# HansiZeng/scaling-retriever

Hardware: AMD Instinct MI355X
Metric: MSMARCO-Dev queries/sec end-to-end (query encode + dense brute-force top-1000) (higher is better)
Workload: dtype f32

## Files before the change

include/sr_hip.h:

```cpp
#ifndef SR_HIP_H
#define SR_HIP_H
#include <stdint.h>
#ifdef __cplusplus
extern "C" {
#endif

#define SR_OK 0
#define SR_ERR_INVALID 1
#define SR_ERR_HIP 2
#define SR_ERR_NOMEM 3
#define SR_ERR_UNSUPPORTED 4

#define SR_DTYPE_F32 0
#define SR_DTYPE_BF16 1

typedef void* sr_stream;

const char* sr_last_error(void);
int sr_version(void);
int sr_max_topk(void);

typedef struct sr_dense_index sr_dense_index;

int sr_dense_index_create(sr_dense_index** out, int dim);
int sr_dense_index_add(sr_dense_index* idx, const float* d_rows, int64_t n_rows,
                       int64_t id_base, int64_t id_stride);
int64_t sr_dense_index_ntotal(const sr_dense_index* idx);
int sr_dense_search(sr_dense_index* idx, const float* d_queries, int64_t nq, int k,
                    float* d_out_scores, int64_t* d_out_ids, sr_stream stream);
#define SR_PRECISION_FP32 0
#define SR_PRECISION_BF16X3 1
#define SR_PRECISION_BF16X6 2
#define SR_PRECISION_FP32_FILTERED 3
int sr_dense_index_set_precision(sr_dense_index* idx, int mode);
int sr_dense_search_begin(sr_dense_index* idx, const float* d_queries, int64_t nq, int k, int share,
                          float* d_lower, sr_stream stream);
int sr_dense_search_finish(sr_dense_index* idx, const float* d_queries, int64_t nq, int k, const float* d_threshold,
                           float* d_out_scores, int64_t* d_out_ids, sr_stream stream);
int sr_dense_index_filter_stats(sr_dense_index* idx, int64_t* n_filtered, int64_t* n_fallback);
int sr_dense_index_filter_query_stats(sr_dense_index* idx, int64_t* n_certified, int64_t* n_redone);
int sr_dense_index_set_workspace_limit(sr_dense_index* idx, int64_t bytes);
int sr_dense_index_set_batch_invariant(sr_dense_index* idx, int on);
int sr_dense_index_destroy(sr_dense_index* idx);
int sr_dense_index_profile(sr_dense_index* idx, int enable);
int sr_dense_index_profile_read(sr_dense_index* idx, int64_t* n_launches, double* total_ms,
                                double* total_flop, double* total_d_bytes);

typedef struct sr_sparse_index sr_sparse_index;

int sr_sparse_index_create(sr_sparse_index** out, const int64_t* d_indptr,
                           const int32_t* d_doc_ids, const float* d_vals,
                           int64_t n_terms, int64_t n_docs, sr_stream stream);
int sr_sparse_search(sr_sparse_index* idx, const int64_t* d_q_indptr, const int32_t* d_q_cols,
                     const float* d_q_vals, int64_t nq, int k, float threshold,
                     int64_t id_base, int64_t id_stride,
                     float* d_out_scores, int64_t* d_out_ids, int32_t* d_out_counts,
                     sr_stream stream);
int sr_sparse_index_set_workspace_limit(sr_sparse_index* idx, int64_t bytes);
int sr_sparse_index_destroy(sr_sparse_index* idx);
int sr_sparse_index_work_counters(sr_sparse_index* idx, int enable, uint64_t* out6);
int sr_sparse_index_profile(sr_sparse_index* idx, int enable);
int sr_sparse_index_profile_read(sr_sparse_index* idx, int64_t* n_launches, double* total_ms,
                                 double* total_posting_bytes);
int sr_sparse_index_block_stats(sr_sparse_index* idx, int64_t* n_dense_terms, int64_t* n_block_calls,
                                int64_t* n_fallback_calls);

int sr_sparse_index_cert_stats(sr_sparse_index* idx, int64_t* out8);
int sr_sparse_index_cert_debug(sr_sparse_index* idx, int enable, uint16_t* h_keys, int64_t keys_capacity,
                               float* h_consts, int64_t nq_pad, float* vscale, int32_t* T);

int sr_sparse_csr_expand_terms(const int64_t* d_indptr, int64_t n_terms, int64_t nnz, int32_t* d_out_terms,
                               sr_stream stream);
int sr_sparse_csr_build(const int32_t* d_rows, const int32_t* d_cols, const float* d_vals, int64_t nnz,
                        int64_t n_terms, int64_t n_docs, int sort_docs, int64_t* d_indptr,
                        int32_t* d_out_rows, float* d_out_vals, sr_stream stream);

int sr_topk_merge(const float* d_scores, const int64_t* d_ids, int n_lists, int64_t nq, int k,
                  float pad_score, float* d_out_scores, int64_t* d_out_ids, sr_stream stream);

typedef struct sr_model sr_model;

typedef struct {
    int32_t vocab_size, hidden_size, intermediate_size, num_layers;
    int32_t num_heads, num_kv_heads, head_dim;
    float rms_norm_eps;
    float rope_theta;
    int32_t rope_llama3;
    float rope_factor, rope_low_freq_factor, rope_high_freq_factor;
    int32_t rope_original_max_pos;
    int32_t tie_word_embeddings;
    int32_t has_lm_head;
    int32_t max_batch_tokens;
    int32_t max_batch_seqs;
    int32_t fp32_planes;
} sr_model_config;

int sr_model_create(sr_model** out, const sr_model_config* cfg);
int sr_model_set_weight(sr_model* m, const char* name, const void* d_ptr, int dtype,
                        int64_t rows, int64_t cols, sr_stream stream);
int sr_model_finalize(sr_model* m);
int sr_encode_dense(sr_model* m, const int64_t* d_input_ids, const int64_t* d_attention_mask,
                    int32_t B, int32_t L, float* d_out, sr_stream stream);
int sr_encode_sparse(sr_model* m, const int64_t* d_input_ids, const int64_t* d_attention_mask,
                     int32_t B, int32_t L, float* d_out, sr_stream stream);
int sr_encode_dense_fp32(sr_model* m, const int64_t* d_input_ids, const int64_t* d_attention_mask,
                         int32_t B, int32_t L, float* d_out, sr_stream stream);
int sr_encode_sparse_fp32(sr_model* m, const int64_t* d_input_ids, const int64_t* d_attention_mask,
                          int32_t B, int32_t L, float* d_out, sr_stream stream);
int sr_encode_both(sr_model* m, const int64_t* d_input_ids, const int64_t* d_attention_mask,
                   int32_t B, int32_t L, int32_t fp32, float* d_out_sparse, float* d_out_dense,
                   sr_stream stream);
int sr_encode_rows(sr_model* m, const int64_t* d_input_ids, const int64_t* d_attention_mask, int32_t B, int32_t L,
                   const int32_t* d_row_shift, int32_t mode, int32_t fp32, float* d_out_sparse, float* d_out_dense,
                   sr_stream stream);
int sr_model_last_hidden(sr_model* m, float* d_out, int64_t capacity_rows, int64_t* n_tokens, sr_stream stream);
int sr_model_destroy(sr_model* m);

int sr_lora_merge(float* d_W, const float* d_A, const float* d_B, int64_t out_features,
                  int64_t in_features, int32_t r, float scale, sr_stream stream);

int sr_sparse_compact(const float* d_reps, int64_t B, int64_t V, int64_t* d_row_ptr,
                      int32_t* d_cols, float* d_vals, int64_t capacity, int64_t* h_nnz,
                      sr_stream stream);

int sr_write_run_json(const char* path, int64_t nq, int64_t k, const float* h_scores, const int64_t* h_idx, const int32_t* h_counts,
                      const int64_t* h_qid_i64, const char* h_qid_bytes, const int64_t* h_qid_off, int64_t qid_width,
                      const int64_t* h_doc_i64, const char* h_doc_bytes, const int64_t* h_doc_off, int64_t doc_width,
                      int64_t n_docs, int32_t n_threads, int64_t* bytes_written);
int sr_write_run_json_part(const char* path, int32_t part, int64_t nq, int64_t k, const float* h_scores, const int64_t* h_idx,
                           const int32_t* h_counts, const int64_t* h_qid_i64, const char* h_qid_bytes, const int64_t* h_qid_off,
                           int64_t qid_width, const int64_t* h_doc_i64, const char* h_doc_bytes, const int64_t* h_doc_off,
                           int64_t doc_width, int64_t n_docs, int32_t n_threads, int64_t* bytes_written);
int64_t sr_run_writer_mapped_rounds(void);

int sr_gemm_bf16(const void* d_A, const void* d_W, int32_t M, int32_t N, int32_t K, int32_t epilogue,
                 void* d_C, const int32_t* d_seq_of, sr_stream stream);
int sr_gemm_f16_scaled(const void* d_A, const void* d_W, int32_t M, int32_t N, int32_t K, const float* d_a_scale,
                       const float* d_w_scale, float* d_C, sr_stream stream);
int sr_gemm_qkv_rope(const void* d_A, const void* d_W, int32_t M, int32_t N, int32_t K, void* d_C,
                     const int32_t* d_pos, const float* d_rope_cos, const float* d_rope_sin,
                     int32_t n_rope, int32_t head_dim, sr_stream stream);
int sr_attention_varlen(const void* d_qkv, void* d_out, const int32_t* d_cu_seqlens, const int32_t* d_pos,
                        const uint8_t* d_key_valid, const float* d_rope_cos, const float* d_rope_sin,
                        int32_t B, int32_t num_heads, int32_t num_kv_heads, int32_t head_dim, sr_stream stream);

#ifdef __cplusplus
}
#endif
#endif
```

scaling_retriever_amd/_lib.py:

```python
import ctypes
import os
import threading

_HERE = os.path.dirname(os.path.abspath(__file__))
LIB_PATH = os.environ.get("SR_HIP_LIB") or os.path.join(_HERE, "libsr_hip.so")

SR_OK, SR_ERR_INVALID, SR_ERR_HIP, SR_ERR_NOMEM, SR_ERR_UNSUPPORTED = 0, 1, 2, 3, 4
SR_DTYPE_F32, SR_DTYPE_BF16 = 0, 1

c_void_p, c_int, c_int32, c_int64, c_float, c_char_p = (ctypes.c_void_p, ctypes.c_int, ctypes.c_int32,
                                                         ctypes.c_int64, ctypes.c_float, ctypes.c_char_p)


class SrModelConfig(ctypes.Structure):
    _fields_ = [
        ("vocab_size", c_int32), ("hidden_size", c_int32), ("intermediate_size", c_int32), ("num_layers", c_int32),
        ("num_heads", c_int32), ("num_kv_heads", c_int32), ("head_dim", c_int32),
        ("rms_norm_eps", c_float), ("rope_theta", c_float), ("rope_llama3", c_int32),
        ("rope_factor", c_float), ("rope_low_freq_factor", c_float), ("rope_high_freq_factor", c_float),
        ("rope_original_max_pos", c_int32), ("tie_word_embeddings", c_int32), ("has_lm_head", c_int32),
        ("max_batch_tokens", c_int32), ("max_batch_seqs", c_int32), ("fp32_planes", c_int32),
    ]


SIGNATURES = {
    "sr_last_error": (c_char_p, []),
    "sr_version": (c_int, []),
    "sr_max_topk": (c_int, []),
    "sr_dense_index_create": (c_int, [ctypes.POINTER(c_void_p), c_int]),
    "sr_dense_index_add": (c_int, [c_void_p, c_void_p, c_int64, c_int64, c_int64]),
    "sr_dense_index_ntotal": (c_int64, [c_void_p]),
    "sr_dense_search": (c_int, [c_void_p, c_void_p, c_int64, c_int, c_void_p, c_void_p, c_void_p]),
    "sr_dense_index_set_workspace_limit": (c_int, [c_void_p, c_int64]),
    "sr_dense_index_set_batch_invariant": (c_int, [c_void_p, c_int]),
    "sr_dense_index_set_precision": (c_int, [c_void_p, c_int]),
    "sr_dense_search_begin": (c_int, [c_void_p, c_void_p, c_int64, c_int, c_int, c_void_p, c_void_p]),
    "sr_dense_search_finish": (c_int, [c_void_p, c_void_p, c_int64, c_int, c_void_p, c_void_p, c_void_p, c_void_p]),
    "sr_dense_index_filter_stats": (c_int, [c_void_p, ctypes.POINTER(c_int64), ctypes.POINTER(c_int64)]),
    "sr_dense_index_filter_query_stats": (c_int, [c_void_p, ctypes.POINTER(c_int64), ctypes.POINTER(c_int64)]),
    "sr_dense_index_destroy": (c_int, [c_void_p]),
    "sr_dense_index_profile": (c_int, [c_void_p, c_int]),
    "sr_dense_index_profile_read": (c_int, [c_void_p, ctypes.POINTER(c_int64), ctypes.POINTER(ctypes.c_double),
                                            ctypes.POINTER(ctypes.c_double), ctypes.POINTER(ctypes.c_double)]),
    "sr_sparse_index_work_counters": (c_int, [c_void_p, c_int, ctypes.POINTER(ctypes.c_uint64)]),
    "sr_sparse_index_profile": (c_int, [c_void_p, c_int]),
    "sr_sparse_index_profile_read": (c_int, [c_void_p, ctypes.POINTER(c_int64), ctypes.POINTER(ctypes.c_double),
                                             ctypes.POINTER(ctypes.c_double)]),
    "sr_sparse_index_create": (c_int, [ctypes.POINTER(c_void_p), c_void_p, c_void_p, c_void_p, c_int64, c_int64,
                                       c_void_p]),
    "sr_sparse_search": (c_int, [c_void_p, c_void_p, c_void_p, c_void_p, c_int64, c_int, c_float, c_int64, c_int64,
                                 c_void_p, c_void_p, c_void_p, c_void_p]),
    "sr_sparse_index_set_workspace_limit": (c_int, [c_void_p, c_int64]),
    "sr_sparse_index_block_stats": (c_int, [c_void_p, ctypes.POINTER(c_int64), ctypes.POINTER(c_int64),
                                            ctypes.POINTER(c_int64)]),
    "sr_sparse_index_destroy": (c_int, [c_void_p]),
    "sr_sparse_index_cert_stats": (c_int, [c_void_p, ctypes.POINTER(c_int64)]),
    "sr_sparse_index_cert_debug": (c_int, [c_void_p, c_int, c_void_p, c_int64, c_void_p, c_int64,
                                           ctypes.POINTER(c_float), ctypes.POINTER(ctypes.c_int32)]),
    "sr_sparse_csr_expand_terms": (c_int, [c_void_p, c_int64, c_int64, c_void_p, c_void_p]),
    "sr_sparse_csr_build": (c_int, [c_void_p, c_void_p, c_void_p, c_int64, c_int64, c_int64, c_int, c_void_p, c_void_p,
                                    c_void_p, c_void_p]),
    "sr_topk_merge": (c_int, [c_void_p, c_void_p, c_int, c_int64, c_int, c_float, c_void_p, c_void_p, c_void_p]),
    "sr_model_create": (c_int, [ctypes.POINTER(c_void_p), ctypes.POINTER(SrModelConfig)]),
    "sr_model_set_weight": (c_int, [c_void_p, c_char_p, c_void_p, c_int, c_int64, c_int64, c_void_p]),
    "sr_model_finalize": (c_int, [c_void_p]),
    "sr_encode_dense": (c_int, [c_void_p, c_void_p, c_void_p, c_int32, c_int32, c_void_p, c_void_p]),
    "sr_encode_sparse": (c_int, [c_void_p, c_void_p, c_void_p, c_int32, c_int32, c_void_p, c_void_p]),
    "sr_encode_dense_fp32": (c_int, [c_void_p, c_void_p, c_void_p, c_int32, c_int32, c_void_p, c_void_p]),
    "sr_encode_sparse_fp32": (c_int, [c_void_p, c_void_p, c_void_p, c_int32, c_int32, c_void_p, c_void_p]),
    "sr_encode_both": (c_int, [c_void_p, c_void_p, c_void_p, c_int32, c_int32, c_int32, c_void_p, c_void_p, c_void_p]),
    "sr_encode_rows": (c_int, [c_void_p, c_void_p, c_void_p, c_int32, c_int32, c_void_p, c_int32, c_int32, c_void_p, c_void_p, c_void_p]),
    "sr_model_last_hidden": (c_int, [c_void_p, c_void_p, c_int64, ctypes.POINTER(c_int64), c_void_p]),
    "sr_model_destroy": (c_int, [c_void_p]),
    "sr_lora_merge": (c_int, [c_void_p, c_void_p, c_void_p, c_int64, c_int64, c_int32, c_float, c_void_p]),
    "sr_run_writer_mapped_rounds": (c_int64, []),
    "sr_write_run_json": (c_int, [c_char_p, c_int64, c_int64, c_void_p, c_void_p, c_void_p, c_void_p, c_void_p, c_void_p, c_int64,
                                  c_void_p, c_void_p, c_void_p, c_int64, c_int64, c_int32, ctypes.POINTER(c_int64)]),
    "sr_write_run_json_part": (c_int, [c_char_p, c_int32, c_int64, c_int64, c_void_p, c_void_p, c_void_p, c_void_p, c_void_p, c_void_p, c_int64,
                                       c_void_p, c_void_p, c_void_p, c_int64, c_int64, c_int32, ctypes.POINTER(c_int64)]),
    "sr_gemm_bf16": (c_int, [c_void_p, c_void_p, c_int32, c_int32, c_int32, c_int32, c_void_p, c_void_p, c_void_p]),
    "sr_gemm_f16_scaled": (c_int, [c_void_p, c_void_p, c_int32, c_int32, c_int32, c_void_p, c_void_p, c_void_p, c_void_p]),
    "sr_gemm_qkv_rope": (c_int, [c_void_p, c_void_p, c_int32, c_int32, c_int32, c_void_p, c_void_p, c_void_p, c_void_p,
                                 c_int32, c_int32, c_void_p]),
    "sr_attention_varlen": (c_int, [c_void_p, c_void_p, c_void_p, c_void_p, c_void_p, c_void_p, c_void_p, c_int32,
                                    c_int32, c_int32, c_int32, c_void_p]),
    "sr_sparse_compact": (c_int, [c_void_p, c_int64, c_int64, c_void_p, c_void_p, c_void_p, c_int64,
                                  ctypes.POINTER(c_int64), c_void_p]),
}

_lib = None
_lock = threading.Lock()


class SrHipError(RuntimeError):
    pass


def load():
    global _lib
    with _lock:
        if _lib is not None:
            return _lib
        if not os.path.exists(LIB_PATH):
            raise SrHipError(
                f"{LIB_PATH} not found: the HIP extension is not built. There is no CPU fallback; "
                "run `make -C scaling_retriever_amd/csrc` (needs hipcc, targets gfx950).")
        import torch
        lib = ctypes.CDLL(LIB_PATH)
        for name, (res, args) in SIGNATURES.items():
            fn = getattr(lib, name)
            fn.restype = res
            fn.argtypes = args
        _lib = lib
        return lib


def check(rc, what=""):
    if rc == SR_OK:
        return
    msg = load().sr_last_error().decode("utf-8", "replace")
    if rc == SR_ERR_INVALID:
        raise ValueError(f"{what}: {msg}" if what else msg)
    if rc == SR_ERR_NOMEM:
        raise MemoryError(f"{what}: {msg}" if what else msg)
    raise SrHipError(f"{what}: [{rc}] {msg}" if what else f"[{rc}] {msg}")


def stream_ptr():
    import torch
    return ctypes.c_void_p(torch.cuda.current_stream().cuda_stream)


def require_gpu():
    import torch
    if not torch.cuda.is_available():
        raise SrHipError("no ROCm device visible: scaling_retriever_amd runs its hot path on MI355X only "
                         "(there is no CPU fallback)")
```

scaling_retriever_amd/csrc/encoder.hip:

```cpp
#include "kernels.h"
#include <math.h>
#include <mutex>
#include <string>
#include <vector>

__global__ void plan_rows_kernel(const int64_t* __restrict__ mask, int B, int L, int mode, int* __restrict__ span_start,
                                 int* __restrict__ span_len, int* __restrict__ pool_start, int* __restrict__ row_len,
                                 const int* __restrict__ row_shift) {
    const int b = blockIdx.x;
    const int lane = threadIdx.x;
    int len = 0, first = L, last = -1;
    for (int p = lane; p < L; p += 64) {
        if (mask[(int64_t)b * L + p] != 0) {
            ++len;
            first = p < first ? p : first;
            last = p > last ? p : last;
        }
    }
    for (int off = 32; off > 0; off >>= 1) {
        len += __shfl_xor(len, off);
        const int f = __shfl_xor(first, off), l = __shfl_xor(last, off);
        first = f < first ? f : first;
        last = l > last ? l : last;
    }
    if (lane == 0) {
        int st, ln, ps;
        if (len == 0) {
            st = 0; ln = 0; ps = 0;
        } else if (mode != 1) {
            ps = L - len;
            st = first < ps ? first : ps;
            ln = L - st;
        } else {
            ps = first;
            st = first;
            ln = last + 1 - first;
        }
        span_start[b] = st;
        span_len[b] = ln;
        pool_start[b] = ps - (row_shift ? row_shift[b] : 0);
        row_len[b] = len;
    }
}

__global__ void plan_scan_kernel(const int* __restrict__ span_len, int B, int* __restrict__ cu) {
    __shared__ int part[256];
    const int tid = threadIdx.x;
    const int per = (B + 255) / 256;
    const int b0 = tid * per, b1 = (b0 + per) < B ? (b0 + per) : B;
    int s = 0;
    for (int b = b0; b < b1; ++b) s += span_len[b];
    part[tid] = s;
    __syncthreads();
    if (tid == 0) {
        int run = 0;
        for (int i = 0; i < 256; ++i) { const int v = part[i]; part[i] = run; run += v; }
        cu[B] = run;
    }
    __syncthreads();
    int run = part[tid];
    for (int b = b0; b < b1; ++b) { cu[b] = run; run += span_len[b]; }
}

__global__ void plan_tokens_kernel(const int64_t* __restrict__ ids, const int64_t* __restrict__ mask, int L,
                                   const int* __restrict__ span_start, const int* __restrict__ cu, int* __restrict__ tok_id,
                                   int* __restrict__ pos, unsigned char* __restrict__ key_valid, int* __restrict__ seq_of,
                                   int vocab, int mode, const int* __restrict__ row_shift) {
    const int b = blockIdx.x;
    const int t0 = cu[b], n = cu[b + 1] - t0, st = span_start[b];
    const int shift = row_shift ? row_shift[b] : 0;
    for (int j = threadIdx.x; j < n; j += blockDim.x) {
        const int p = st + j;
        int64_t id = ids[(int64_t)b * L + p];
        id = id < 0 ? 0 : (id >= vocab ? vocab - 1 : id);
        tok_id[t0 + j] = (int)id;
        pos[t0 + j] = p - shift < 0 ? 0 : p - shift;
        const bool valid = mask[(int64_t)b * L + p] != 0;
        key_valid[t0 + j] = valid ? 1 : 0;
        seq_of[t0 + j] = (mode != 0 && !valid) ? -2 : b;
    }
}

template <int NCH>
__global__ __launch_bounds__(256) void rmsnorm_kernel(float* __restrict__ x, const float* __restrict__ embed,
                                                      const int* __restrict__ tok_id, const bf16_t* __restrict__ delta,
                                                      const float* __restrict__ w, bf16_t* __restrict__ xn,
                                                      float* __restrict__ xn_f32, int T, int H, float eps) {
    const int t = blockIdx.x * 4 + (threadIdx.x >> 6);
    const int lane = threadIdx.x & 63;
    if (t >= T) return;
    float* xr = x + (int64_t)t * H;
    const float* src = embed ? embed + (int64_t)tok_id[t] * H : xr;
    const bf16_t* dr = delta ? delta + (int64_t)t * H : nullptr;
    float ss = 0.f;
    if constexpr (NCH > 0) {
        f32x4 v[NCH];
#pragma unroll
        for (int c = 0; c < NCH; ++c) v[c] = *reinterpret_cast<const f32x4*>(src + lane * 4 + c * 256);
        if (dr) {
            bf16x4 d[NCH];
#pragma unroll
            for (int c = 0; c < NCH; ++c) d[c] = *reinterpret_cast<const bf16x4*>(dr + lane * 4 + c * 256);
#pragma unroll
            for (int c = 0; c < NCH; ++c)
#pragma unroll
                for (int e = 0; e < 4; ++e) v[c][e] += bf16_to_f32((unsigned short)d[c][e]);
        }
#pragma unroll
        for (int c = 0; c < NCH; ++c) {
            ss += v[c][0] * v[c][0] + v[c][1] * v[c][1] + v[c][2] * v[c][2] + v[c][3] * v[c][3];
            if (embed || dr) *reinterpret_cast<f32x4*>(xr + lane * 4 + c * 256) = v[c];
        }
        for (int off = 32; off > 0; off >>= 1) ss += __shfl_xor(ss, off);
        const float rs = 1.0f / sqrtf(ss / (float)H + eps);
        if (!w) return;
#pragma unroll
        for (int c = 0; c < NCH; ++c) {
            const int i = lane * 4 + c * 256;
            const f32x4 g = *reinterpret_cast<const f32x4*>(w + i);
            f32x4 y;
#pragma unroll
            for (int e = 0; e < 4; ++e) y[e] = (v[c][e] * rs) * g[e];
            if (xn) {
                bf16x4 o;
#pragma unroll
                for (int e = 0; e < 4; ++e) o[e] = (short)f32_to_bf16(y[e]);
                *reinterpret_cast<bf16x4*>(xn + (int64_t)t * H + i) = o;
            }
            if (xn_f32) *reinterpret_cast<f32x4*>(xn_f32 + (int64_t)t * H + i) = y;
        }
    } else {
        for (int i = lane * 4; i < H; i += 256) {
            f32x4 v = *reinterpret_cast<const f32x4*>(src + i);
            if (dr) {
                const bf16x4 d = *reinterpret_cast<const bf16x4*>(dr + i);
#pragma unroll
                for (int c = 0; c < 4; ++c) v[c] += bf16_to_f32((unsigned short)d[c]);
            }
            ss += v[0] * v[0] + v[1] * v[1] + v[2] * v[2] + v[3] * v[3];
            if (embed || dr) *reinterpret_cast<f32x4*>(xr + i) = v;
        }
        for (int off = 32; off > 0; off >>= 1) ss += __shfl_xor(ss, off);
        const float rs = 1.0f / sqrtf(ss / (float)H + eps);
        if (!w) return;
        for (int i = lane * 4; i < H; i += 256) {
            const f32x4 v = *reinterpret_cast<const f32x4*>(xr + i);
            const f32x4 g = *reinterpret_cast<const f32x4*>(w + i);
            f32x4 y;
#pragma unroll
            for (int c = 0; c < 4; ++c) y[c] = (v[c] * rs) * g[c];
            if (xn) {
                bf16x4 o;
#pragma unroll
                for (int c = 0; c < 4; ++c) o[c] = (short)f32_to_bf16(y[c]);
                *reinterpret_cast<bf16x4*>(xn + (int64_t)t * H + i) = o;
            }
            if (xn_f32) *reinterpret_cast<f32x4*>(xn_f32 + (int64_t)t * H + i) = y;
        }
    }
}

static int launch_rmsnorm(float* x, const float* embed, const int* tok_id, const bf16_t* delta, const float* w, bf16_t* xn,
                          float* xn_f32, int T, int H, float eps, hipStream_t s) {
    if (T == 0) return SR_OK;
    const dim3 grid((unsigned)ceil_div64(T, 4)), block(256);
#define SR_RMS(NCH) hipLaunchKernelGGL(rmsnorm_kernel<NCH>, grid, block, 0, s, x, embed, tok_id, delta, w, xn, xn_f32, T, H, eps)
    switch (H) {
        case 256: SR_RMS(1); break;
        case 512: SR_RMS(2); break;
        case 1024: SR_RMS(4); break;
        case 2048: SR_RMS(8); break;
        case 3072: SR_RMS(12); break;
        case 4096: SR_RMS(16); break;
        default: SR_RMS(0); break;
    }
#undef SR_RMS
    SR_CHECK_LAUNCH();
    return SR_OK;
}

__global__ __launch_bounds__(256) void dense_head_stats_kernel(const float* __restrict__ x, const float* __restrict__ w,
                                                               float2* __restrict__ stats, int T, int H, float eps) {
    const int t = blockIdx.x * 4 + (threadIdx.x >> 6);
    const int lane = threadIdx.x & 63;
    if (t >= T) return;
    const float* xr = x + (int64_t)t * H;
    float ss = 0.f;
    for (int i = lane * 4; i < H; i += 256) {
        const f32x4 v = *reinterpret_cast<const f32x4*>(xr + i);
        ss += v[0] * v[0] + v[1] * v[1] + v[2] * v[2] + v[3] * v[3];
    }
    for (int off = 32; off > 0; off >>= 1) ss += __shfl_xor(ss, off);
    const float rs = 1.0f / sqrtf(ss / (float)H + eps);
    float s2 = 0.f;
    for (int i = lane * 4; i < H; i += 256) {
        const f32x4 v = *reinterpret_cast<const f32x4*>(xr + i);
        const f32x4 g = *reinterpret_cast<const f32x4*>(w + i);
#pragma unroll
        for (int c = 0; c < 4; ++c) { const float y = (v[c] * rs) * g[c]; s2 += y * y; }
    }
    for (int off = 32; off > 0; off >>= 1) s2 += __shfl_xor(s2, off);
    if (lane == 0) stats[t] = make_float2(rs, 1.0f / fmaxf(sqrtf(s2), 1e-12f));
}
__global__ __launch_bounds__(256) void dense_head_pool_kernel(const float* __restrict__ x, const float* __restrict__ w,
                                                              const float2* __restrict__ stats, const int* __restrict__ cu,
                                                              const int* __restrict__ pos, const int* __restrict__ pool_start,
                                                              float* __restrict__ out, int H) {
    const int b = blockIdx.x, c = blockIdx.y * 256 + threadIdx.x;
    if (c >= H) return;
    const int t0 = cu[b], n = cu[b + 1] - t0, ps = pool_start[b];
    const float wc = w[c];
    float acc = 0.f;
    int cnt = 0;
    for (int j = 0; j < n; ++j) {
        const int t = t0 + j;
        if (pos[t] < ps) continue;
        const float2 st = stats[t];
        acc += ((x[(int64_t)t * H + c] * st.x) * wc) * st.y;
        ++cnt;
    }
    out[(int64_t)b * H + c] = cnt > 0 ? acc / (float)cnt : 0.f;
}

__global__ void sparse_finish_kernel(float* __restrict__ out, int64_t n, float scale, int round_bf16) {
    const int64_t i = (int64_t)blockIdx.x * blockDim.x + threadIdx.x;
    if (i >= n) return;
    float v = out[i];
    if (round_bf16) v = bf16_to_f32(f32_to_bf16(v));
    v *= scale;
    out[i] = logf(fmaxf(v, 0.f) + 1.0f);
}

__global__ void convert_rows_kernel(const void* __restrict__ src, int src_dtype, int64_t rows, int64_t cols,
                                    bf16_t* __restrict__ dst_bf16, float* __restrict__ dst_f32, int64_t dst_row_base,
                                    int interleave ) {
    const int64_t r = blockIdx.x;
    int64_t dr = r;
    if (interleave) dr = (r / 16) * 32 + (interleave == 2 ? 16 : 0) + (r % 16);
    dr += dst_row_base;
    for (int64_t c = threadIdx.x; c < cols; c += blockDim.x) {
        float v;
        if (src_dtype == SR_DTYPE_F32) v = reinterpret_cast<const float*>(src)[r * cols + c];
        else v = bf16_to_f32(reinterpret_cast<const bf16_t*>(src)[r * cols + c]);
        if (dst_bf16) dst_bf16[dr * cols + c] = f32_to_bf16(v);
        if (dst_f32) dst_f32[dr * cols + c] = v;
    }
}

__global__ void convert_rows_split_kernel(const void* __restrict__ src, int src_dtype, int64_t rows, int64_t cols,
                                          bf16_t* __restrict__ dst, int64_t dst_row_base, int interleave, SplitMap map) {
    const int64_t r = blockIdx.x;
    int64_t dr = r;
    if (interleave) dr = (r / 16) * 32 + (interleave == 2 ? 16 : 0) + (r % 16);
    dr += dst_row_base;
    bf16_t* drow = dst + dr * cols * map.n_seg;
    for (int64_t c = threadIdx.x; c < cols; c += blockDim.x) {
        float v;
        if (src_dtype == SR_DTYPE_F32) v = reinterpret_cast<const float*>(src)[r * cols + c];
        else v = bf16_to_f32(reinterpret_cast<const bf16_t*>(src)[r * cols + c]);
        unsigned short p[3];
        split_bf16x3(v, p[0], p[1], p[2]);
        for (int sg = 0; sg < map.n_seg; ++sg) drow[(int64_t)sg * cols + c] = p[map.plane[sg]];
    }
}

__global__ __launch_bounds__(256) void rmsnorm_split_kernel(float* __restrict__ x, const float* __restrict__ embed,
                                                            const int* __restrict__ tok_id, const float* __restrict__ w,
                                                            bf16_t* __restrict__ xs, int T, int H, float eps, SplitMap map) {
    const int t = blockIdx.x * 4 + (threadIdx.x >> 6);
    const int lane = threadIdx.x & 63;
    if (t >= T) return;
    float* xr = x + (int64_t)t * H;
    const float* src = embed ? embed + (int64_t)tok_id[t] * H : xr;
    float ss = 0.f;
    for (int i = lane * 4; i < H; i += 256) {
        const f32x4 v = *reinterpret_cast<const f32x4*>(src + i);
        ss += v[0] * v[0] + v[1] * v[1] + v[2] * v[2] + v[3] * v[3];
        if (embed) *reinterpret_cast<f32x4*>(xr + i) = v;
    }
    for (int off = 32; off > 0; off >>= 1) ss += __shfl_xor(ss, off);
    const float rs = 1.0f / sqrtf(ss / (float)H + eps);
    bf16_t* orow = xs + (int64_t)t * H * map.n_seg;
    for (int i = lane * 4; i < H; i += 256) {
        const f32x4 v = *reinterpret_cast<const f32x4*>(src + i);
        const f32x4 g = *reinterpret_cast<const f32x4*>(w + i);
        bf16x4 pl[3];
#pragma unroll
        for (int c = 0; c < 4; ++c) {
            unsigned short a0, a1, a2;
            split_bf16x3((v[c] * rs) * g[c], a0, a1, a2);
            pl[0][c] = (short)a0; pl[1][c] = (short)a1; pl[2][c] = (short)a2;
        }
        for (int sg = 0; sg < map.n_seg; ++sg) {
            const int pi = map.plane[sg];
            *reinterpret_cast<bf16x4*>(orow + (int64_t)sg * H + i) = pi == 0 ? pl[0] : (pi == 1 ? pl[1] : pl[2]);
        }
    }
}

__global__ __launch_bounds__(256) void convert_rows_split_h_kernel(const void* __restrict__ src, int src_dtype, int64_t rows, int64_t cols,
                                                                   bf16_t* __restrict__ dst, float* __restrict__ w_inv,
                                                                   int64_t dst_row_base, int interleave) {
    __shared__ float red[4];
    const int64_t r = blockIdx.x;
    int64_t dr = r;
    if (interleave) dr = (r / 16) * 32 + (interleave == 2 ? 16 : 0) + (r % 16);
    dr += dst_row_base;
    auto at = [&](int64_t c) {
        return src_dtype == SR_DTYPE_F32 ? reinterpret_cast<const float*>(src)[r * cols + c]
                                         : bf16_to_f32(reinterpret_cast<const bf16_t*>(src)[r * cols + c]);
    };
    float mx = 0.f;
    for (int64_t c = threadIdx.x; c < cols; c += 256) mx = fmaxf(mx, fabsf(at(c)));
    for (int off = 32; off > 0; off >>= 1) mx = fmaxf(mx, __shfl_xor(mx, off));
    if ((threadIdx.x & 63) == 0) red[threadIdx.x >> 6] = mx;
    __syncthreads();
    mx = fmaxf(fmaxf(red[0], red[1]), fmaxf(red[2], red[3]));
    const float sc = row_scale_pow2(mx);
    if (threadIdx.x == 0) w_inv[dr] = 1.0f / sc;
    bf16_t* drow = dst + dr * cols * 3;
    for (int64_t c = threadIdx.x; c < cols; c += 256) {
        unsigned short f0, f1;
        split_f16x2(at(c) * sc, f0, f1);
        drow[c] = f0; drow[cols + c] = f1; drow[2 * cols + c] = f0;
    }
}

__global__ __launch_bounds__(256) void rows_split_h_kernel(float* __restrict__ x, const float* __restrict__ embed,
                                                           const int* __restrict__ tok_id, const float* __restrict__ w,
                                                           bf16_t* __restrict__ xs, float* __restrict__ a_inv, int T, int K, float eps,
                                                           const float* __restrict__ gu_cmax, float* __restrict__ act_sc,
                                                           float* __restrict__ act_inv) {
    const int t = blockIdx.x * 4 + (threadIdx.x >> 6);
    const int lane = threadIdx.x & 63;
    if (t >= T) return;
    float* xr = x + (int64_t)t * K;
    const float* src = embed ? embed + (int64_t)tok_id[t] * K : xr;
    float rs = 1.f;
    if (w) {
        float ss = 0.f;
        for (int i = lane * 4; i < K; i += 256) {
            const f32x4 v = *reinterpret_cast<const f32x4*>(src + i);
            ss += v[0] * v[0] + v[1] * v[1] + v[2] * v[2] + v[3] * v[3];
            if (embed) *reinterpret_cast<f32x4*>(xr + i) = v;
        }
        for (int off = 32; off > 0; off >>= 1) ss += __shfl_xor(ss, off);
        rs = 1.0f / sqrtf(ss / (float)K + eps);
    }
    float mx = 0.f, s2 = 0.f;
    for (int i = lane * 4; i < K; i += 256) {
        const f32x4 v = *reinterpret_cast<const f32x4*>(src + i);
        f32x4 g = {1.f, 1.f, 1.f, 1.f};
        if (w) g = *reinterpret_cast<const f32x4*>(w + i);
#pragma unroll
        for (int c = 0; c < 4; ++c) {
            const float y = w ? (v[c] * rs) * g[c] : v[c];
            mx = fmaxf(mx, fabsf(y));
            s2 += y * y;
        }
    }
    for (int off = 32; off > 0; off >>= 1) mx = fmaxf(mx, __shfl_xor(mx, off));
    const float sc = row_scale_pow2(mx);
    if (lane == 0) a_inv[t] = 1.0f / sc;
    if (gu_cmax) {
        for (int off = 32; off > 0; off >>= 1) s2 += __shfl_xor(s2, off);
        const float osc = row_scale_pow2(s2 * *gu_cmax * 1.02f);
        if (lane == 0) { act_sc[t] = osc; act_inv[t] = 1.0f / osc; }
    }
    bf16_t* orow = xs + (int64_t)t * K * 3;
    for (int i = lane * 4; i < K; i += 256) {
        const f32x4 v = *reinterpret_cast<const f32x4*>(src + i);
        f32x4 g = {1.f, 1.f, 1.f, 1.f};
        if (w) g = *reinterpret_cast<const f32x4*>(w + i);
        bf16x4 p0, p1;
#pragma unroll
        for (int c = 0; c < 4; ++c) {
            unsigned short f0, f1;
            split_f16x2((w ? (v[c] * rs) * g[c] : v[c]) * sc, f0, f1);
            p0[c] = (short)f0; p1[c] = (short)f1;
        }
        *reinterpret_cast<bf16x4*>(orow + i) = p1;
        *reinterpret_cast<bf16x4*>(orow + K + i) = p0;
        *reinterpret_cast<bf16x4*>(orow + 2 * K + i) = p0;
    }
}

template <int NV>
__global__ __launch_bounds__(256) void rows_split_h_reg_kernel(float* __restrict__ x, const float* __restrict__ embed,
                                                               const int* __restrict__ tok_id, const float* __restrict__ w,
                                                               bf16_t* __restrict__ xs, float* __restrict__ a_inv, int T, float eps,
                                                               const float* __restrict__ gu_cmax, float* __restrict__ act_sc,
                                                               float* __restrict__ act_inv) {
    constexpr int K = 256 * NV;
    const int t = blockIdx.x * 4 + (threadIdx.x >> 6);
    const int lane = threadIdx.x & 63;
    if (t >= T) return;
    float* xr = x + (int64_t)t * K;
    const float* src = embed ? embed + (int64_t)tok_id[t] * K : xr;
    f32x4 v[NV];
#pragma unroll
    for (int j = 0; j < NV; ++j) v[j] = *reinterpret_cast<const f32x4*>(src + lane * 4 + 256 * j);
    if (w) {
        float ss = 0.f;
#pragma unroll
        for (int j = 0; j < NV; ++j) {
            ss += v[j][0] * v[j][0] + v[j][1] * v[j][1] + v[j][2] * v[j][2] + v[j][3] * v[j][3];
            if (embed) *reinterpret_cast<f32x4*>(xr + lane * 4 + 256 * j) = v[j];
        }
        for (int off = 32; off > 0; off >>= 1) ss += __shfl_xor(ss, off);
        const float rs = 1.0f / sqrtf(ss / (float)K + eps);
#pragma unroll
        for (int j = 0; j < NV; ++j) {
            const f32x4 g = *reinterpret_cast<const f32x4*>(w + lane * 4 + 256 * j);
#pragma unroll
            for (int c = 0; c < 4; ++c) v[j][c] = (v[j][c] * rs) * g[c];
        }
    }
    float mx = 0.f;
#pragma unroll
    for (int j = 0; j < NV; ++j)
#pragma unroll
        for (int c = 0; c < 4; ++c) mx = fmaxf(mx, fabsf(v[j][c]));
    for (int off = 32; off > 0; off >>= 1) mx = fmaxf(mx, __shfl_xor(mx, off));
    const float sc = row_scale_pow2(mx);
    if (lane == 0) a_inv[t] = 1.0f / sc;
    if (gu_cmax) {
        float s2 = 0.f;
#pragma unroll
        for (int j = 0; j < NV; ++j) s2 += v[j][0] * v[j][0] + v[j][1] * v[j][1] + v[j][2] * v[j][2] + v[j][3] * v[j][3];
        for (int off = 32; off > 0; off >>= 1) s2 += __shfl_xor(s2, off);
        const float osc = row_scale_pow2(s2 * *gu_cmax * 1.02f);
        if (lane == 0) { act_sc[t] = osc; act_inv[t] = 1.0f / osc; }
    }
    bf16_t* orow = xs + (int64_t)t * K * 3;
#pragma unroll
    for (int j = 0; j < NV; ++j) {
        bf16x4 p0, p1;
#pragma unroll
        for (int c = 0; c < 4; ++c) {
            unsigned short f0, f1;
            split_f16x2(v[j][c] * sc, f0, f1);
            p0[c] = (short)f0; p1[c] = (short)f1;
        }
        const int i = lane * 4 + 256 * j;
        *reinterpret_cast<bf16x4*>(orow + i) = p1;
        *reinterpret_cast<bf16x4*>(orow + K + i) = p0;
        *reinterpret_cast<bf16x4*>(orow + 2 * K + i) = p0;
    }
}

static void launch_rows_split_h(float* x, const float* embed, const int* tok, const float* w, bf16_t* xs, float* inv, int T, int K,
                                float eps, hipStream_t s, const float* gu_cmax = nullptr, float* act_sc = nullptr,
                                float* act_inv = nullptr) {
    const dim3 grid((unsigned)ceil_div64(T, 4)), block(256);
    switch (K) {
        case 2048: hipLaunchKernelGGL(rows_split_h_reg_kernel<8>, grid, block, 0, s, x, embed, tok, w, xs, inv, T, eps, gu_cmax, act_sc, act_inv); break;
        case 4096: hipLaunchKernelGGL(rows_split_h_reg_kernel<16>, grid, block, 0, s, x, embed, tok, w, xs, inv, T, eps, gu_cmax, act_sc, act_inv); break;
        case 8192: hipLaunchKernelGGL(rows_split_h_reg_kernel<32>, grid, block, 0, s, x, embed, tok, w, xs, inv, T, eps, gu_cmax, act_sc, act_inv); break;
        default: hipLaunchKernelGGL(rows_split_h_kernel, grid, block, 0, s, x, embed, tok, w, xs, inv, T, K, eps, gu_cmax, act_sc, act_inv);
    }
}

__global__ __launch_bounds__(256) void gu_cmax_kernel(const bf16_t* __restrict__ wgu_s, const float* __restrict__ wgu_i, int I, int K,
                                                      float* __restrict__ cmax) {
    const int j = blockIdx.x * 4 + (threadIdx.x >> 6);
    const int lane = threadIdx.x & 63;
    if (j >= I) return;
    const int64_t rg = (int64_t)(j / 16) * 32 + (j % 16), ru = rg + 16;
    float n2[2];
#pragma unroll
    for (int h = 0; h < 2; ++h) {
        const bf16_t* row = wgu_s + (h ? ru : rg) * 3 * (int64_t)K;
        float ss = 0.f;
        for (int i = lane; i < K; i += 64) {
            const float v = (float)__builtin_bit_cast(_Float16, row[i]) + (float)__builtin_bit_cast(_Float16, row[K + i]);
            ss += v * v;
        }
        for (int off = 32; off > 0; off >>= 1) ss += __shfl_xor(ss, off);
        const float inv = wgu_i[h ? ru : rg];
        n2[h] = ss * inv * inv;
    }
    if (lane == 0) atomicMax(reinterpret_cast<unsigned int*>(cmax), __float_as_uint(sqrtf(n2[0]) * sqrtf(n2[1]) * 1.001f));
}

__global__ void lora_merge_kernel(float* __restrict__ W, const float* __restrict__ A, const float* __restrict__ Bm,
                                  int64_t out_f, int64_t in_f, int r, float scale) {
    const int64_t o = blockIdx.y;
    const int64_t i = (int64_t)blockIdx.x * blockDim.x + threadIdx.x;
    if (i >= in_f) return;
    float acc = 0.f;
    for (int k = 0; k < r; ++k) acc += Bm[o * r + k] * A[(int64_t)k * in_f + i];
    W[o * in_f + i] += scale * acc;
}

__global__ __launch_bounds__(256) void nnz_count_kernel(const float* __restrict__ reps, int64_t V, int64_t* __restrict__ row_nnz) {
    __shared__ int red[4];
    const int64_t b = blockIdx.x;
    int c = 0;
    for (int64_t i = threadIdx.x; i < V; i += 256) c += reps[b * V + i] != 0.f ? 1 : 0;
    for (int off = 32; off > 0; off >>= 1) c += __shfl_xor(c, off);
    if ((threadIdx.x & 63) == 0) red[threadIdx.x >> 6] = c;
    __syncthreads();
    if (threadIdx.x == 0) row_nnz[b] = red[0] + red[1] + red[2] + red[3];
}
__global__ void nnz_scan_kernel(const int64_t* __restrict__ row_nnz, int64_t B, int64_t* __restrict__ row_ptr) {
    if (threadIdx.x == 0 && blockIdx.x == 0) {
        int64_t run = 0;
        for (int64_t b = 0; b < B; ++b) { row_ptr[b] = run; run += row_nnz[b]; }
        row_ptr[B] = run;
    }
}
__global__ __launch_bounds__(256) void nnz_fill_kernel(const float* __restrict__ reps, int64_t V, const int64_t* __restrict__ row_ptr,
                                                       int32_t* __restrict__ cols, float* __restrict__ vals, int64_t capacity) {
    __shared__ int wtot[4];
    __shared__ int64_t base;
    const int64_t b = blockIdx.x;
    const int tid = threadIdx.x, lane = tid & 63, wave = tid >> 6;
    if (tid == 0) base = row_ptr[b];
    __syncthreads();
    for (int64_t i0 = 0; i0 < V; i0 += 256) {
        const int64_t i = i0 + tid;
        const float v = i < V ? reps[b * V + i] : 0.f;
        const int nz = v != 0.f ? 1 : 0;
        int incl = nz;
        for (int off = 1; off < 64; off <<= 1) { const int o = __shfl_up(incl, off); if (lane >= off) incl += o; }
        if (lane == 63) wtot[wave] = incl;
        __syncthreads();
        int wb = 0, tot = 0;
        for (int w = 0; w < 4; ++w) { if (w < wave) wb += wtot[w]; tot += wtot[w]; }
        const int64_t p = base + wb + incl - nz;
        if (nz && p < capacity) { cols[p] = (int32_t)i; vals[p] = v; }
        __syncthreads();
        if (tid == 0) base += tot;
        __syncthreads();
    }
}

struct LayerW {
    bf16_t* wqkv = nullptr;
    bf16_t* wo = nullptr;
    bf16_t* wgu = nullptr;
    bf16_t* wdown = nullptr;
    float* ln1 = nullptr;
    float* ln2 = nullptr;
    unsigned have = 0;
    bf16_t *wqkv_s = nullptr, *wo_s = nullptr, *wgu_s = nullptr, *wdown_s = nullptr;
    float *wqkv_i = nullptr, *wo_i = nullptr, *wgu_i = nullptr, *wdown_i = nullptr;
    float* gu_cmax = nullptr;
};

struct sr_model {
    sr_model_config cfg;
    int Tm = 0, Bm = 0;
    int max_pos = 0;
    float* embed = nullptr;
    bf16_t* lm_head = nullptr;
    bf16_t* lm_head_s = nullptr;
    float* lm_head_i = nullptr;
    float *attn_f = nullptr, *act_f = nullptr;
    float *xs_i = nullptr, *attn_i = nullptr, *act_i = nullptr;
    float* act_sc = nullptr;
    bf16_t* xs = nullptr;
    float* qkv_f = nullptr;
    bf16_t* attn_s = nullptr;
    bf16_t* act_s = nullptr;
    float* norm_w = nullptr;
    std::vector<LayerW> layers;
    bool have_embed = false, have_norm = false, have_lm_head = false, finalized = false;
    float* rope_cos = nullptr;
    float* rope_sin = nullptr;
    float* x = nullptr;
    bf16_t* xn = nullptr;
    bf16_t* qkv = nullptr;
    bf16_t* attn = nullptr;
    bf16_t* act = nullptr;
    bf16_t* delta = nullptr;
    int *span_start = nullptr, *span_len = nullptr, *pool_start = nullptr, *row_len = nullptr, *cu = nullptr;
    int *tok_id = nullptr, *pos = nullptr, *seq_of = nullptr;
    unsigned char* key_valid = nullptr;
    int* h_cu = nullptr;
    int last_T = 0;
    std::mutex mu;
    StreamOrder order;
};

static void model_free(sr_model* m) {
    auto F = [](void* p) { if (p) (void)hipFree(p); };
    F(m->embed); F(m->lm_head); F(m->norm_w); F(m->rope_cos); F(m->rope_sin);
    F(m->lm_head_s); F(m->xs); F(m->qkv_f); F(m->attn_s); F(m->act_s);
    F(m->lm_head_i); F(m->attn_f); F(m->act_f); F(m->xs_i); F(m->attn_i); F(m->act_i); F(m->act_sc);
    for (auto& l : m->layers) {
        F(l.wqkv); F(l.wo); F(l.wgu); F(l.wdown); F(l.ln1); F(l.ln2); F(l.wqkv_s); F(l.wo_s); F(l.wgu_s); F(l.wdown_s);
        F(l.wqkv_i); F(l.wo_i); F(l.wgu_i); F(l.wdown_i); F(l.gu_cmax);
    }
    F(m->x); F(m->xn); F(m->qkv); F(m->attn); F(m->act); F(m->delta);
    F(m->span_start); F(m->span_len); F(m->pool_start); F(m->row_len); F(m->cu);
    F(m->tok_id); F(m->pos); F(m->seq_of); F(m->key_valid);
    if (m->h_cu) (void)hipHostFree(m->h_cu);
}

#define SR_ALLOC(ptr, bytes)                                                                      \
    do {                                                                                          \
        const hipError_t e_ = hipMalloc((void**)&(ptr), (size_t)(bytes));                          \
        if (e_ != hipSuccess) {                                                                   \
            sr_set_error("sr_model_create: hipMalloc of %zu bytes failed: %s", (size_t)(bytes), hipGetErrorString(e_)); \
            model_free(m);                                                                        \
            delete m;                                                                             \
            return SR_ERR_NOMEM;                                                                  \
        }                                                                                         \
    } while (0)

static void rope_tables(const sr_model_config& c, int max_pos, std::vector<float>& cosv, std::vector<float>& sinv) {
    const int hd = c.head_dim, half = hd / 2;
    std::vector<float> inv(half);
    for (int i = 0; i < half; ++i) {
        double f = 1.0 / pow((double)c.rope_theta, (double)(2 * i) / (double)hd);
        if (c.rope_llama3) {
            const double factor = c.rope_factor, lo = c.rope_low_freq_factor, hi = c.rope_high_freq_factor;
            const double old = (double)c.rope_original_max_pos;
            const double low_wl = old / lo, high_wl = old / hi;
            const double wl = 2.0 * M_PI / f;
            const double f_l = wl > low_wl ? f / factor : f;
            if (!(wl < high_wl) && !(wl > low_wl)) {
                const double smooth = (old / wl - lo) / (hi - lo);
                f = (1.0 - smooth) * f_l / factor + smooth * f_l;
            } else {
                f = f_l;
            }
        }
        inv[i] = (float)f;
    }
    cosv.resize((size_t)max_pos * half);
    sinv.resize((size_t)max_pos * half);
    for (int p = 0; p < max_pos; ++p)
        for (int i = 0; i < half; ++i) {
            const float ang = (float)p * inv[i];
            cosv[(size_t)p * half + i] = (float)cos((double)ang);
            sinv[(size_t)p * half + i] = (float)sin((double)ang);
        }
}

extern "C" int sr_model_create(sr_model** out, const sr_model_config* cfg) {
    SR_REQUIRE(out && cfg, "sr_model_create: null argument");
    const sr_model_config& c = *cfg;
    SR_REQUIRE(c.vocab_size > 0 && c.hidden_size > 0 && c.intermediate_size > 0 && c.num_layers > 0,
               "sr_model_create: bad dimensions");
    SR_REQUIRE(c.num_heads > 0 && c.num_kv_heads > 0 && c.num_heads % c.num_kv_heads == 0,
               "sr_model_create: num_heads %d must be a multiple of num_kv_heads %d", c.num_heads, c.num_kv_heads);
    SR_REQUIRE(c.head_dim == 64 || c.head_dim == 128, "sr_model_create: head_dim %d not supported (64 or 128)", c.head_dim);
    SR_REQUIRE(c.hidden_size % 64 == 0 && c.intermediate_size % 64 == 0,
               "sr_model_create: hidden_size and intermediate_size must be multiples of 64");
    SR_REQUIRE(c.vocab_size % 16 == 0 || !c.has_lm_head, "sr_model_create: vocab_size must be a multiple of 16 for the sparse head");
    SR_REQUIRE(c.max_batch_tokens > 0 && c.max_batch_seqs > 0 && c.max_batch_seqs <= 65536, "sr_model_create: bad workspace sizes");
    SR_REQUIRE(c.fp32_planes == 0 || c.fp32_planes == 2 || c.fp32_planes == 3 || c.fp32_planes == SR_FP32_PLANES_F16,
               "sr_model_create: fp32_planes must be 0, 2, 3 or 16");
    sr_model* m = new sr_model();
    m->cfg = c;
    m->Tm = (int)(ceil_div64(c.max_batch_tokens, 128) * 128);
    m->Bm = c.max_batch_seqs;
    m->max_pos = 8192;
    m->layers.resize(c.num_layers);
    const int64_t H = c.hidden_size, I = c.intermediate_size, V = c.vocab_size;
    const int64_t nq = (int64_t)c.num_heads * c.head_dim, nkv = (int64_t)c.num_kv_heads * c.head_dim;
    SR_ALLOC(m->embed, V * H * 4);
    if (c.has_lm_head) SR_ALLOC(m->lm_head, V * H * 2);
    const int64_t nsg = c.fp32_planes ? split_map_w(c.fp32_planes).n_seg : 0;
    const bool f16p = c.fp32_planes == SR_FP32_PLANES_F16;
    if (c.has_lm_head && nsg) SR_ALLOC(m->lm_head_s, V * H * 2 * nsg);
    if (c.has_lm_head && f16p) SR_ALLOC(m->lm_head_i, V * 4);
    SR_ALLOC(m->norm_w, H * 4);
    for (auto& l : m->layers) {
        SR_ALLOC(l.wqkv, (nq + 2 * nkv) * H * 2);
        SR_ALLOC(l.wo, H * nq * 2);
        SR_ALLOC(l.wgu, 2 * I * H * 2);
        SR_ALLOC(l.wdown, H * I * 2);
        if (nsg) {
            SR_ALLOC(l.wqkv_s, (nq + 2 * nkv) * H * 2 * nsg);
            SR_ALLOC(l.wo_s, H * nq * 2 * nsg);
            SR_ALLOC(l.wgu_s, 2 * I * H * 2 * nsg);
            SR_ALLOC(l.wdown_s, H * I * 2 * nsg);
        }
        if (f16p) {
            SR_ALLOC(l.wqkv_i, (nq + 2 * nkv) * 4);
            SR_ALLOC(l.wo_i, H * 4);
            SR_ALLOC(l.wgu_i, 2 * I * 4);
            SR_ALLOC(l.wdown_i, H * 4);
        }
        SR_ALLOC(l.ln1, H * 4);
        SR_ALLOC(l.ln2, H * 4);
    }
    SR_ALLOC(m->rope_cos, (int64_t)m->max_pos * (c.head_dim / 2) * 4);
    SR_ALLOC(m->rope_sin, (int64_t)m->max_pos * (c.head_dim / 2) * 4);
    const int64_t Tm = m->Tm;
    SR_ALLOC(m->x, Tm * H * 4);
    SR_ALLOC(m->xn, Tm * H * 2);
    SR_ALLOC(m->qkv, Tm * (nq + 2 * nkv) * 2);
    SR_ALLOC(m->attn, Tm * nq * 2);
    SR_ALLOC(m->act, Tm * I * 2);
    SR_ALLOC(m->delta, Tm * H * 2);
    SR_ALLOC(m->span_start, m->Bm * 4);
    SR_ALLOC(m->span_len, m->Bm * 4);
    SR_ALLOC(m->pool_start, m->Bm * 4);
    SR_ALLOC(m->row_len, m->Bm * 4);
    SR_ALLOC(m->cu, (m->Bm + 1) * 4);
    SR_ALLOC(m->tok_id, Tm * 4);
    SR_ALLOC(m->pos, Tm * 4);
    SR_ALLOC(m->seq_of, Tm * 4);
    SR_ALLOC(m->key_valid, Tm);
    if (hipHostMalloc((void**)&m->h_cu, (size_t)(2 * m->Bm + 2) * 4) != hipSuccess) {
        sr_set_error("sr_model_create: hipHostMalloc failed");
        model_free(m);
        delete m;
        return SR_ERR_NOMEM;
    }
    (void)hipMemset(m->xn, 0, (size_t)(Tm * H * 2));
    (void)hipMemset(m->attn, 0, (size_t)(Tm * nq * 2));
    (void)hipMemset(m->act, 0, (size_t)(Tm * I * 2));
    std::vector<float> cs, sn;
    rope_tables(c, m->max_pos, cs, sn);
    if (hipMemcpy(m->rope_cos, cs.data(), cs.size() * 4, hipMemcpyHostToDevice) != hipSuccess ||
        hipMemcpy(m->rope_sin, sn.data(), sn.size() * 4, hipMemcpyHostToDevice) != hipSuccess) {
        sr_set_error("sr_model_create: rope table upload failed");
        model_free(m);
        delete m;
        return SR_ERR_HIP;
    }
    *out = m;
    return SR_OK;
}

extern "C" int sr_model_destroy(sr_model* m) {
    if (!m) return SR_OK;
    model_free(m);
    m->order.release();
    delete m;
    return SR_OK;
}

static int convert_rows(const void* src, int dtype, int64_t rows, int64_t cols, bf16_t* dbf, float* df32, int64_t base,
                        int interleave, hipStream_t s, bf16_t* dsplit = nullptr, int planes = 0, float* w_inv = nullptr) {
    hipLaunchKernelGGL(convert_rows_kernel, dim3((unsigned)rows), dim3(256), 0, s, src, dtype, rows, cols, dbf, df32, base,
                       interleave);
    if (dsplit && planes == SR_FP32_PLANES_F16)
        hipLaunchKernelGGL(convert_rows_split_h_kernel, dim3((unsigned)rows), dim3(256), 0, s, src, dtype, rows, cols, dsplit, w_inv, base,
                           interleave);
    else if (dsplit && planes)
        hipLaunchKernelGGL(convert_rows_split_kernel, dim3((unsigned)rows), dim3(256), 0, s, src, dtype, rows, cols, dsplit, base,
                           interleave, split_map_w(planes));
    SR_CHECK_LAUNCH();
    return SR_OK;
}

extern "C" int sr_model_set_weight(sr_model* m, const char* name, const void* d_ptr, int dtype, int64_t rows, int64_t cols,
                                   sr_stream stream) {
    SR_REQUIRE(m && name && d_ptr, "sr_model_set_weight: null argument");
    SR_REQUIRE(dtype == SR_DTYPE_F32 || dtype == SR_DTYPE_BF16, "sr_model_set_weight: dtype %d not supported", dtype);
    hipStream_t s = (hipStream_t)stream;
    std::lock_guard<std::mutex> lock(m->mu);
    const sr_model_config& c = m->cfg;
    const int64_t H = c.hidden_size, I = c.intermediate_size, V = c.vocab_size;
    const int64_t nq = (int64_t)c.num_heads * c.head_dim, nkv = (int64_t)c.num_kv_heads * c.head_dim;
    std::string n(name);
    auto shape_is = [&](int64_t r, int64_t cc) { return rows == r && cols == cc; };
#define SHAPE_REQ(r, cc) SR_REQUIRE(shape_is((r), (cc)), "sr_model_set_weight: %s has shape [%lld, %lld], expected [%lld, %lld]", name, (long long)rows, (long long)cols, (long long)(r), (long long)(cc))
    if (n == "model.embed_tokens.weight") {
        SHAPE_REQ(V, H);
        SR_TRY(convert_rows(d_ptr, dtype, V, H, (c.has_lm_head && c.tie_word_embeddings) ? m->lm_head : nullptr, m->embed, 0, 0, s,
                            (c.has_lm_head && c.tie_word_embeddings) ? m->lm_head_s : nullptr, c.fp32_planes, m->lm_head_i));
        m->have_embed = true;
        if (c.has_lm_head && c.tie_word_embeddings) m->have_lm_head = true;
        return SR_OK;
    }
    if (n == "lm_head.weight") {
        SR_REQUIRE(c.has_lm_head, "sr_model_set_weight: model was created without an lm_head");
        SHAPE_REQ(V, H);
        SR_TRY(convert_rows(d_ptr, dtype, V, H, m->lm_head, nullptr, 0, 0, s, m->lm_head_s, c.fp32_planes, m->lm_head_i));
        m->have_lm_head = true;
        return SR_OK;
    }
    if (n == "model.norm.weight") {
        SHAPE_REQ(H, 1);
        SR_TRY(convert_rows(d_ptr, dtype, H, 1, nullptr, m->norm_w, 0, 0, s));
        m->have_norm = true;
        return SR_OK;
    }
    int li = -1;
    char rest[128] = {0};
    if (sscanf(name, "model.layers.%d.%127s", &li, rest) == 2 && li >= 0 && li < c.num_layers) {
        LayerW& l = m->layers[li];
        std::string r(rest);
        if (r == "self_attn.q_proj.weight") { SHAPE_REQ(nq, H); SR_TRY(convert_rows(d_ptr, dtype, nq, H, l.wqkv, nullptr, 0, 0, s, l.wqkv_s, c.fp32_planes, l.wqkv_i)); l.have |= 1; return SR_OK; }
        if (r == "self_attn.k_proj.weight") { SHAPE_REQ(nkv, H); SR_TRY(convert_rows(d_ptr, dtype, nkv, H, l.wqkv, nullptr, nq, 0, s, l.wqkv_s, c.fp32_planes, l.wqkv_i)); l.have |= 2; return SR_OK; }
        if (r == "self_attn.v_proj.weight") { SHAPE_REQ(nkv, H); SR_TRY(convert_rows(d_ptr, dtype, nkv, H, l.wqkv, nullptr, nq + nkv, 0, s, l.wqkv_s, c.fp32_planes, l.wqkv_i)); l.have |= 4; return SR_OK; }
        if (r == "self_attn.o_proj.weight") { SHAPE_REQ(H, nq); SR_TRY(convert_rows(d_ptr, dtype, H, nq, l.wo, nullptr, 0, 0, s, l.wo_s, c.fp32_planes, l.wo_i)); l.have |= 8; return SR_OK; }
        if (r == "mlp.gate_proj.weight") { SHAPE_REQ(I, H); SR_TRY(convert_rows(d_ptr, dtype, I, H, l.wgu, nullptr, 0, 1, s, l.wgu_s, c.fp32_planes, l.wgu_i)); l.have |= 16; return SR_OK; }
        if (r == "mlp.up_proj.weight") { SHAPE_REQ(I, H); SR_TRY(convert_rows(d_ptr, dtype, I, H, l.wgu, nullptr, 0, 2, s, l.wgu_s, c.fp32_planes, l.wgu_i)); l.have |= 32; return SR_OK; }
        if (r == "mlp.down_proj.weight") { SHAPE_REQ(H, I); SR_TRY(convert_rows(d_ptr, dtype, H, I, l.wdown, nullptr, 0, 0, s, l.wdown_s, c.fp32_planes, l.wdown_i)); l.have |= 64; return SR_OK; }
        if (r == "input_layernorm.weight") { SHAPE_REQ(H, 1); SR_TRY(convert_rows(d_ptr, dtype, H, 1, nullptr, l.ln1, 0, 0, s)); l.have |= 128; return SR_OK; }
        if (r == "post_attention_layernorm.weight") { SHAPE_REQ(H, 1); SR_TRY(convert_rows(d_ptr, dtype, H, 1, nullptr, l.ln2, 0, 0, s)); l.have |= 256; return SR_OK; }
    }
    sr_set_error("sr_model_set_weight: unknown tensor name '%s'", name);
    return SR_ERR_INVALID;
}

extern "C" int sr_model_finalize(sr_model* m) {
    SR_REQUIRE(m, "sr_model_finalize: null model");
    SR_REQUIRE(m->have_embed, "sr_model_finalize: model.embed_tokens.weight missing");
    SR_REQUIRE(m->have_norm, "sr_model_finalize: model.norm.weight missing");
    SR_REQUIRE(!m->cfg.has_lm_head || m->have_lm_head, "sr_model_finalize: lm_head.weight missing");
    for (int i = 0; i < m->cfg.num_layers; ++i)
        SR_REQUIRE(m->layers[i].have == 511, "sr_model_finalize: layer %d is missing tensors (mask 0x%x)", i, m->layers[i].have);
    SR_CHECK_HIP(hipDeviceSynchronize());
    if (m->cfg.fp32_planes == SR_FP32_PLANES_F16) {
        for (int i = 0; i < m->cfg.num_layers; ++i) {
            LayerW& l = m->layers[i];
            if (!l.gu_cmax) SR_CHECK_HIP(hipMalloc((void**)&l.gu_cmax, 4));
            SR_CHECK_HIP(hipMemsetAsync(l.gu_cmax, 0, 4, nullptr));
            hipLaunchKernelGGL(gu_cmax_kernel, dim3((unsigned)ceil_div64(m->cfg.intermediate_size, 4)), dim3(256), 0, nullptr, l.wgu_s, l.wgu_i,
                               m->cfg.intermediate_size, m->cfg.hidden_size, l.gu_cmax);
        }
        SR_CHECK_LAUNCH();
    }
    SR_CHECK_HIP(hipDeviceSynchronize());
    m->finalized = true;
    return SR_OK;
}

enum { PREC_BF16 = 0, PREC_FP32 = 1 };

static int ensure_fp32_workspace(sr_model* m) {
    if (m->xs) return SR_OK;
    const sr_model_config& c = m->cfg;
    SR_REQUIRE(c.fp32_planes > 0, "encode(fp32): the model was created with fp32_planes = 0 (bf16 regime only)");
    const int64_t Tm = m->Tm, H = c.hidden_size, I = c.intermediate_size;
    const int64_t nq = (int64_t)c.num_heads * c.head_dim, nkv = (int64_t)c.num_kv_heads * c.head_dim;
    const int64_t nsg = split_map_a(c.fp32_planes).n_seg;
    auto A = [&](void** p, int64_t bytes) {
        if (hipMalloc(p, (size_t)bytes) != hipSuccess) { *p = nullptr; return false; }
        return hipMemset(*p, 0, (size_t)bytes) == hipSuccess;
    };
    const bool f16p = c.fp32_planes == SR_FP32_PLANES_F16;
    bool ok = A((void**)&m->xs, Tm * H * 2 * nsg) && A((void**)&m->qkv_f, Tm * (nq + 2 * nkv) * 4) &&
              A((void**)&m->attn_s, Tm * nq * 2 * nsg) && A((void**)&m->act_s, Tm * I * 2 * nsg);
    if (ok && f16p)
        ok = A((void**)&m->attn_f, Tm * nq * 4) && A((void**)&m->act_f, Tm * I * 4) && A((void**)&m->xs_i, Tm * 4) &&
             A((void**)&m->attn_i, Tm * 4) && A((void**)&m->act_i, Tm * 4) && A((void**)&m->act_sc, Tm * 4);
    if (!ok) {
        auto F = [](void* p) { if (p) (void)hipFree(p); };
        F(m->xs); F(m->qkv_f); F(m->attn_s); F(m->act_s); F(m->attn_f); F(m->act_f); F(m->xs_i); F(m->attn_i); F(m->act_i);
        m->xs = nullptr; m->qkv_f = nullptr; m->attn_s = nullptr; m->act_s = nullptr;
        m->attn_f = nullptr; m->act_f = nullptr; m->xs_i = nullptr; m->attn_i = nullptr; m->act_i = nullptr;
        sr_set_error("encode(fp32): hipMalloc of the fp32-regime workspace failed (%lld tokens)", (long long)Tm);
        return SR_ERR_NOMEM;
    }
    return SR_OK;
}

static int launch_rmsnorm_split(float* x, const float* embed, const int* tok_id, const float* w, bf16_t* xs, int T, int H,
                                float eps, const SplitMap& map, hipStream_t s) {
    if (T == 0) return SR_OK;
    hipLaunchKernelGGL(rmsnorm_split_kernel, dim3((unsigned)ceil_div64(T, 4)), dim3(256), 0, s, x, embed, tok_id, w, xs, T, H, eps,
                       map);
    SR_CHECK_LAUNCH();
    return SR_OK;
}

static int model_forward(sr_model* m, const int64_t* d_ids, const int64_t* d_mask, int B, int L, int mode, int prec,
                         hipStream_t s, int* T_out, const int32_t* d_shift = nullptr) {
    const sr_model_config& c = m->cfg;
    SR_REQUIRE(m->finalized, "encode: sr_model_finalize was not called");
    SR_REQUIRE(B >= 1 && L >= 1, "encode: bad batch shape [%d, %d]", B, L);
    SR_REQUIRE(B <= m->Bm, "encode: batch of %d sequences exceeds max_batch_seqs %d", B, m->Bm);
    SR_REQUIRE(L <= m->max_pos, "encode: sequence length %d exceeds %d", L, m->max_pos);
    SR_REQUIRE(d_ids && d_mask, "encode: null input");
    if (prec == PREC_FP32) SR_TRY(ensure_fp32_workspace(m));
    const int H = c.hidden_size, I = c.intermediate_size;
    const int nq = c.num_heads * c.head_dim, nkv = c.num_kv_heads * c.head_dim;

    hipLaunchKernelGGL(plan_rows_kernel, dim3(B), dim3(64), 0, s, d_mask, B, L, mode, m->span_start, m->span_len,
                       m->pool_start, m->row_len, d_shift);
    hipLaunchKernelGGL(plan_scan_kernel, dim3(1), dim3(256), 0, s, m->span_len, B, m->cu);
    SR_CHECK_LAUNCH();
    SR_CHECK_HIP(hipMemcpyAsync(m->h_cu, m->cu, (size_t)(B + 1) * 4, hipMemcpyDeviceToHost, s));
    SR_CHECK_HIP(hipStreamSynchronize(s));
    const int T = m->h_cu[B];
    int max_len = 0;
    for (int b = 0; b < B; ++b) max_len = (m->h_cu[b + 1] - m->h_cu[b]) > max_len ? (m->h_cu[b + 1] - m->h_cu[b]) : max_len;
    SR_REQUIRE(T <= m->Tm, "encode: batch packs to %d tokens, workspace holds %d (raise max_batch_tokens or split the batch)", T, m->Tm);
    *T_out = T;
    m->last_T = T;
    if (T == 0) return SR_OK;
    hipLaunchKernelGGL(plan_tokens_kernel, dim3(B), dim3(128), 0, s, d_ids, d_mask, L, m->span_start, m->cu, m->tok_id,
                       m->pos, m->key_valid, m->seq_of, c.vocab_size, mode, d_shift);
    SR_CHECK_LAUNCH();

    if (prec == PREC_FP32 && c.fp32_planes == SR_FP32_PLANES_F16) {
        auto split_rows = [&](float* src, const float* embed, const int* tok, const float* w, bf16_t* dst, float* inv, int K) {
            launch_rows_split_h(src, embed, tok, w, dst, inv, T, K, c.rms_norm_eps, s);
        };
        const char* env_fa = sr_dev_getenv("SR_FP32_FUSED_ACT");
        const bool fused_act = m->layers[0].gu_cmax && !(env_fa && *env_fa == '0');
        for (int li = 0; li < c.num_layers; ++li) {
            LayerW& l = m->layers[li];
            split_rows(m->x, li == 0 ? m->embed : (const float*)nullptr, li == 0 ? m->tok_id : (const int*)nullptr, l.ln1, m->xs, m->xs_i, H);
            GemmArgs g{};
            g.A = m->xs; g.W = l.wqkv_s; g.M = T; g.N = nq + 2 * nkv; g.K = 3 * H; g.C = m->qkv_f; g.a_scale = m->xs_i; g.w_scale = l.wqkv_i;
            g.pos = m->pos; g.rope_cos = m->rope_cos; g.rope_sin = m->rope_sin; g.n_rope = nq + nkv; g.head_dim = c.head_dim;
            SR_TRY(launch_gemm_bf16(EPI_QKV_ROPE_F32_H, g, s));
            AttnF32Args a{};
            a.qkv = m->qkv_f; a.out_f32 = m->attn_f; a.out = nullptr; a.cu_seqlens = m->cu; a.key_valid = m->key_valid;
            a.B = B; a.nh = c.num_heads; a.nkv = c.num_kv_heads; a.hd = c.head_dim;
            a.scale = 1.0f / sqrtf((float)c.head_dim); a.max_seqlen = max_len;
            SR_TRY(launch_attention_f32(a, s));
            split_rows(m->attn_f, nullptr, nullptr, nullptr, m->attn_s, m->attn_i, nq);
            g = GemmArgs{};
            g.A = m->attn_s; g.W = l.wo_s; g.M = T; g.N = H; g.K = 3 * nq; g.C = m->x; g.a_scale = m->attn_i; g.w_scale = l.wo_i;
            SR_TRY(launch_gemm_bf16(EPI_RESID_F32_H, g, s));
            if (fused_act) {
                launch_rows_split_h(m->x, nullptr, nullptr, l.ln2, m->xs, m->xs_i, T, H, c.rms_norm_eps, s, l.gu_cmax, m->act_sc, m->act_i);
                g = GemmArgs{};
                g.A = m->xs; g.W = l.wgu_s; g.M = T; g.N = 2 * I; g.K = 3 * H; g.C = m->act_s; g.a_scale = m->xs_i; g.w_scale = l.wgu_i;
                g.out_scale = m->act_sc;
                SR_TRY(launch_gemm_bf16(EPI_SWIGLU_SPLIT_H, g, s));
            } else {
                split_rows(m->x, nullptr, nullptr, l.ln2, m->xs, m->xs_i, H);
                g = GemmArgs{};
                g.A = m->xs; g.W = l.wgu_s; g.M = T; g.N = 2 * I; g.K = 3 * H; g.C = m->act_f; g.a_scale = m->xs_i; g.w_scale = l.wgu_i;
                SR_TRY(launch_gemm_bf16(EPI_SWIGLU_F32_H, g, s));
                split_rows(m->act_f, nullptr, nullptr, nullptr, m->act_s, m->act_i, I);
            }
            g = GemmArgs{};
            g.A = m->act_s; g.W = l.wdown_s; g.M = T; g.N = H; g.K = 3 * I; g.C = m->x; g.a_scale = m->act_i; g.w_scale = l.wdown_i;
            SR_TRY(launch_gemm_bf16(EPI_RESID_F32_H, g, s));
        }
        SR_CHECK_LAUNCH();
        return SR_OK;
    }
    if (prec == PREC_FP32) {
        const SplitMap ma = split_map_a(c.fp32_planes);
        const int nsg = ma.n_seg;
        for (int li = 0; li < c.num_layers; ++li) {
            LayerW& l = m->layers[li];
            SR_TRY(launch_rmsnorm_split(m->x, li == 0 ? m->embed : (const float*)nullptr, li == 0 ? m->tok_id : (const int*)nullptr,
                                        l.ln1, m->xs, T, H, c.rms_norm_eps, ma, s));
            GemmArgs g{};
            g.A = m->xs; g.W = l.wqkv_s; g.M = T; g.N = nq + 2 * nkv; g.K = nsg * H; g.C = m->qkv_f;
            g.pos = m->pos; g.rope_cos = m->rope_cos; g.rope_sin = m->rope_sin; g.n_rope = nq + nkv; g.head_dim = c.head_dim;
            SR_TRY(launch_gemm_bf16(EPI_QKV_ROPE_F32, g, s));
            AttnF32Args a{};
            a.qkv = m->qkv_f; a.out = m->attn_s; a.cu_seqlens = m->cu; a.key_valid = m->key_valid;
            a.B = B; a.nh = c.num_heads; a.nkv = c.num_kv_heads; a.hd = c.head_dim;
            a.scale = 1.0f / sqrtf((float)c.head_dim); a.max_seqlen = max_len; a.out_map = ma;
            SR_TRY(launch_attention_f32(a, s));
            g = GemmArgs{};
            g.A = m->attn_s; g.W = l.wo_s; g.M = T; g.N = H; g.K = nsg * nq; g.C = m->x;
            SR_TRY(launch_gemm_bf16(EPI_RESID_F32, g, s));
            SR_TRY(launch_rmsnorm_split(m->x, (const float*)nullptr, (const int*)nullptr, l.ln2, m->xs, T, H, c.rms_norm_eps, ma, s));
            g = GemmArgs{};
            g.A = m->xs; g.W = l.wgu_s; g.M = T; g.N = 2 * I; g.K = nsg * H; g.C = m->act_s; g.out_map = ma;
            SR_TRY(launch_gemm_bf16(EPI_SWIGLU_SPLIT, g, s));
            g = GemmArgs{};
            g.A = m->act_s; g.W = l.wdown_s; g.M = T; g.N = H; g.K = nsg * I; g.C = m->x;
            SR_TRY(launch_gemm_bf16(EPI_RESID_F32, g, s));
        }
        return SR_OK;
    }

    SR_TRY(launch_rmsnorm(m->x, m->embed, m->tok_id, (const bf16_t*)nullptr, m->layers[0].ln1, m->xn,
                       (float*)nullptr, T, H, c.rms_norm_eps, s));
    for (int li = 0; li < c.num_layers; ++li) {
        LayerW& l = m->layers[li];
        if (li > 0) {
            SR_TRY(launch_rmsnorm(m->x, (const float*)nullptr, (const int*)nullptr,
                               (const bf16_t*)m->delta, l.ln1, m->xn, (float*)nullptr, T, H, c.rms_norm_eps, s));
        }
        GemmArgs g{};
        g.A = m->xn; g.W = l.wqkv; g.M = T; g.N = nq + 2 * nkv; g.K = H; g.C = m->qkv;
        g.pos = m->pos; g.rope_cos = m->rope_cos; g.rope_sin = m->rope_sin; g.n_rope = nq + nkv; g.head_dim = c.head_dim;
        SR_TRY(launch_gemm_bf16(EPI_QKV_ROPE, g, s));
        AttnArgs a{};
        a.qkv = m->qkv; a.out = m->attn; a.cu_seqlens = m->cu; a.pos = m->pos; a.key_valid = m->key_valid;
        a.rope_cos = m->rope_cos; a.rope_sin = m->rope_sin; a.B = B; a.nh = c.num_heads; a.nkv = c.num_kv_heads;
        a.hd = c.head_dim; a.scale = 1.0f / sqrtf((float)c.head_dim);
        a.apply_rope = 0; a.max_seqlen = max_len;
        SR_TRY(launch_attention(a, s));
        g = GemmArgs{};
        g.A = m->attn; g.W = l.wo; g.M = T; g.N = H; g.K = nq; g.C = m->delta;
        SR_TRY(launch_gemm_bf16(EPI_STORE_BF16, g, s));
        SR_TRY(launch_rmsnorm(m->x, (const float*)nullptr, (const int*)nullptr,
                           (const bf16_t*)m->delta, l.ln2, m->xn, (float*)nullptr, T, H, c.rms_norm_eps, s));
        g = GemmArgs{};
        g.A = m->xn; g.W = l.wgu; g.M = T; g.N = 2 * I; g.K = H; g.C = m->act;
        SR_TRY(launch_gemm_bf16(EPI_SWIGLU, g, s));
        g = GemmArgs{};
        g.A = m->act; g.W = l.wdown; g.M = T; g.N = H; g.K = I; g.C = m->delta;
        SR_TRY(launch_gemm_bf16(EPI_STORE_BF16, g, s));
    }
    SR_TRY(launch_rmsnorm(m->x, (const float*)nullptr, (const int*)nullptr,
                       (const bf16_t*)m->delta, (const float*)nullptr, (bf16_t*)nullptr, (float*)nullptr, T, H, c.rms_norm_eps, s));
    return SR_OK;
}

static int head_dense(sr_model* m, int B, int T, int prec, float* d_out, hipStream_t s) {
    const int H = m->cfg.hidden_size;
    if (T == 0) {
        SR_CHECK_HIP(hipMemsetAsync(d_out, 0, (size_t)B * H * 4, s));
        return SR_OK;
    }
    float2* stats = reinterpret_cast<float2*>(prec == PREC_FP32 ? (void*)m->xs : (void*)m->xn);
    hipLaunchKernelGGL(dense_head_stats_kernel, dim3((unsigned)ceil_div64(T, 4)), dim3(256), 0, s, m->x, m->norm_w, stats, T, H,
                       m->cfg.rms_norm_eps);
    hipLaunchKernelGGL(dense_head_pool_kernel, dim3((unsigned)B, (unsigned)ceil_div64(H, 256)), dim3(256), 0, s, m->x, m->norm_w,
                       stats, m->cu, m->pos, m->pool_start, d_out, H);
    SR_CHECK_LAUNCH();
    return SR_OK;
}

static int head_sparse(sr_model* m, int B, int T, int prec, float* d_out, hipStream_t s) {
    const int H = m->cfg.hidden_size, V = m->cfg.vocab_size;
    SR_CHECK_HIP(hipMemsetAsync(d_out, 0, (size_t)B * V * 4, s));
    if (T == 0) return SR_OK;
    GemmArgs g{};
    GemmEpilogue epi = EPI_SEGMAX;
    if (prec == PREC_FP32 && m->cfg.fp32_planes == SR_FP32_PLANES_F16) {
        launch_rows_split_h(m->x, (const float*)nullptr, (const int*)nullptr, (const float*)m->norm_w, m->xs, m->xs_i, T, H,
                            m->cfg.rms_norm_eps, s);
        g.A = m->xs; g.W = m->lm_head_s; g.K = 3 * H; g.a_scale = m->xs_i; g.w_scale = m->lm_head_i;
        epi = EPI_SEGMAX_H;
    } else if (prec == PREC_FP32) {
        const SplitMap ma = split_map_a(m->cfg.fp32_planes);
        SR_TRY(launch_rmsnorm_split(m->x, (const float*)nullptr, (const int*)nullptr, m->norm_w, m->xs, T, H, m->cfg.rms_norm_eps,
                                    ma, s));
        g.A = m->xs; g.W = m->lm_head_s; g.K = ma.n_seg * H;
    } else {
        SR_TRY(launch_rmsnorm(m->x, (const float*)nullptr,
                           (const int*)nullptr, (const bf16_t*)nullptr, m->norm_w, m->xn, (float*)nullptr, T, H, m->cfg.rms_norm_eps, s));
        g.A = m->xn; g.W = m->lm_head; g.K = H;
    }
    g.M = T; g.N = V; g.C = d_out; g.seq_of = m->seq_of; g.out_ld = V;
    SR_TRY(launch_gemm_bf16(epi, g, s));
    const int64_t n = (int64_t)B * V;
    hipLaunchKernelGGL(sparse_finish_kernel, dim3((unsigned)ceil_div64(n, 256)), dim3(256), 0, s, d_out, n,
                       powf((float)H, -0.25f), prec == PREC_FP32 ? 0 : 1);
    SR_CHECK_LAUNCH();
    return SR_OK;
}

static int encode_any(sr_model* m, const int64_t* d_input_ids, const int64_t* d_attention_mask, int32_t B, int32_t L, int mode,
                      int prec, float* d_dense, float* d_sparse, hipStream_t s, const int32_t* d_shift = nullptr) {
    std::lock_guard<std::mutex> lock(m->mu);
    StreamOrder::Scope in_order(m->order, s);
    int T = 0;
    SR_TRY(model_forward(m, d_input_ids, d_attention_mask, B, L, mode, prec, s, &T, d_shift));
    if (mode != 1) SR_TRY(head_dense(m, B, T, prec, d_dense, s));
    if (mode != 0) SR_TRY(head_sparse(m, B, T, prec, d_sparse, s));
    return SR_OK;
}

static int encode_dense(sr_model* m, const int64_t* d_input_ids, const int64_t* d_attention_mask, int32_t B, int32_t L, int prec,
                        float* d_out, hipStream_t s) {
    return encode_any(m, d_input_ids, d_attention_mask, B, L, 0, prec, d_out, nullptr, s);
}

static int encode_sparse(sr_model* m, const int64_t* d_input_ids, const int64_t* d_attention_mask, int32_t B, int32_t L, int prec,
                         float* d_out, hipStream_t s) {
    return encode_any(m, d_input_ids, d_attention_mask, B, L, 1, prec, nullptr, d_out, s);
}

extern "C" int sr_encode_dense(sr_model* m, const int64_t* d_input_ids, const int64_t* d_attention_mask, int32_t B, int32_t L,
                               float* d_out, sr_stream stream) {
    SR_REQUIRE(m && d_out, "sr_encode_dense: null argument");
    return encode_dense(m, d_input_ids, d_attention_mask, B, L, PREC_BF16, d_out, (hipStream_t)stream);
}

extern "C" int sr_encode_dense_fp32(sr_model* m, const int64_t* d_input_ids, const int64_t* d_attention_mask, int32_t B, int32_t L,
                                    float* d_out, sr_stream stream) {
    SR_REQUIRE(m && d_out, "sr_encode_dense_fp32: null argument");
    return encode_dense(m, d_input_ids, d_attention_mask, B, L, PREC_FP32, d_out, (hipStream_t)stream);
}

extern "C" int sr_encode_sparse(sr_model* m, const int64_t* d_input_ids, const int64_t* d_attention_mask, int32_t B, int32_t L,
                                float* d_out, sr_stream stream) {
    SR_REQUIRE(m && d_out, "sr_encode_sparse: null argument");
    SR_REQUIRE(m->cfg.has_lm_head, "sr_encode_sparse: model was created without an lm_head (LlamaBiModel)");
    return encode_sparse(m, d_input_ids, d_attention_mask, B, L, PREC_BF16, d_out, (hipStream_t)stream);
}

extern "C" int sr_encode_sparse_fp32(sr_model* m, const int64_t* d_input_ids, const int64_t* d_attention_mask, int32_t B, int32_t L,
                                     float* d_out, sr_stream stream) {
    SR_REQUIRE(m && d_out, "sr_encode_sparse_fp32: null argument");
    SR_REQUIRE(m->cfg.has_lm_head, "sr_encode_sparse_fp32: model was created without an lm_head (LlamaBiModel)");
    return encode_sparse(m, d_input_ids, d_attention_mask, B, L, PREC_FP32, d_out, (hipStream_t)stream);
}

extern "C" int sr_encode_both(sr_model* m, const int64_t* d_input_ids, const int64_t* d_attention_mask, int32_t B, int32_t L,
                              int32_t fp32, float* d_out_sparse, float* d_out_dense, sr_stream stream) {
    SR_REQUIRE(m && d_out_sparse && d_out_dense, "sr_encode_both: null argument");
    SR_REQUIRE(m->cfg.has_lm_head, "sr_encode_both: model was created without an lm_head (LlamaBiModel)");
    return encode_any(m, d_input_ids, d_attention_mask, B, L, 2, fp32 ? PREC_FP32 : PREC_BF16, d_out_dense, d_out_sparse,
                      (hipStream_t)stream);
}

extern "C" int sr_encode_rows(sr_model* m, const int64_t* d_input_ids, const int64_t* d_attention_mask, int32_t B, int32_t L,
                              const int32_t* d_row_shift, int32_t mode, int32_t fp32, float* d_out_sparse, float* d_out_dense,
                              sr_stream stream) {
    SR_REQUIRE(m, "sr_encode_rows: null model");
    SR_REQUIRE(mode >= 0 && mode <= 2, "sr_encode_rows: mode %d (0 dense, 1 sparse, 2 both)", mode);
    SR_REQUIRE(mode == 1 || d_out_dense, "sr_encode_rows: null dense output");
    SR_REQUIRE(mode == 0 || d_out_sparse, "sr_encode_rows: null sparse output");
    SR_REQUIRE(mode == 0 || m->cfg.has_lm_head, "sr_encode_rows: model was created without an lm_head (LlamaBiModel)");
    return encode_any(m, d_input_ids, d_attention_mask, B, L, mode, fp32 ? PREC_FP32 : PREC_BF16, d_out_dense, d_out_sparse,
                      (hipStream_t)stream, d_row_shift);
}

extern "C" int sr_model_last_hidden(sr_model* m, float* d_out, int64_t capacity_rows, int64_t* n_tokens, sr_stream stream) {
    SR_REQUIRE(m && d_out && n_tokens, "sr_model_last_hidden: null argument");
    hipStream_t s = (hipStream_t)stream;
    std::lock_guard<std::mutex> lock(m->mu);
    StreamOrder::Scope in_order(m->order, s);
    const int T = m->last_T;
    *n_tokens = T;
    SR_REQUIRE(capacity_rows >= T, "sr_model_last_hidden: capacity %lld < %d tokens", (long long)capacity_rows, T);
    if (T == 0) return SR_OK;
    SR_TRY(launch_rmsnorm(m->x, (const float*)nullptr,
                       (const int*)nullptr, (const bf16_t*)nullptr, m->norm_w, (bf16_t*)nullptr, d_out, T, m->cfg.hidden_size, m->cfg.rms_norm_eps, s));
    return SR_OK;
}

extern "C" int sr_lora_merge(float* d_W, const float* d_A, const float* d_B, int64_t out_features, int64_t in_features,
                             int32_t r, float scale, sr_stream stream) {
    SR_REQUIRE(d_W && d_A && d_B && out_features > 0 && in_features > 0 && r > 0, "sr_lora_merge: bad argument");
    SR_REQUIRE(out_features < 65536 * 32, "sr_lora_merge: out_features too large");
    hipLaunchKernelGGL(lora_merge_kernel, dim3((unsigned)ceil_div64(in_features, 256), (unsigned)out_features), dim3(256), 0,
                       (hipStream_t)stream, d_W, d_A, d_B, out_features, in_features, r, scale);
    SR_CHECK_LAUNCH();
    return SR_OK;
}

extern "C" int sr_sparse_compact(const float* d_reps, int64_t B, int64_t V, int64_t* d_row_ptr, int32_t* d_cols, float* d_vals,
                                 int64_t capacity, int64_t* h_nnz, sr_stream stream) {
    SR_REQUIRE(d_reps && d_row_ptr && h_nnz && B >= 0 && V > 0, "sr_sparse_compact: bad argument");
    hipStream_t s = (hipStream_t)stream;
    if (B == 0) { *h_nnz = 0; return SR_OK; }
    int64_t* d_cnt = nullptr;
    SR_CHECK_HIP(hipMalloc((void**)&d_cnt, (size_t)B * 8));
    hipLaunchKernelGGL(nnz_count_kernel, dim3((unsigned)B), dim3(256), 0, s, d_reps, V, d_cnt);
    hipLaunchKernelGGL(nnz_scan_kernel, dim3(1), dim3(64), 0, s, d_cnt, B, d_row_ptr);
    int64_t total = 0;
    hipError_t e = hipMemcpyAsync(&total, d_row_ptr + B, 8, hipMemcpyDeviceToHost, s);
    if (e == hipSuccess) e = hipStreamSynchronize(s);
    (void)hipFree(d_cnt);
    SR_CHECK_HIP(e);
    *h_nnz = total;
    if (total > capacity || (total > 0 && (!d_cols || !d_vals))) {
        sr_set_error("sr_sparse_compact: %lld non-zeros, capacity %lld", (long long)total, (long long)capacity);
        return SR_ERR_NOMEM;
    }
    if (total > 0) {
        hipLaunchKernelGGL(nnz_fill_kernel, dim3((unsigned)B), dim3(256), 0, s, d_reps, V, d_row_ptr, d_cols, d_vals, capacity);
        SR_CHECK_LAUNCH();
    }
    return SR_OK;
}
```

scaling_retriever_amd/csrc/gemm_bf16.hip:

```cpp
#include "kernels.h"
#include <math.h>
#include <stdlib.h>
#include <string.h>
#include <type_traits>

typedef __bf16 mfma_bf16x8 __attribute__((ext_vector_type(8)));
typedef _Float16 mfma_f16x8 __attribute__((ext_vector_type(8)));
template <bool F16>
__device__ __forceinline__ f32x4 sr_mma(const mfma_bf16x8& w, const mfma_bf16x8& a, const f32x4& c) {
    if constexpr (F16)
        return __builtin_amdgcn_mfma_f32_16x16x32_f16(__builtin_bit_cast(mfma_f16x8, w), __builtin_bit_cast(mfma_f16x8, a), c, 0, 0, 0);
    else
        return __builtin_amdgcn_mfma_f32_16x16x32_bf16(w, a, c, 0, 0, 0);
}
__device__ __forceinline__ f32x4 sr_rope_lo(const f32x4& x1, const f32x4& x2, const f32x4& c, const f32x4& s) {
#pragma clang fp contract(off)
    f32x4 y;
#pragma unroll
    for (int r = 0; r < 4; ++r) { const float a = x1[r] * c[r], b = x2[r] * s[r]; y[r] = a - b; }
    return y;
}
__device__ __forceinline__ f32x4 sr_rope_hi(const f32x4& x1, const f32x4& x2, const f32x4& c, const f32x4& s) {
#pragma clang fp contract(off)
    f32x4 y;
#pragma unroll
    for (int r = 0; r < 4; ++r) { const float a = x2[r] * c[r], b = x1[r] * s[r]; y[r] = a + b; }
    return y;
}
typedef __attribute__((address_space(3))) void* lds_void_ptr;
typedef __attribute__((address_space(1))) const void* gbl_void_ptr;

#define G_BK 64

typedef int sr_i32x4 __attribute__((ext_vector_type(4)));
template <int EPI, int WAVES_N, int WAVES_M, int NB, int MB, bool PIPE = false, int NS = 2, int KL = 0>
__global__ __launch_bounds__(64 * WAVES_N * WAVES_M, KL == 1 ? 1 : (WAVES_N * WAVES_M) / 4 * (WAVES_N * WAVES_M == 4 ? 2 : 1))
void gemm_bf16_kernel(GemmArgs g) {
    constexpr bool F16 = EPI >= EPI_H_FIRST;
    constexpr int BEPI = !F16 ? EPI : (EPI == EPI_QKV_ROPE_F32_H ? EPI_QKV_ROPE_F32 : (EPI == EPI_RESID_F32_H ? EPI_RESID_F32
                                      : (EPI == EPI_SWIGLU_F32_H ? EPI_SWIGLU_F32 : (EPI == EPI_SWIGLU_SPLIT_H ? EPI_SWIGLU_SPLITH_BASE : EPI_SEGMAX))));
    constexpr int NW = WAVES_N * WAVES_M;
    constexpr int BN = 16 * NB * WAVES_N, BM = 16 * MB * WAVES_M;
    constexpr int W_BYTES = BN * 128, A_BYTES = BM * 128, STAGE_BYTES = W_BYTES + A_BYTES;
    constexpr int W_INSTR = BN / 8 / NW, A_INSTR = BM / 8 / NW;
    static_assert(BN % (8 * NW) == 0 && BM % (8 * NW) == 0, "tile rows must split evenly over the waves");
    extern __shared__ __attribute__((aligned(16))) unsigned char smem[];
    const int tid = threadIdx.x, lane = tid & 63, wave = tid >> 6;
    const int wn = wave / WAVES_M, wm = wave % WAVES_M;
    const int tiles_n = (g.N + BN - 1) / BN, tiles_m = (g.M + BM - 1) / BM;
    const int n_tiles = tiles_n * tiles_m;
    const int K = g.K;
    constexpr bool CROSS_PREFETCH = true;

    const int srow = lane >> 3;
    const int schunk = (lane & 7) ^ (srow & 7);
    const bf16_t* wsrc[W_INSTR];
    const bf16_t* asrc[A_INSTR];
    const int G = (int)gridDim.x;
    const bool swz = g.xcd_order && !g.m_fastest && (G & 7) == 0;
    auto fits = [&](int b) { return tiles_n % b == 0 && (G / 8) % b == 0; };
    const int bnt = !swz ? 1 : (fits(8) ? 8 : fits(4) ? 4 : fits(2) ? 2 : 1);
    const int bmt = !swz ? 1 : (G / 8) / bnt;
    const int slot_limit = !swz ? n_tiles : ((((tiles_m + bmt - 1) / bmt) * bmt * tiles_n + G - 1) / G) * G;
    auto slot_tile = [&](int slot, int& tn, int& tm) -> bool {
        if (!swz) {
            tn = g.m_fastest ? slot / tiles_m : slot % tiles_n;
            tm = g.m_fastest ? slot % tiles_m : slot / tiles_n;
            return true;
        }
        const int r = slot / G, w = slot - r * G;
        const int c = r * G + (w & 7) * (G >> 3) + (w >> 3);
        const int per = bmt * bnt, blk = c / per, w2 = c - blk * per;
        const int nbn = tiles_n / bnt, bm = blk / nbn, bn = blk - bm * nbn;
        tm = bm * bmt + w2 / bnt;
        tn = bn * bnt + w2 % bnt;
        return tm < tiles_m;
    };
    auto next_slot = [&](int slot) {
        for (; slot < slot_limit; slot += G) {
            int tn, tm;
            if (slot_tile(slot, tn, tm)) break;
        }
        return slot < slot_limit ? slot : slot_limit;
    };
    auto set_tile = [&](int tile) {
        int tn_i, tm_i;
        (void)slot_tile(tile, tn_i, tm_i);
        const int tn0 = tn_i * BN, tm0 = tm_i * BM;
#pragma unroll
        for (int i = 0; i < W_INSTR; ++i) {
            int rn = tn0 + (wave * W_INSTR + i) * 8 + srow;
            rn = rn < g.N ? rn : g.N - 1;
            wsrc[i] = g.W + (int64_t)rn * K + schunk * 8;
        }
#pragma unroll
        for (int i = 0; i < A_INSTR; ++i) {
            int rm = tm0 + (wave * A_INSTR + i) * 8 + srow;
            rm = rm < g.M ? rm : g.M - 1;
            asrc[i] = g.A + (int64_t)rm * K + schunk * 8;
        }
    };
    auto stage = [&](int st, int k0) {
        unsigned char* wbase = smem + st * STAGE_BYTES + (wave * W_INSTR) * 1024;
        unsigned char* abase = smem + st * STAGE_BYTES + W_BYTES + (wave * A_INSTR) * 1024;
#pragma unroll
        for (int i = 0; i < W_INSTR; ++i)
            __builtin_amdgcn_global_load_lds((gbl_void_ptr)(wsrc[i] + k0), (lds_void_ptr)(wbase + i * 1024), 16, 0, 0);
#pragma unroll
        for (int i = 0; i < A_INSTR; ++i)
            __builtin_amdgcn_global_load_lds((gbl_void_ptr)(asrc[i] + k0), (lds_void_ptr)(abase + i * 1024), 16, 0, 0);
    };

    f32x4 acc[NB][MB];
    const int frow = lane & 15, fg = lane >> 4;
    const int nk = K / G_BK;
    int tile = next_slot((int)blockIdx.x);
    if (tile >= slot_limit) return;
    const bool stamp = g.stamps != nullptr && tid == 0;
    unsigned long long* stp = g.stamps ? g.stamps + (size_t)blockIdx.x * 64 : nullptr;
    int titer = 0;
    if (stamp) stp[0] = __builtin_amdgcn_s_memrealtime();
    if constexpr (KL == 0) {
        set_tile(tile);
        stage(0, 0);
        if constexpr (PIPE) stage(1, G_BK);
        if constexpr (PIPE && NS > 2) {
#pragma unroll
            for (int st = 2; st < NS; ++st) stage(st, st * G_BK);
        }
        __syncthreads();
    }
    int buf = 0;
    [[maybe_unused]] sr_i32x4 srd_w, srd_a;
    [[maybe_unused]] uint32_t kl_koff = 0, kl_m0 = 0, kl_bw0 = 0, kl_bw1 = 0, kl_ba0 = 0, kl_ba1 = 0;
    [[maybe_unused]] uint32_t kl_voff[8];
    [[maybe_unused]] auto kl_rebase = [&](int t) {
        int tn_i, tm_i;
        (void)slot_tile(t, tn_i, tm_i);
        const int tn0 = tn_i * BN, tm0 = tm_i * BM;
        const uint64_t pw = reinterpret_cast<uint64_t>(g.W + (int64_t)tn0 * K), pa = reinterpret_cast<uint64_t>(g.A + (int64_t)tm0 * K);
        const int rows_w = (g.N - tn0) < BN ? (g.N - tn0) : BN, rows_a = (g.M - tm0) < BM ? (g.M - tm0) : BM;
        srd_w[0] = (int)(uint32_t)pw; srd_w[1] = (int)(uint32_t)(pw >> 32); srd_w[2] = rows_w * K * 2; srd_w[3] = 0x00020000;
        srd_a[0] = (int)(uint32_t)pa; srd_a[1] = (int)(uint32_t)(pa >> 32); srd_a[2] = rows_a * K * 2; srd_a[3] = 0x00020000;
        kl_koff = 0;
    };
    auto load_frags = [&](int st, int kk, mfma_bf16x8 (&wf)[NB], mfma_bf16x8 (&af)[MB]) {
        const unsigned char* wt = smem + st * STAGE_BYTES;
        const unsigned char* at = wt + W_BYTES;
        const int pos = ((4 * kk + fg) ^ (frow & 7)) * 16;
#pragma unroll
        for (int i = 0; i < NB; ++i)
            wf[i] = *reinterpret_cast<const mfma_bf16x8*>(wt + (wn * NB * 16 + i * 16 + frow) * 128 + pos);
#pragma unroll
        for (int j = 0; j < MB; ++j)
            af[j] = *reinterpret_cast<const mfma_bf16x8*>(at + (wm * MB * 16 + j * 16 + frow) * 128 + pos);
    };
    auto mfma_all = [&](const mfma_bf16x8 (&wf)[NB], const mfma_bf16x8 (&af)[MB]) {
#pragma unroll
        for (int i = 0; i < NB; ++i)
#pragma unroll
            for (int j = 0; j < MB; ++j)
                acc[i][j] = sr_mma<F16>(wf[i], af[j], acc[i][j]);
    };
    if constexpr (KL == 1) {
        const uint32_t lds0 = (uint32_t)(size_t)(lds_void_ptr)smem;
        const int wave_s = __builtin_amdgcn_readfirstlane(wave);
#pragma unroll
        for (int i = 0; i < 8; ++i) kl_voff[i] = (uint32_t)(((wave_s * 8 + i) * 8 + srow) * K * 2 + schunk * 16);
        kl_m0 = lds0 + (uint32_t)wave_s * 8192u;
        const uint32_t c0 = (uint32_t)((fg ^ (frow & 7)) * 16), c1 = (uint32_t)(((4 + fg) ^ (frow & 7)) * 16);
        kl_bw0 = lds0 + (uint32_t)((wn * 128 + frow) * 128) + c0;
        kl_bw1 = lds0 + (uint32_t)((wn * 128 + frow) * 128) + c1;
        kl_ba0 = lds0 + (uint32_t)W_BYTES + (uint32_t)((wm * 128 + frow) * 128) + c0;
        kl_ba1 = lds0 + (uint32_t)W_BYTES + (uint32_t)((wm * 128 + frow) * 128) + c1;
    }
    [[maybe_unused]] bool kl_first = true;
    for (; tile < slot_limit;) {
    int tn_i, tm_i;
    (void)slot_tile(tile, tn_i, tm_i);
    const int n0 = tn_i * BN, m0 = tm_i * BM;
    const int tile_next = next_slot(tile + G);
    const bool has_next = tile_next < slot_limit;
#pragma unroll
    for (int i = 0; i < NB; ++i)
#pragma unroll
        for (int j = 0; j < MB; ++j) acc[i][j] = f32x4{0.f, 0.f, 0.f, 0.f};
    int sj[MB];
    if constexpr (BEPI == EPI_SEGMAX) {
#pragma unroll
        for (int j = 0; j < MB; ++j) {
            const int m = m0 + wm * MB * 16 + j * 16 + frow;
            sj[j] = m < g.M ? g.seq_of[m] : -1;
        }
    }
    if (stamp && titer < 16) stp[titer * 4 + 1] = __builtin_amdgcn_s_memrealtime();
    if (stamp && titer == 1) stp[62] = __builtin_amdgcn_s_memtime();
    if constexpr (KL == 1) {
        static_assert(PIPE && NS == 2 && NW == 4 && NB == 8 && MB == 8 && WAVES_N == 2, "KL = 1 is the 2 x 2 x (128 x 128) configuration");
        sr_i32x4 w0[8], a0[8], w1[8], a1[8];
#define KL_MMA(C, WF, AF, INV)                                                                                      \
        do {                                                                                                        \
            if constexpr (F16) {                                                                                    \
                if (INV) asm volatile("v_mfma_f32_16x16x32_f16 %0, %1, %2, %0" : "+v"(C) : "v"(WF), "v"(AF)); \
                else asm volatile("v_mfma_f32_16x16x32_f16 %0, %1, %2, %0" : "+a"(C) : "v"(WF), "v"(AF));              \
            } else {                                                                                                \
                if (INV) asm volatile("v_mfma_f32_16x16x32_bf16 %0, %1, %2, %0" : "+v"(C) : "v"(WF), "v"(AF)); \
                else asm volatile("v_mfma_f32_16x16x32_bf16 %0, %1, %2, %0" : "+a"(C) : "v"(WF), "v"(AF));             \
            }                                                                                                       \
        } while (0)
#define KL_DSR(DST, BASE, OFF) asm volatile("ds_read_b128 %0, %1 offset:%2" : "=v"(DST) : "v"(BASE), "n"(OFF))
#define KL_DMA(SRD, VOFF, KOFF, M0B, M0OFF)                                                                         \
        asm volatile("s_add_u32 m0, %3, %4\n\ts_nop 0\n\tbuffer_load_dwordx4 %0, %1, %2 offen lds" ::"v"(VOFF), "s"(SRD), "s"(KOFF), "s"(M0B), "n"(M0OFF) : "memory", "scc", "m0")
#define KL_MMA_N(n, WS, AS) KL_MMA(acc[(n) >> 3][(n) & 7], WS[(n) >> 3], AS[(n) & 7], (((n) >> 3) == 7))
#define KL_DSR_N(r, WS, AS, BW, BA)                                                 \
        do {                                                                         \
            if ((r) < 8) KL_DSR(WS[(r) & 7], BW, ((r) & 7) * 2048);                  \
            else KL_DSR(AS[(r) & 7], BA, ((r) & 7) * 2048);                          \
        } while (0)
#ifndef KL_RD1_EVERY
#define KL_RD1_EVERY 2
#define KL_B1_AT 39
#define KL_DMA_EVERY 3
#define KL_B2_AT 87
#define KL_RD2_EVERY 2
#endif
        static_assert(16 * KL_RD1_EVERY - 1 <= KL_B1_AT && KL_B1_AT + 16 * KL_DMA_EVERY <= KL_B2_AT && KL_B2_AT + 16 * KL_RD2_EVERY <= 127,
                      "k-step schedule");
        auto kstep = [&]() {
            sr_i32x4 sw, sa;
#pragma unroll
            for (int c = 0; c < 4; ++c) {
                sw[c] = __builtin_amdgcn_readfirstlane(srd_w[c]);
                sa[c] = __builtin_amdgcn_readfirstlane(srd_a[c]);
            }
            const uint32_t koff = (uint32_t)__builtin_amdgcn_readfirstlane((int)kl_koff);
            const uint32_t m0b = (uint32_t)__builtin_amdgcn_readfirstlane((int)kl_m0);
#define KL_MMA_G(n)                                        \
            do {                                           \
                if ((n) < 64) KL_MMA_N((n) & 63, w0, a0);  \
                else KL_MMA_N((n) & 63, w1, a1);           \
            } while (0)
#pragma unroll
            for (int r = 0; r < 16; ++r) {
#pragma unroll
                for (int t = 0; t < KL_RD1_EVERY; ++t) KL_MMA_G(r * KL_RD1_EVERY + t);
                KL_DSR_N(r, w1, a1, kl_bw1, kl_ba1);
            }
#pragma unroll
            for (int n = 16 * KL_RD1_EVERY; n <= KL_B1_AT; ++n) KL_MMA_G(n);
            asm volatile("s_waitcnt lgkmcnt(0)\n\ts_barrier" ::: "memory");
#pragma unroll
            for (int r = 0; r < 16; ++r) {
#pragma unroll
                for (int t = 0; t < KL_DMA_EVERY; ++t) KL_MMA_G(KL_B1_AT + 1 + r * KL_DMA_EVERY + t);
                if (r < 8) KL_DMA(sw, kl_voff[r & 7], koff, m0b, (r & 7) * 1024);
                else KL_DMA(sa, kl_voff[r & 7], koff, m0b, W_BYTES + (r & 7) * 1024);
            }
#pragma unroll
            for (int n = KL_B1_AT + 1 + 16 * KL_DMA_EVERY; n <= KL_B2_AT; ++n) KL_MMA_G(n);
            asm volatile("s_waitcnt vmcnt(16)\n\ts_barrier" ::: "memory");
            kl_bw0 ^= 0x10000u; kl_bw1 ^= 0x10000u; kl_ba0 ^= 0x10000u; kl_ba1 ^= 0x10000u;
            kl_m0 ^= 0x10000u;
#pragma unroll
            for (int r = 0; r < 16; ++r) {
#pragma unroll
                for (int t = 0; t < KL_RD2_EVERY; ++t) KL_MMA_G(KL_B2_AT + 1 + r * KL_RD2_EVERY + t);
                KL_DSR_N(r, w0, a0, kl_bw0, kl_ba0);
            }
#pragma unroll
            for (int n = KL_B2_AT + 1 + 16 * KL_RD2_EVERY; n < 128; ++n) KL_MMA_G(n);
            asm volatile("s_waitcnt lgkmcnt(0)" ::: "memory");
        };
        if (kl_first) {
            kl_first = false;
            kl_rebase(tile);
#pragma unroll
            for (int st = 0; st < 2; ++st) {
                sr_i32x4 sw, sa;
#pragma unroll
                for (int c = 0; c < 4; ++c) {
                    sw[c] = __builtin_amdgcn_readfirstlane(srd_w[c]);
                    sa[c] = __builtin_amdgcn_readfirstlane(srd_a[c]);
                }
                const uint32_t koff = (uint32_t)__builtin_amdgcn_readfirstlane((int)kl_koff);
                const uint32_t m0b = (uint32_t)__builtin_amdgcn_readfirstlane((int)kl_m0);
#pragma unroll
                for (int r = 0; r < 8; ++r) KL_DMA(sw, kl_voff[r], koff, m0b, r * 1024);
#pragma unroll
                for (int r = 0; r < 8; ++r) KL_DMA(sa, kl_voff[r], koff, m0b, W_BYTES + r * 1024);
                kl_koff += 128;
                kl_m0 ^= 0x10000u;
            }
            asm volatile("s_waitcnt vmcnt(16)\n\ts_barrier" ::: "memory");
#pragma unroll
            for (int r = 0; r < 16; ++r) KL_DSR_N(r, w0, a0, kl_bw0, kl_ba0);
            asm volatile("s_waitcnt lgkmcnt(0)" ::: "memory");
        }
        for (int kt = 0; kt < nk; ++kt) {
            if (kt + 2 == nk) {
                if (has_next) kl_rebase(tile_next);
                else { srd_w[2] = 0; srd_a[2] = 0; }
            }
            kstep();
            kl_koff += 128;
        }
#undef KL_MMA
#undef KL_DSR
#undef KL_DMA
#undef KL_MMA_N
#undef KL_MMA_G
#undef KL_DSR_N
    } else if constexpr (PIPE && NS > 2) {
        constexpr int HB = NB / 2, PIECES = W_INSTR + A_INSTR;
        mfma_bf16x8 wx[HB], wy[HB], a0[MB], a1[MB];
        auto load_w = [&](int st, int kk, int h, mfma_bf16x8 (&wf)[HB]) {
            const unsigned char* wt = smem + st * STAGE_BYTES;
            const int pos = ((4 * kk + fg) ^ (frow & 7)) * 16;
#pragma unroll
            for (int i = 0; i < HB; ++i)
                wf[i] = *reinterpret_cast<const mfma_bf16x8*>(wt + (wn * NB * 16 + (h * HB + i) * 16 + frow) * 128 + pos);
        };
        auto load_a = [&](int st, int kk, mfma_bf16x8 (&af)[MB]) {
            const unsigned char* at = smem + st * STAGE_BYTES + W_BYTES;
            const int pos = ((4 * kk + fg) ^ (frow & 7)) * 16;
#pragma unroll
            for (int j = 0; j < MB; ++j)
                af[j] = *reinterpret_cast<const mfma_bf16x8*>(at + (wm * MB * 16 + j * 16 + frow) * 128 + pos);
        };
#define SR_MFMA_HALF(H, WF, AF)                                                                              \
        _Pragma("unroll") for (int i = 0; i < HB; ++i)                                                       \
            _Pragma("unroll") for (int j = 0; j < MB; ++j)                                                   \
                acc[(H) * HB + i][j] = sr_mma<F16>(WF[i], AF[j], acc[(H) * HB + i][j]);
        load_w(buf, 0, 0, wx);
        load_a(buf, 0, a0);
        int kt = 0;
#define SR_SGB2(MASK, N, ID) __builtin_amdgcn_sched_group_barrier(MASK, N, ID)
        constexpr int PH = HB * MB;
        constexpr int R0 = HB + MB < PH ? HB + MB : PH, R1 = HB < PH ? HB : PH;
        for (; kt + NS < nk; ++kt) {
            const int nxt = buf + 1 == NS ? 0 : buf + 1;
            load_w(buf, 0, 1, wy);
            load_a(buf, 1, a1);
            SR_MFMA_HALF(0, wx, a0)
#pragma unroll
            for (int i = 0; i < R0; ++i) { SR_SGB2(0x008, 1, 0); SR_SGB2(0x100, 1, 0); }
            if constexpr (PH > R0) SR_SGB2(0x008, PH - R0, 0);
            __builtin_amdgcn_sched_barrier(0);
            load_w(buf, 1, 0, wx);
            SR_MFMA_HALF(1, wy, a0)
#pragma unroll
            for (int i = 0; i < R1; ++i) { SR_SGB2(0x008, 1, 1); SR_SGB2(0x100, 1, 1); }
            if constexpr (PH > R1) SR_SGB2(0x008, PH - R1, 1);
            __builtin_amdgcn_sched_barrier(0);
            load_w(buf, 1, 1, wy);
            SR_MFMA_HALF(0, wx, a1)
#pragma unroll
            for (int i = 0; i < R1; ++i) { SR_SGB2(0x008, 1, 2); SR_SGB2(0x100, 1, 2); }
            if constexpr (PH > R1) SR_SGB2(0x008, PH - R1, 2);
            __builtin_amdgcn_sched_barrier(0);
            asm volatile("s_waitcnt vmcnt(%0) lgkmcnt(0)\n\ts_barrier" ::"n"((NS - 2) * PIECES) : "memory");
            load_w(nxt, 0, 0, wx);
            load_a(nxt, 0, a0);
            stage(buf, (kt + NS) * G_BK);
            SR_MFMA_HALF(1, wy, a1)
#pragma unroll
            for (int i = 0; i < R0; ++i) { SR_SGB2(0x008, 1, 3); SR_SGB2(0x100, 1, 3); }
            __builtin_amdgcn_sched_barrier(0);
            buf = nxt;
        }
#undef SR_SGB2
        for (; kt < nk; ++kt) {
            const int nxt = buf + 1 == NS ? 0 : buf + 1;
            load_w(buf, 0, 1, wy);
            load_a(buf, 1, a1);
            SR_MFMA_HALF(0, wx, a0)
            load_w(buf, 1, 0, wx);
            SR_MFMA_HALF(1, wy, a0)
            load_w(buf, 1, 1, wy);
            SR_MFMA_HALF(0, wx, a1)
            asm volatile("s_waitcnt vmcnt(0) lgkmcnt(0)\n\ts_barrier" ::: "memory");
            if (kt + 1 < nk) {
                load_w(nxt, 0, 0, wx);
                load_a(nxt, 0, a0);
            }
            SR_MFMA_HALF(1, wy, a1)
            buf = nxt;
        }
#undef SR_MFMA_HALF
    } else if constexpr (PIPE) {
        constexpr int HB = NB / 2;
        mfma_bf16x8 wx[HB], wy[HB], a0[MB], a1[MB];
        auto load_w = [&](int st, int kk, int h, mfma_bf16x8 (&wf)[HB]) {
            const unsigned char* wt = smem + st * STAGE_BYTES;
            const int pos = ((4 * kk + fg) ^ (frow & 7)) * 16;
#pragma unroll
            for (int i = 0; i < HB; ++i)
                wf[i] = *reinterpret_cast<const mfma_bf16x8*>(wt + (wn * NB * 16 + (h * HB + i) * 16 + frow) * 128 + pos);
        };
        auto load_a = [&](int st, int kk, mfma_bf16x8 (&af)[MB]) {
            const unsigned char* at = smem + st * STAGE_BYTES + W_BYTES;
            const int pos = ((4 * kk + fg) ^ (frow & 7)) * 16;
#pragma unroll
            for (int j = 0; j < MB; ++j)
                af[j] = *reinterpret_cast<const mfma_bf16x8*>(at + (wm * MB * 16 + j * 16 + frow) * 128 + pos);
        };
#define SR_MFMA_HALF(H, WF, AF)                                                                              \
        _Pragma("unroll") for (int i = 0; i < HB; ++i)                                                       \
            _Pragma("unroll") for (int j = 0; j < MB; ++j)                                                   \
                acc[(H) * HB + i][j] = sr_mma<F16>(WF[i], AF[j], acc[(H) * HB + i][j]);
        load_w(buf, 0, 0, wx);
        load_a(buf, 0, a0);
        int kt = 0;
#define SR_SGB(MASK, N, ID) __builtin_amdgcn_sched_group_barrier(MASK, N, ID)
        for (; kt + 2 < nk; ++kt) {
            load_w(buf, 0, 1, wy);
            load_a(buf, 1, a1);
            SR_MFMA_HALF(0, wx, a0)
#pragma unroll
            for (int i = 0; i < HB + MB; ++i) { SR_SGB(0x008, 1, 0); SR_SGB(0x100, 1, 0); }
            SR_SGB(0x008, HB * MB - HB - MB, 0);
            __builtin_amdgcn_sched_barrier(0);
            load_w(buf, 1, 0, wx);
            SR_MFMA_HALF(1, wy, a0)
#pragma unroll
            for (int i = 0; i < HB; ++i) { SR_SGB(0x008, 1, 1); SR_SGB(0x100, 1, 1); }
            SR_SGB(0x008, HB * MB - HB, 1);
            __builtin_amdgcn_sched_barrier(0);
            load_w(buf, 1, 1, wy);
            SR_MFMA_HALF(0, wx, a1)
#pragma unroll
            for (int i = 0; i < HB; ++i) { SR_SGB(0x008, 1, 2); SR_SGB(0x100, 1, 2); }
            SR_SGB(0x008, HB * MB - HB, 2);
            __builtin_amdgcn_sched_barrier(0);
            asm volatile("s_waitcnt vmcnt(0)" ::: "memory");
            __syncthreads();
            load_w(buf ^ 1, 0, 0, wx);
            load_a(buf ^ 1, 0, a0);
            stage(buf, (kt + 2) * G_BK);
            SR_MFMA_HALF(1, wy, a1)
#pragma unroll
            for (int i = 0; i < HB + MB; ++i) { SR_SGB(0x008, 1, 3); SR_SGB(0x100, 1, 3); }
#pragma unroll
            for (int i = 0; i < W_INSTR + A_INSTR; ++i) { SR_SGB(0x008, 1, 3); SR_SGB(0x010, 1, 3); }
            __builtin_amdgcn_sched_barrier(0);
            buf ^= 1;
        }
#undef SR_SGB
        for (; kt < nk; ++kt) {
            load_w(buf, 0, 1, wy);
            SR_MFMA_HALF(0, wx, a0)
            load_w(buf, 1, 0, wx);
            load_a(buf, 1, a1);
            SR_MFMA_HALF(1, wy, a0)
            load_w(buf, 1, 1, wy);
            SR_MFMA_HALF(0, wx, a1)
            asm volatile("s_waitcnt vmcnt(0)" ::: "memory");
            __syncthreads();
            if (kt + 2 < nk) {
                stage(buf, (kt + 2) * G_BK);
            } else if (has_next) {
                if (kt + 2 == nk) set_tile(tile_next);
                stage(buf, (kt + 2 - nk) * G_BK);
            }
            if (kt + 1 < nk) {
                load_w(buf ^ 1, 0, 0, wx);
                load_a(buf ^ 1, 0, a0);
            }
            SR_MFMA_HALF(1, wy, a1)
            buf ^= 1;
        }
#undef SR_MFMA_HALF
    } else {
    for (int kt = 0; kt < nk; ++kt) {
        if (kt + 1 < nk) {
            stage(buf ^ 1, (kt + 1) * G_BK);
        } else if (CROSS_PREFETCH && has_next) {
            set_tile(tile_next);
            stage(buf ^ 1, 0);
        }
        mfma_bf16x8 wf[NB], af[MB];
#pragma unroll
        for (int kk = 0; kk < 2; ++kk) {
            load_frags(buf, kk, wf, af);
            mfma_all(wf, af);
        }
        __syncthreads();
        buf ^= 1;
    }
    }

    if (stamp && titer < 16) stp[titer * 4 + 2] = __builtin_amdgcn_s_memrealtime();
    if (stamp && titer == 1) stp[63] = __builtin_amdgcn_s_memtime();
    if constexpr (F16) {
        float sa[MB];
#pragma unroll
        for (int j = 0; j < MB; ++j) {
            const int m = m0 + wm * MB * 16 + j * 16 + frow;
            sa[j] = m < g.M ? g.a_scale[m] : 0.f;
        }
#pragma unroll
        for (int i = 0; i < NB; ++i) {
            const int n = n0 + wn * NB * 16 + i * 16 + fg * 4;
            f32x4 sw = {0.f, 0.f, 0.f, 0.f};
            if (n < g.N) sw = *reinterpret_cast<const f32x4*>(g.w_scale + n);
#pragma unroll
            for (int j = 0; j < MB; ++j)
#pragma unroll
                for (int r = 0; r < 4; ++r) acc[i][j][r] *= sa[j] * sw[r];
        }
    }
#ifdef KL_NO_STAGING
    constexpr bool KL_STAGED = false;
#else
    constexpr bool KL_STAGED = KL == 1 && (BEPI == EPI_STORE_BF16 || BEPI == EPI_SWIGLU || BEPI == EPI_QKV_ROPE);
#endif
    [[maybe_unused]] int frow_e = frow, fg_e = fg, lane_e = lane;
    if constexpr (KL == 1) asm volatile("" : "+v"(frow_e), "+v"(fg_e), "+v"(lane_e));
    if constexpr (KL_STAGED) {
        constexpr int OUT_F = BEPI == EPI_SWIGLU ? 64 : 128;
        constexpr int ROWB = OUT_F * 2, NP = ROWB / 16;
        unsigned char* const stg0 = smem + 2 * STAGE_BYTES + wave * 8192;
        const int ldc = BEPI == EPI_SWIGLU ? (g.N >> 1) : g.N;
        const int nb = (BEPI == EPI_SWIGLU ? (n0 >> 1) : n0) + wn * OUT_F;
        unsigned char* stg = stg0;
        auto put = [&](int f_local, const f32x4& v) {
            bf16x4 o;
#pragma unroll
            for (int r = 0; r < 4; ++r) o[r] = (short)f32_to_bf16(v[r]);
            *reinterpret_cast<bf16x4*>(stg + frow_e * ROWB + (((f_local >> 3) ^ (frow_e & (NP - 1))) << 4) + ((f_local & 4) << 1)) = o;
        };
#pragma unroll
        for (int j = 0; j < MB; ++j) {
            const int mrow = m0 + wm * MB * 16 + j * 16;
            stg = stg0 + (j & 1) * 4096;
            if constexpr (BEPI == EPI_STORE_BF16) {
#pragma unroll
                for (int i = 0; i < NB; ++i) put(i * 16 + fg_e * 4, acc[i][j]);
            } else if constexpr (BEPI == EPI_SWIGLU) {
#pragma unroll
                for (int i = 0; i < NB; i += 2) {
                    const f32x4 gt = acc[i][j], up = acc[i + 1][j];
                    f32x4 y;
#pragma unroll
                    for (int r = 0; r < 4; ++r) y[r] = (gt[r] * __builtin_amdgcn_rcpf(1.f + __expf(-gt[r]))) * up[r];
                    put((i >> 1) * 16 + fg_e * 4, y);
                }
            } else if constexpr (BEPI == EPI_QKV_ROPE) {
                const int mtok = mrow + frow_e;
                const int pos_t = mtok < g.M ? g.pos[mtok] : 0;
                const int hd2 = g.head_dim >> 1;
                const float* ct = g.rope_cos + (int64_t)pos_t * hd2 + fg_e * 4;
                const float* st = g.rope_sin + (int64_t)pos_t * hd2 + fg_e * 4;
                if (n0 + wn * NB * 16 < g.n_rope) {
                    if (g.head_dim == 64) {
#pragma unroll
                        for (int i = 0; i < NB; ++i) {
                            if ((i & 2) != 0) continue;
                            const f32x4 c = *reinterpret_cast<const f32x4*>(ct + (i & 1) * 16), sn = *reinterpret_cast<const f32x4*>(st + (i & 1) * 16);
                            const f32x4 x1 = acc[i][j], x2 = acc[i + 2][j];
                            put(i * 16 + fg_e * 4, sr_rope_lo(x1, x2, c, sn));
                            put((i + 2) * 16 + fg_e * 4, sr_rope_hi(x1, x2, c, sn));
                        }
                    } else {
#pragma unroll
                        for (int i = 0; i < NB / 2; ++i) {
                            const f32x4 c = *reinterpret_cast<const f32x4*>(ct + i * 16), sn = *reinterpret_cast<const f32x4*>(st + i * 16);
                            const f32x4 x1 = acc[i][j], x2 = acc[i + 4][j];
                            put(i * 16 + fg_e * 4, sr_rope_lo(x1, x2, c, sn));
                            put((i + 4) * 16 + fg_e * 4, sr_rope_hi(x1, x2, c, sn));
                        }
                    }
                } else {
#pragma unroll
                    for (int i = 0; i < NB; ++i) put(i * 16 + fg_e * 4, acc[i][j]);
                }
            }
            constexpr int LPR = OUT_F * 2 / 16;
            constexpr int RPI = 64 / LPR;
#pragma unroll
            for (int it = 0; it < 16 / RPI; ++it) {
                const int tok = it * RPI + lane_e / LPR, pc = lane_e % LPR;
                const sr_i32x4 v = *reinterpret_cast<const sr_i32x4*>(stg + tok * ROWB + ((pc ^ (tok & (NP - 1))) << 4));
                const int m = mrow + tok, n = nb + pc * 8;
                if (m < g.M && n < ldc) *reinterpret_cast<sr_i32x4*>(reinterpret_cast<bf16_t*>(g.C) + (int64_t)m * ldc + n) = v;
            }
            __builtin_amdgcn_sched_barrier(0);
        }
    } else if constexpr (KL == 1 && (BEPI == EPI_STORE_F32 || BEPI == EPI_RESID_F32)) {
        unsigned char* const stg0 = smem + 2 * STAGE_BYTES + wave * 8192;
#pragma unroll
        for (int j = 0; j < MB; ++j) {
            const int mrow = m0 + wm * MB * 16 + j * 16;
#pragma unroll
            for (int h = 0; h < 2; ++h) {
                unsigned char* stg = stg0 + h * 4096;
#pragma unroll
                for (int ii = 0; ii < 4; ++ii) {
                    const int i = 4 * h + ii;
                    f32x4 y = acc[i][j];
                    *reinterpret_cast<f32x4*>(stg + frow_e * 256 + (((ii * 4 + fg_e) ^ frow_e) << 4)) = y;
                }
#pragma unroll
                for (int it = 0; it < 4; ++it) {
                    const int tok = it * 4 + (lane_e >> 4), pc = lane_e & 15;
                    f32x4 v = *reinterpret_cast<const f32x4*>(stg + tok * 256 + ((pc ^ tok) << 4));
                    const int m = mrow + tok, n = n0 + wn * NB * 16 + h * 64 + pc * 4;
                    if (m < g.M && n < g.N) {
                        f32x4* dst = reinterpret_cast<f32x4*>(reinterpret_cast<float*>(g.C) + (int64_t)m * g.N + n);
                        if constexpr (BEPI == EPI_RESID_F32) {
                            f32x4 x = *dst;
                            x += v;
                            v = x;
                        }
                        *dst = v;
                    }
                }
                __builtin_amdgcn_sched_barrier(0);
            }
        }
    } else if constexpr (KL == 1 && BEPI == EPI_SWIGLU_SPLITH_BASE) {
        unsigned char* const stg0 = smem + 2 * STAGE_BYTES + wave * 8192;
        const int half_n = g.N >> 1;
        const int64_t ldc = 3 * (int64_t)half_n;
        const int nb = (n0 >> 1) + wn * 64;
#pragma unroll
        for (int j = 0; j < MB; ++j) {
            const int mrow = m0 + wm * MB * 16 + j * 16;
            unsigned char* stg = stg0 + (j & 1) * 4096;
            const float osc = (mrow + frow_e) < g.M ? g.out_scale[mrow + frow_e] : 0.f;
#pragma unroll
            for (int i = 0; i < NB; i += 2) {
                const f32x4 gt = acc[i][j], up = acc[i + 1][j];
                bf16x4 p0, p1;
#pragma unroll
                for (int r = 0; r < 4; ++r) {
                    const float y = (gt[r] / (1.f + expf(-gt[r]))) * up[r];
                    unsigned short f0, f1;
                    split_f16x2(y * osc, f0, f1);
                    p0[r] = (short)f0; p1[r] = (short)f1;
                }
                const int sl = (i >> 1) * 4 + fg_e;
                *reinterpret_cast<bf16x4*>(stg + frow_e * 256 + ((((sl >> 1)) ^ (frow_e & 7)) << 4) + ((sl & 1) << 3)) = p1;
                *reinterpret_cast<bf16x4*>(stg + frow_e * 256 + 128 + ((((sl >> 1)) ^ (frow_e & 7)) << 4) + ((sl & 1) << 3)) = p0;
            }
#pragma unroll
            for (int it = 0; it < 4; ++it) {
                const int tok = it * 4 + (lane_e >> 4), pl = (lane_e >> 3) & 1, pc = lane_e & 7;
                const sr_i32x4 v = *reinterpret_cast<const sr_i32x4*>(stg + tok * 256 + pl * 128 + ((pc ^ (tok & 7)) << 4));
                const int m = mrow + tok, n = nb + pc * 8;
                if (m < g.M && n < half_n) {
                    bf16_t* crow = reinterpret_cast<bf16_t*>(g.C) + (int64_t)m * ldc + n;
                    if (pl == 0) {
                        *reinterpret_cast<sr_i32x4*>(crow) = v;
                    } else {
                        *reinterpret_cast<sr_i32x4*>(crow + half_n) = v;
                        *reinterpret_cast<sr_i32x4*>(crow + 2 * half_n) = v;
                    }
                }
            }
            __builtin_amdgcn_sched_barrier(0);
        }
    } else if constexpr (BEPI == EPI_STORE_BF16 || BEPI == EPI_STORE_F32 || BEPI == EPI_RESID_F32) {
#pragma unroll
        for (int j = 0; j < MB; ++j) {
            const int m = m0 + wm * MB * 16 + j * 16 + frow;
            if (m >= g.M) continue;
#pragma unroll
            for (int i = 0; i < NB; ++i) {
                const int n = n0 + wn * NB * 16 + i * 16 + fg * 4;
                if (n >= g.N) continue;
                const f32x4 v = acc[i][j];
                if constexpr (BEPI == EPI_STORE_BF16) {
                    bf16x4 o;
                    o[0] = (short)f32_to_bf16(v[0]);
                    o[1] = (short)f32_to_bf16(v[1]);
                    o[2] = (short)f32_to_bf16(v[2]);
                    o[3] = (short)f32_to_bf16(v[3]);
#ifdef KL_DIAG_NOSTORE
                    if (o[0] == 12345 && o[1] == 23456 && lane == 77)
#endif
                    *reinterpret_cast<bf16x4*>(reinterpret_cast<bf16_t*>(g.C) + (int64_t)m * g.N + n) = o;
                } else if constexpr (BEPI == EPI_STORE_F32) {
                    *reinterpret_cast<f32x4*>(reinterpret_cast<float*>(g.C) + (int64_t)m * g.N + n) = v;
                } else {
                    f32x4* p = reinterpret_cast<f32x4*>(reinterpret_cast<float*>(g.C) + (int64_t)m * g.N + n);
                    f32x4 x = *p;
                    x += v;
                    *p = x;
                }
            }
        }
    } else if constexpr (BEPI == EPI_QKV_ROPE || BEPI == EPI_QKV_ROPE_F32) {
        constexpr bool F32OUT = BEPI == EPI_QKV_ROPE_F32;
        const int hd = g.head_dim, hb = hd / 32;
        auto put = [&](int64_t off, const f32x4& v) {
            if constexpr (F32OUT) {
                *reinterpret_cast<f32x4*>(reinterpret_cast<float*>(g.C) + off) = v;
            } else {
                bf16x4 o;
#pragma unroll
                for (int r = 0; r < 4; ++r) o[r] = (short)f32_to_bf16(v[r]);
                *reinterpret_cast<bf16x4*>(reinterpret_cast<bf16_t*>(g.C) + off) = o;
            }
        };
#pragma unroll
        for (int j = 0; j < MB; ++j) {
            const int m = m0 + wm * MB * 16 + j * 16 + frow;
            if (m >= g.M) continue;
            const int p = g.pos[m];
            const int64_t crow = (int64_t)m * g.N;
#pragma unroll
            for (int i = 0; i < NB; ++i) {
                const int n = n0 + wn * NB * 16 + i * 16 + fg * 4;
                if (n >= g.N) continue;
                if (n < g.n_rope) {
                    const int d = n % hd;
                    if (d >= hd / 2) continue;
                    f32x4 x1 = acc[i][j], x2;
                    if (hb == 2) x2 = acc[(i + 2) % NB][j]; else x2 = acc[(i + 4) % NB][j];
                    const f32x4 c = *reinterpret_cast<const f32x4*>(g.rope_cos + (int64_t)p * (hd / 2) + d);
                    const f32x4 sn = *reinterpret_cast<const f32x4*>(g.rope_sin + (int64_t)p * (hd / 2) + d);
                    put(crow + n, sr_rope_lo(x1, x2, c, sn));
                    put(crow + n + hd / 2, sr_rope_hi(x1, x2, c, sn));
                } else {
                    put(crow + n, acc[i][j]);
                }
            }
        }
    } else if constexpr (BEPI == EPI_SWIGLU) {
        const int half_n = g.N >> 1;
#pragma unroll
        for (int j = 0; j < MB; ++j) {
            const int m = m0 + wm * MB * 16 + j * 16 + frow;
            if (m >= g.M) continue;
#pragma unroll
            for (int i = 0; i < NB; i += 2) {
                const int n = (n0 >> 1) + wn * NB * 8 + (i >> 1) * 16 + fg * 4;
                if (n >= half_n) continue;
                const f32x4 gt = acc[i][j], up = acc[i + 1][j];
                bf16x4 o;
#pragma unroll
                for (int r = 0; r < 4; ++r) {
                    const float sg = gt[r] * __builtin_amdgcn_rcpf(1.f + __expf(-gt[r]));
                    o[r] = (short)f32_to_bf16(sg * up[r]);
                }
                *reinterpret_cast<bf16x4*>(reinterpret_cast<bf16_t*>(g.C) + (int64_t)m * half_n + n) = o;
            }
        }
    } else if constexpr (BEPI == EPI_SWIGLU_F32) {
        const int half_n = g.N >> 1;
#pragma unroll
        for (int j = 0; j < MB; ++j) {
            const int m = m0 + wm * MB * 16 + j * 16 + frow;
            if (m >= g.M) continue;
#pragma unroll
            for (int i = 0; i < NB; i += 2) {
                const int n = (n0 >> 1) + wn * NB * 8 + (i >> 1) * 16 + fg * 4;
                if (n >= half_n) continue;
                const f32x4 gt = acc[i][j], up = acc[i + 1][j];
                f32x4 y;
#pragma unroll
                for (int r = 0; r < 4; ++r) y[r] = (gt[r] / (1.f + expf(-gt[r]))) * up[r];
                *reinterpret_cast<f32x4*>(reinterpret_cast<float*>(g.C) + (int64_t)m * half_n + n) = y;
            }
        }
    } else if constexpr (BEPI == EPI_SWIGLU_SPLITH_BASE) {
        const int half_n = g.N >> 1;
        const int64_t ldc = 3 * (int64_t)half_n;
#pragma unroll
        for (int j = 0; j < MB; ++j) {
            const int m = m0 + wm * MB * 16 + j * 16 + frow;
            if (m >= g.M) continue;
            const float osc = g.out_scale[m];
#pragma unroll
            for (int i = 0; i < NB; i += 2) {
                const int n = (n0 >> 1) + wn * NB * 8 + (i >> 1) * 16 + fg * 4;
                if (n >= half_n) continue;
                const f32x4 gt = acc[i][j], up = acc[i + 1][j];
                bf16x4 p0, p1;
#pragma unroll
                for (int r = 0; r < 4; ++r) {
                    const float y = (gt[r] / (1.f + expf(-gt[r]))) * up[r];
                    unsigned short f0, f1;
                    split_f16x2(y * osc, f0, f1);
                    p0[r] = (short)f0; p1[r] = (short)f1;
                }
                bf16_t* crow = reinterpret_cast<bf16_t*>(g.C) + (int64_t)m * ldc + n;
                *reinterpret_cast<bf16x4*>(crow) = p1;
                *reinterpret_cast<bf16x4*>(crow + half_n) = p0;
                *reinterpret_cast<bf16x4*>(crow + 2 * half_n) = p0;
            }
        }
    } else if constexpr (BEPI == EPI_SWIGLU_SPLIT) {
        const int half_n = g.N >> 1;
        const int nsg = g.out_map.n_seg;
        const int64_t ldc = (int64_t)nsg * half_n;
#pragma unroll
        for (int j = 0; j < MB; ++j) {
            const int m = m0 + wm * MB * 16 + j * 16 + frow;
            if (m >= g.M) continue;
#pragma unroll
            for (int i = 0; i < NB; i += 2) {
                const int n = (n0 >> 1) + wn * NB * 8 + (i >> 1) * 16 + fg * 4;
                if (n >= half_n) continue;
                const f32x4 gt = acc[i][j], up = acc[i + 1][j];
                bf16x4 pl0, pl1, pl2;
#pragma unroll
                for (int r = 0; r < 4; ++r) {
                    const float y = (gt[r] / (1.f + expf(-gt[r]))) * up[r];
                    unsigned short a0, a1, a2;
                    split_bf16x3(y, a0, a1, a2);
                    pl0[r] = (short)a0; pl1[r] = (short)a1; pl2[r] = (short)a2;
                }
                bf16_t* crow = reinterpret_cast<bf16_t*>(g.C) + (int64_t)m * ldc + n;
                for (int sg = 0; sg < nsg; ++sg) {
                    const int pi = g.out_map.plane[sg];
                    *reinterpret_cast<bf16x4*>(crow + (int64_t)sg * half_n) = pi == 0 ? pl0 : (pi == 1 ? pl1 : pl2);
                }
            }
        }
    } else {
        int lo = 0x7fffffff, hi = -1;
#pragma unroll
        for (int j = 0; j < MB; ++j) {
            if (sj[j] >= 0) {
                lo = sj[j] < lo ? sj[j] : lo;
                hi = sj[j] > hi ? sj[j] : hi;
            }
        }
#pragma unroll
        for (int off = 32; off > 0; off >>= 1) {
            const int l2 = __shfl_xor(lo, off), h2 = __shfl_xor(hi, off);
            lo = l2 < lo ? l2 : lo;
            hi = h2 > hi ? h2 : hi;
        }
        float* out = reinterpret_cast<float*>(g.C);
        auto row_max = [](float v) {
            v = fmaxf(v, __int_as_float(__builtin_amdgcn_update_dpp(0, __float_as_int(v), 0xB1, 0xF, 0xF, true)));
            v = fmaxf(v, __int_as_float(__builtin_amdgcn_update_dpp(0, __float_as_int(v), 0x4E, 0xF, 0xF, true)));
            v = fmaxf(v, __int_as_float(__builtin_amdgcn_update_dpp(0, __float_as_int(v), 0x141, 0xF, 0xF, true)));
            v = fmaxf(v, __int_as_float(__builtin_amdgcn_update_dpp(0, __float_as_int(v), 0x140, 0xF, 0xF, true)));
            return v;
        };
        constexpr int PER_LANE = NB * 4 / 16;
        static_assert(NB * 4 % 16 == 0, "");
        for (int q = lo; q <= hi; ++q) {
            float mine[PER_LANE];
#pragma unroll
            for (int i = 0; i < NB; ++i)
#pragma unroll
                for (int r = 0; r < 4; ++r) {
                    float v = 0.f;
#pragma unroll
                    for (int j = 0; j < MB; ++j) v = (sj[j] == q) ? fmaxf(v, acc[i][j][r]) : v;
                    v = row_max(v);
                    const int idx = i * 4 + r;
                    if ((idx & 15) == frow) mine[idx >> 4] = v;
                }
#pragma unroll
            for (int k = 0; k < PER_LANE; ++k) {
                const int idx = frow + 16 * k;
                const int n = n0 + wn * NB * 16 + (idx >> 2) * 16 + fg * 4 + (idx & 3);
                if (mine[k] > 0.f && n < g.N)
                    atomicMax(reinterpret_cast<int*>(out + (int64_t)q * g.out_ld + n), __float_as_int(mine[k]));
            }
        }
    }
    if (stamp && titer < 16) {
        __builtin_amdgcn_s_waitcnt(0);
        stp[titer * 4 + 3] = __builtin_amdgcn_s_memrealtime();
        if (titer + 1 < 16) stp[(titer + 1) * 4] = stp[titer * 4 + 3];
    }
    ++titer;
    if constexpr (PIPE && NS > 2) {
        if (has_next) {
            __syncthreads();
            set_tile(tile_next);
#pragma unroll
            for (int st = 0; st < NS; ++st) stage(st, st * G_BK);
            __syncthreads();
            buf = 0;
        }
    }
    tile = tile_next;
    }
}

template <int EPI, int WAVES_N, int WAVES_M, int NB, int MB, bool PIPE = false, int NS = 2, int KL = 0>
static int launch_cfg(const GemmArgs& g_in, hipStream_t s) {
    constexpr int BN = 16 * NB * WAVES_N, BM = 16 * MB * WAVES_M;
    constexpr size_t lds = NS * (size_t)(BN + BM) * 128 + (KL == 1 ? 4 * 8192 : 0);
    static DeviceOnce attr_once;
    bool* attr_slot = attr_once.pending();
    if (attr_slot) {
        SR_CHECK_HIP(hipFuncSetAttribute(reinterpret_cast<const void*>(&gemm_bf16_kernel<EPI, WAVES_N, WAVES_M, NB, MB, PIPE, NS, KL>),
                                         hipFuncAttributeMaxDynamicSharedMemorySize, (int)lds));
        *attr_slot = true;
    }
    GemmArgs g = g_in;
    g.m_fastest = ((int64_t)g.N * g.K * 2 > (128ll << 20) && (int64_t)g.N > 4 * (int64_t)g.M) ? 1 : 0;
    if (const char* e = sr_dev_getenv("SR_GEMM_MFAST")) g.m_fastest = atoi(e);
    g.xcd_order = 1;
    if (const char* e = sr_dev_getenv("SR_GEMM_XCD")) g.xcd_order = atoi(e);
    int64_t tiles = ceil_div64(g.N, BN) * ceil_div64(g.M, BM);
    const char* env = sr_dev_getenv("SR_GEMM_PERSIST");
    constexpr int64_t by_lds = (160 * 1024) / lds;
    const int64_t slots = 256 * (WAVES_N * WAVES_M == 4 ? (by_lds > 3 ? 3 : by_lds) : (WAVES_N * WAVES_M == 1 ? (by_lds > 8 ? 8 : by_lds) : 1));
    if (!(env && *env == '0') && tiles > slots) tiles = slots;
    hipLaunchKernelGGL((gemm_bf16_kernel<EPI, WAVES_N, WAVES_M, NB, MB, PIPE, NS, KL>), dim3((unsigned)tiles), dim3(64 * WAVES_N * WAVES_M), lds,
                       s, g);
    SR_CHECK_LAUNCH();
    return SR_OK;
}

static double plan_cost(int64_t big_tiles, int64_t small_tiles) {
    double c = (double)ceil_div64(big_tiles, 256);
    if (small_tiles > 0) {
        const int64_t full = small_tiles / 512, rest = small_tiles % 512;
        c += 0.61 * (double)full + (rest == 0 ? 0.0 : (rest <= 256 ? 0.45 : 0.61));
        c += 0.03;
    }
    return c;
}

static int plan_big_rows(const GemmArgs& g, bool small_allowed) {
    const char* env = sr_dev_getenv("SR_GEMM_TILE");
    if (env && *env) {
        if (atoi(env) == 256) return g.M;
        if (atoi(env) == 128) return 0;
        if (!strncmp(env, "split:", 6)) {
            const int rows = atoi(env + 6) / 256 * 256;
            return rows < g.M ? rows : g.M;
        }
    }
    if (!small_allowed) return g.M;
    const int64_t tn256 = ceil_div64(g.N, 256), tn128 = ceil_div64(g.N, 128);
    int best_rows = 0;
    double best = plan_cost(0, tn128 * ceil_div64(g.M, 128));
    if (tn256 * ceil_div64(g.M, 256) >= 128) {
        const double all_big = plan_cost(tn256 * ceil_div64(g.M, 256), 0);
        if (all_big <= best) { best = all_big; best_rows = g.M; }
        for (int rows = 256; rows < g.M; rows += 256) {
            const double c = plan_cost(tn256 * (rows / 256), tn128 * ceil_div64(g.M - rows, 128));
            if (c < best - 1e-9) { best = c; best_rows = rows; }
        }
    }
    return best_rows;
}

template <int EPI>
static int launch_big(const GemmArgs& g, hipStream_t s) {
    if constexpr (EPI == EPI_STORE_BF16 || EPI == EPI_SWIGLU || EPI == EPI_QKV_ROPE) {
        const char* big = sr_dev_getenv("SR_GEMM_BIG");
        if (big && big[0] == 's' && big[1] == '3' && g.K / G_BK >= 4) {
            if constexpr (EPI == EPI_QKV_ROPE) {
                if (g.head_dim == 64) return launch_cfg<EPI, 2, 4, 8, 2, true, 3>(g, s);
            } else {
                return launch_cfg<EPI, 2, 4, 8, 2, true, 3>(g, s);
            }
        }
    }
    const char* env = sr_dev_getenv("SR_GEMM_PIPE");
    {
        const char* big = sr_dev_getenv("SR_GEMM_BIG");
        const bool want8 = big && big[0] == '8', want4 = big && big[0] == '4';
        constexpr bool STAGED_BF16 = EPI == EPI_STORE_BF16 || EPI == EPI_SWIGLU || EPI == EPI_STORE_F32 || EPI == EPI_RESID_F32 || EPI == EPI_QKV_ROPE;
        constexpr bool STAGED_F16 = EPI == EPI_RESID_F32_H || EPI == EPI_SWIGLU_SPLIT_H;
        if constexpr (STAGED_BF16 || STAGED_F16) {
            const bool rope_ok = EPI != EPI_QKV_ROPE || g.n_rope % 128 == 0;
            if (g.K / G_BK >= 4 && (int64_t)g.K * 512 < (1ll << 31) && !want8 && (STAGED_BF16 || want4) && rope_ok && !(env && *env == '0'))
                return launch_cfg<EPI, 2, 2, 8, 8, true, 2, 1>(g, s);
        }
    }
    if (g.K / G_BK >= 4 && !(env && *env == '0')) return launch_cfg<EPI, 2, 4, 8, 4, true>(g, s);
    return launch_cfg<EPI, 2, 4, 8, 4, false>(g, s);
}

static bool env_off(const char* name) {
    const char* e = sr_dev_getenv(name);
    return e && *e == '0';
}

template <int EPI>
static int launch_small(const GemmArgs& g, hipStream_t s) {
    const bool pipe = g.K / G_BK >= 4 && !env_off("SR_GEMM_PIPE");
    if constexpr (EPI == EPI_QKV_ROPE || EPI == EPI_QKV_ROPE_F32 || EPI == EPI_QKV_ROPE_F32_H) {
        if (g.head_dim == 128) return launch_cfg<EPI, 1, 4, 8, 2>(g, s);
    }
    if constexpr (EPI != EPI_QKV_ROPE && EPI != EPI_QKV_ROPE_F32 && EPI != EPI_QKV_ROPE_F32_H) {
        const int64_t t128 = ceil_div64(g.N, 128) * ceil_div64(g.M, 128);
        if (t128 < 384 && g.M > 64 && !env_off("SR_GEMM_TAIL64"))
            return pipe ? (env_off("SR_GEMM_NS3") ? launch_cfg<EPI, 2, 2, 4, 2, true>(g, s) : launch_cfg<EPI, 2, 2, 4, 2, true, 3>(g, s))
                        : launch_cfg<EPI, 2, 2, 4, 2>(g, s);
    }
    return pipe ? launch_cfg<EPI, 2, 2, 4, 4, true>(g, s) : launch_cfg<EPI, 2, 2, 4, 4>(g, s);
}

template <int EPI>
static GemmArgs rows_from(const GemmArgs& g, int row0) {
    GemmArgs t = g;
    t.A = g.A + (int64_t)row0 * g.K;
    t.M = g.M - row0;
    const int64_t ldc = (EPI == EPI_SWIGLU || EPI == EPI_SWIGLU_F32 || EPI == EPI_SWIGLU_F32_H)
                            ? g.N / 2 : (EPI == EPI_SWIGLU_SPLIT ? (int64_t)g.out_map.n_seg * (g.N / 2) : (EPI == EPI_SWIGLU_SPLIT_H ? 3 * (int64_t)(g.N / 2) : g.N));
    const int64_t esz = (EPI == EPI_STORE_F32 || EPI == EPI_RESID_F32 || EPI == EPI_QKV_ROPE_F32 || EPI == EPI_SWIGLU_F32 ||
                         (EPI >= EPI_H_FIRST && EPI != EPI_SWIGLU_SPLIT_H)) ? 4 : 2;
    if constexpr (EPI != EPI_SEGMAX && EPI != EPI_SEGMAX_H) t.C = reinterpret_cast<unsigned char*>(g.C) + (int64_t)row0 * ldc * esz;
    if (g.a_scale) t.a_scale = g.a_scale + row0;
    if (g.out_scale) t.out_scale = g.out_scale + row0;
    if (g.seq_of) t.seq_of = g.seq_of + row0;
    if (g.pos) t.pos = g.pos + row0;
    t.stamps = nullptr;
    return t;
}

static int skinny_max_rows() {
    const char* e = sr_dev_getenv("SR_GEMM_SKINNY");
    if (!e || !*e) return 64;
    return atoi(e);
}

template <int EPI>
static int launch_one(const GemmArgs& g, hipStream_t s) {
    if constexpr (EPI == EPI_QKV_ROPE || EPI == EPI_QKV_ROPE_F32 || EPI == EPI_QKV_ROPE_F32_H) {
        SR_REQUIRE(g.head_dim == 64 || g.head_dim == 128, "gemm(qkv+rope): head_dim %d not supported", g.head_dim);
        SR_REQUIRE(g.pos && g.rope_cos && g.rope_sin && g.n_rope % g.head_dim == 0 && g.n_rope <= g.N && g.N % g.head_dim == 0,
                   "gemm(qkv+rope): bad rope arguments");
    }
    if (g.M <= skinny_max_rows() && g.K / G_BK >= 4) {
        if (g.M > 32) {
            if constexpr (EPI == EPI_QKV_ROPE || EPI == EPI_QKV_ROPE_F32 || EPI == EPI_QKV_ROPE_F32_H) {
                if (g.head_dim == 128) return launch_cfg<EPI, 1, 1, 8, 4, true, 3>(g, s);
            }
            return launch_cfg<EPI, 1, 1, 4, 4, true, 4>(g, s);
        }
        if (g.M > 16) {
            if constexpr (EPI == EPI_QKV_ROPE || EPI == EPI_QKV_ROPE_F32 || EPI == EPI_QKV_ROPE_F32_H) {
                if (g.head_dim == 128) return launch_cfg<EPI, 1, 1, 8, 2, true, 4>(g, s);
            }
            return launch_cfg<EPI, 1, 1, 4, 2, true, 4>(g, s);
        }
        if constexpr (EPI == EPI_QKV_ROPE || EPI == EPI_QKV_ROPE_F32 || EPI == EPI_QKV_ROPE_F32_H) {
            if (g.head_dim == 128) return launch_cfg<EPI, 1, 1, 8, 1, true, 4>(g, s);
        }
        return launch_cfg<EPI, 1, 1, 4, 1, true, 4>(g, s);
    }
    {
        const int big_rows = plan_big_rows(g, true);
        if (big_rows >= g.M) return launch_big<EPI>(g, s);
        if (big_rows <= 0) return launch_small<EPI>(g, s);
        GemmArgs head = g;
        head.M = big_rows;
        SR_TRY(launch_big<EPI>(head, s));
        return launch_small<EPI>(rows_from<EPI>(g, big_rows), s);
    }
}

int launch_gemm_bf16(GemmEpilogue epi, const GemmArgs& g, hipStream_t s) {
    SR_REQUIRE(g.M >= 0 && g.N > 0 && g.K > 0, "gemm: bad shape M=%d N=%d K=%d", g.M, g.N, g.K);
    if (g.M == 0) return SR_OK;
    SR_REQUIRE(g.K % G_BK == 0, "gemm: K=%d must be a multiple of %d", g.K, G_BK);
    const bool swiglu = epi == EPI_SWIGLU || epi == EPI_SWIGLU_SPLIT || epi == EPI_SWIGLU_F32 || epi == EPI_SWIGLU_F32_H || epi == EPI_SWIGLU_SPLIT_H;
    SR_REQUIRE(epi != EPI_SWIGLU_SPLIT_H || g.out_scale, "gemm(swiglu split, fp16 planes): missing output row scales");
    SR_REQUIRE(g.N % 16 == 0 && (!swiglu || g.N % 32 == 0), "gemm: N=%d must be a multiple of 16 (32 for SwiGLU)", g.N);
    SR_REQUIRE(epi < EPI_H_FIRST || (g.a_scale && g.w_scale), "gemm(fp16 planes): missing row scales");
    SR_REQUIRE(epi != EPI_SWIGLU_SPLIT || (g.out_map.n_seg >= 1 && g.out_map.n_seg <= SR_MAX_SEG), "gemm(swiglu split): bad segment map");
    switch (epi) {
        case EPI_STORE_BF16: return launch_one<EPI_STORE_BF16>(g, s);
#ifndef SR_GEMM_VARIANT_BUILD
        case EPI_RESID_F32: return launch_one<EPI_RESID_F32>(g, s);
        case EPI_SWIGLU: return launch_one<EPI_SWIGLU>(g, s);
        case EPI_SEGMAX: return launch_one<EPI_SEGMAX>(g, s);
        case EPI_STORE_F32: return launch_one<EPI_STORE_F32>(g, s);
        case EPI_QKV_ROPE: return launch_one<EPI_QKV_ROPE>(g, s);
        case EPI_QKV_ROPE_F32: return launch_one<EPI_QKV_ROPE_F32>(g, s);
        case EPI_SWIGLU_SPLIT: return launch_one<EPI_SWIGLU_SPLIT>(g, s);
        case EPI_SWIGLU_F32: return launch_one<EPI_SWIGLU_F32>(g, s);
        case EPI_QKV_ROPE_F32_H: return launch_one<EPI_QKV_ROPE_F32_H>(g, s);
        case EPI_RESID_F32_H: return launch_one<EPI_RESID_F32_H>(g, s);
        case EPI_SWIGLU_F32_H: return launch_one<EPI_SWIGLU_F32_H>(g, s);
        case EPI_SEGMAX_H: return launch_one<EPI_SEGMAX_H>(g, s);
        case EPI_SWIGLU_SPLIT_H: return launch_one<EPI_SWIGLU_SPLIT_H>(g, s);
#endif
        default: break;
    }
    sr_set_error("gemm: unknown epilogue %d", (int)epi);
    return SR_ERR_INVALID;
}
```

scaling_retriever_amd/csrc/kernels.h:

```cpp
#pragma once
#include "common.h"

typedef unsigned short bf16_t;

enum GemmEpilogue {
    EPI_STORE_BF16 = 0,
    EPI_RESID_F32 = 1,
    EPI_SWIGLU = 2,
    EPI_SEGMAX = 3,
    EPI_STORE_F32 = 4,
    EPI_QKV_ROPE = 5,
    EPI_QKV_ROPE_F32 = 6,
    EPI_SWIGLU_SPLIT = 7,
    EPI_SWIGLU_F32 = 8,
    EPI_H_FIRST = 9,
    EPI_QKV_ROPE_F32_H = 9, EPI_RESID_F32_H = 10, EPI_SWIGLU_F32_H = 11, EPI_SEGMAX_H = 12,
    EPI_SWIGLU_SPLIT_H = 13,
    EPI_SWIGLU_SPLITH_BASE = 14,
};

#define SR_MAX_SEG 6
struct SplitMap {
    int n_seg;
    int plane[SR_MAX_SEG];
};
#define SR_FP32_PLANES_F16 16
inline SplitMap split_map_a(int planes) {
    if (planes == 3) return SplitMap{6, {2, 0, 1, 1, 0, 0}};
    return SplitMap{3, {1, 0, 0, 0, 0, 0}};
}
inline SplitMap split_map_w(int planes) {
    if (planes == 3) return SplitMap{6, {0, 2, 1, 0, 1, 0}};
    return SplitMap{3, {0, 1, 0, 0, 0, 0}};
}

struct GemmArgs {
    const bf16_t* A;
    const bf16_t* W;
    int M, N, K;
    void* C;
    const int* seq_of;
    int64_t out_ld;
    const int* pos;
    const float* rope_cos;
    const float* rope_sin;
    int n_rope;
    int head_dim;
    unsigned long long* stamps;
    const float* a_scale;
    const float* w_scale;
    const float* out_scale;
    SplitMap out_map;
    int m_fastest;
    int xcd_order;
};

int launch_gemm_bf16(GemmEpilogue epi, const GemmArgs& g, hipStream_t s);

struct AttnArgs {
    const bf16_t* qkv;
    bf16_t* out;
    const int* cu_seqlens;
    const int* pos;
    const unsigned char* key_valid;
    const float* rope_cos;
    const float* rope_sin;
    int B, nh, nkv, hd;
    float scale;
    int apply_rope;
    int max_seqlen;
};
int launch_attention(const AttnArgs& a, hipStream_t s);

struct AttnF32Args {
    const float* qkv;
    float* out_f32;
    bf16_t* out;
    const int* cu_seqlens;
    const unsigned char* key_valid;
    int B, nh, nkv, hd;
    float scale;
    int max_seqlen;
    SplitMap out_map;
    int only_le = 0, only_gt = 0;
};
int launch_attention_f32(const AttnF32Args& a, hipStream_t s);
```

scaling_retriever_amd/modeling/llm_encoder.py:

```python
import ctypes
import json
import os
from types import SimpleNamespace

import numpy as np
import torch

from .. import _lib

TARGET_MODULES = ["q_proj", "v_proj", "o_proj", "k_proj", "down_proj", "up_proj", "gate_proj"]


class LlamaConfigLite(SimpleNamespace):

    @classmethod
    def from_dict(cls, d):
        d = dict(d)
        nh = d["num_attention_heads"]
        d.setdefault("num_key_value_heads", nh)
        if d.get("num_key_value_heads") is None:
            d["num_key_value_heads"] = nh
        if not d.get("head_dim"):
            d["head_dim"] = d["hidden_size"] // nh
        d.setdefault("rms_norm_eps", 1e-6)
        d.setdefault("rope_theta", 10000.0)
        d.setdefault("tie_word_embeddings", False)
        d.setdefault("rope_scaling", None)
        return cls(**d)

    def to_dict(self):
        return dict(self.__dict__)


def _canonical_name(k):
    if k.startswith("lm_head."):
        return k
    return k if k.startswith("model.") else "model." + k


def _read_checkpoint(path):
    from safetensors import safe_open
    idx = os.path.join(path, "model.safetensors.index.json")
    files = []
    if os.path.exists(idx):
        with open(idx) as f:
            files = sorted(set(json.load(f)["weight_map"].values()))
    elif os.path.exists(os.path.join(path, "model.safetensors")):
        files = ["model.safetensors"]
    out = {}
    if files:
        for fn in files:
            with safe_open(os.path.join(path, fn), framework="pt", device="cpu") as f:
                for k in f.keys():
                    out[_canonical_name(k)] = f.get_tensor(k)
        return out
    binf = os.path.join(path, "pytorch_model.bin")
    if os.path.exists(binf):
        sd = torch.load(binf, map_location="cpu", weights_only=True)
        return {_canonical_name(k): v for k, v in sd.items()}
    raise FileNotFoundError(f"no model.safetensors / pytorch_model.bin under {path}")


def _resolve_dir(name_or_path, access_token=None):
    if os.path.isdir(name_or_path):
        return name_or_path
    try:
        from huggingface_hub import snapshot_download
        return snapshot_download(name_or_path, token=access_token)
    except Exception as e:
        raise FileNotFoundError(f"'{name_or_path}' is not a local directory and could not be fetched from the hub: {e}")


def _load_adapter_state(lora_name_or_path):
    from safetensors.torch import load_file
    if os.path.isdir(lora_name_or_path):
        st = os.path.join(lora_name_or_path, "adapter_model.safetensors")
        if os.path.exists(st):
            return load_file(st)
        bn = os.path.join(lora_name_or_path, "adapter_model.bin")
        if os.path.exists(bn):
            return torch.load(bn, map_location="cpu", weights_only=True)
        raise FileNotFoundError(f"no adapter_model.safetensors / adapter_model.bin under {lora_name_or_path}")
    from huggingface_hub import hf_hub_download
    return torch.load(hf_hub_download(lora_name_or_path, "adapter_model.bin"), map_location="cpu", weights_only=True)


def _adapter_target(key):
    k = key
    if k.startswith("base_model.model."):
        k = k[len("base_model.model."):]
    for tag, ab in ((".lora_A.", "A"), (".lora_B.", "B")):
        if tag in k:
            mod = k.split(tag)[0]
            return _canonical_name(mod + ".weight"), ab
    return None, None


class HipLlamaBackbone(torch.nn.Module):

    def __init__(self, config, weights, has_lm_head, lora=None, max_batch_tokens=32768, max_batch_seqs=1024,
                 precision="auto", fp32_planes=None):
        super().__init__()
        if precision not in ("auto", "bf16", "fp32"):
            raise ValueError(f"precision must be 'auto', 'bf16' or 'fp32', got {precision!r}")
        self.precision = precision
        if fp32_planes is None:
            fp32_planes = int(os.environ.get("SR_FP32_PLANES", "16"))
        if fp32_planes not in (0, 2, 3, 16):
            raise ValueError(f"fp32_planes must be 0, 2, 3 or 16, got {fp32_planes}")
        self.fp32_planes = int(fp32_planes)
        self.config = config if isinstance(config, LlamaConfigLite) else LlamaConfigLite.from_dict(config)
        self._weights = weights
        self._lora = lora
        self.has_lm_head = bool(has_lm_head)
        self.max_batch_tokens = int(max_batch_tokens)
        self.max_batch_seqs = int(max_batch_seqs)
        self._h = None
        self._device = None
        self._lib = None

    def _c_config(self):
        c = self.config
        rs = getattr(c, "rope_scaling", None) or getattr(c, "rope_parameters", None)
        llama3 = 0
        fac = lo = hi = 1.0
        old = 0
        if rs:
            rtype = rs.get("rope_type", rs.get("type"))
            if rtype == "llama3":
                llama3 = 1
                fac, lo, hi = float(rs["factor"]), float(rs["low_freq_factor"]), float(rs["high_freq_factor"])
                old = int(rs["original_max_position_embeddings"])
            elif rtype not in (None, "default"):
                raise NotImplementedError(f"rope scaling '{rtype}' is not supported")
        theta = float(rs["rope_theta"]) if (rs and "rope_theta" in rs) else float(c.rope_theta)
        return _lib.SrModelConfig(
            vocab_size=c.vocab_size, hidden_size=c.hidden_size, intermediate_size=c.intermediate_size,
            num_layers=c.num_hidden_layers, num_heads=c.num_attention_heads, num_kv_heads=c.num_key_value_heads,
            head_dim=c.head_dim, rms_norm_eps=float(c.rms_norm_eps), rope_theta=theta, rope_llama3=llama3,
            rope_factor=fac, rope_low_freq_factor=lo, rope_high_freq_factor=hi, rope_original_max_pos=old,
            tie_word_embeddings=int(bool(c.tie_word_embeddings)), has_lm_head=int(self.has_lm_head),
            max_batch_tokens=self.max_batch_tokens, max_batch_seqs=self.max_batch_seqs, fp32_planes=self.fp32_planes)

    def build_engine(self, device):
        _lib.require_gpu()
        device = torch.device(device if not isinstance(device, int) else f"cuda:{device}")
        if device.type != "cuda":
            raise _lib.SrHipError("the encoder runs on ROCm devices only (there is no CPU fallback)")
        if device.index is None:
            device = torch.device("cuda", torch.cuda.current_device())
        if self._h is not None:
            if device == self._device:
                return self
            raise _lib.SrHipError("model already lives on %s; moving it to %s is not supported" % (self._device, device))
        if self._weights is None:
            raise _lib.SrHipError("checkpoint tensors were released; reload the model")
        lib = _lib.load()
        with torch.cuda.device(device):
            cfg = self._c_config()
            h = ctypes.c_void_p()
            _lib.check(lib.sr_model_create(ctypes.byref(h), ctypes.byref(cfg)), "sr_model_create")
            try:
                stream = _lib.stream_ptr()
                for name, t in self._weights.items():
                    if name == "lm_head.weight" and not self.has_lm_head:
                        continue
                    if "rotary_emb" in name:
                        continue
                    if isinstance(t, np.ndarray):
                        t = torch.from_numpy(t)
                    lora_hit = self._lora is not None and name in self._lora["A"]
                    if lora_hit:
                        t = t.to(device=device, dtype=torch.float32).contiguous()
                        A = self._lora["A"][name].to(device=device, dtype=torch.float32).contiguous()
                        Bm = self._lora["B"][name].to(device=device, dtype=torch.float32).contiguous()
                        r = A.shape[0]
                        if A.shape[1] != t.shape[1] or Bm.shape != (t.shape[0], r):
                            raise ValueError(f"LoRA shapes do not match {name}: W{tuple(t.shape)} A{tuple(A.shape)} B{tuple(Bm.shape)}")
                        _lib.check(lib.sr_lora_merge(t.data_ptr(), A.data_ptr(), Bm.data_ptr(), t.shape[0], t.shape[1], r,
                                                     float(self._lora["scale"]), stream), "sr_lora_merge")
                    elif t.dtype == torch.bfloat16:
                        t = t.to(device=device).contiguous()
                    else:
                        t = t.to(device=device, dtype=torch.float32).contiguous()
                    dt = _lib.SR_DTYPE_BF16 if t.dtype == torch.bfloat16 else _lib.SR_DTYPE_F32
                    rows, cols = (t.shape[0], t.shape[1]) if t.dim() == 2 else (t.shape[0], 1)
                    _lib.check(lib.sr_model_set_weight(h, name.encode(), t.data_ptr(), dt, rows, cols, stream),
                               f"sr_model_set_weight({name})")
                    torch.cuda.current_stream().synchronize()
                    del t
                _lib.check(lib.sr_model_finalize(h), "sr_model_finalize")
            except Exception:
                lib.sr_model_destroy(h)
                raise
        self._h, self._device, self._lib = h, device, lib
        self._weights = None
        self._lora = None
        return self

    @property
    def device(self):
        return self._device if self._device is not None else torch.device("cpu")

    def to(self, *args, **kwargs):
        device = kwargs.get("device", args[0] if args else None)
        if isinstance(device, (str, int, torch.device)):
            d = torch.device(device if not isinstance(device, int) else f"cuda:{device}")
            if d.type == "cuda":
                self.build_engine(d)
        return self

    def cuda(self, device=None):
        return self.to(torch.device("cuda", torch.cuda.current_device() if device is None else device))

    def _ensure_engine(self, like):
        if self._h is None:
            if like is not None and like.is_cuda:
                self.build_engine(like.device)
            elif torch.cuda.is_available():
                self.build_engine(torch.device("cuda", torch.cuda.current_device()))
            else:
                raise _lib.SrHipError("no ROCm device: LlamaBi* encode runs on MI355X only (no CPU fallback)")

    def resolve_precision(self):
        if self.precision != "auto":
            return self.precision
        if torch.is_autocast_enabled("cuda"):
            dt = torch.get_autocast_dtype("cuda")
            if dt != torch.bfloat16:
                raise NotImplementedError(f"autocast dtype {dt} is not supported (the reference uses torch.bfloat16)")
            return "bf16"
        return "fp32"

    def _encode(self, input_ids, attention_mask, sparse):
        if input_ids.dim() != 2 or attention_mask.shape != input_ids.shape:
            raise ValueError("input_ids and attention_mask must both be [batch, length]")
        prec = self.resolve_precision()
        if prec == "fp32" and self.fp32_planes == 0:
            raise _lib.SrHipError("fp32-regime encode requested (no torch.autocast(bf16) active) but the model was built "
                                  "with fp32_planes=0; wrap the call in torch.autocast('cuda', dtype=torch.bfloat16) or "
                                  "build the model with fp32_planes=3")
        self._ensure_engine(input_ids)
        src_device = input_ids.device
        ids = input_ids.to(device=self._device, dtype=torch.int64).contiguous()
        mask = attention_mask.to(device=self._device, dtype=torch.int64).contiguous()
        B, L = ids.shape
        if sparse == "both":
            out_s = torch.empty((B, self.config.vocab_size), dtype=torch.float32, device=self._device)
            out_d = torch.empty((B, self.config.hidden_size), dtype=torch.float32, device=self._device)
            with torch.cuda.device(self._device):
                stream = _lib.stream_ptr()
                for b0, b1 in self._call_ranges(mask, False):
                    _lib.check(self._lib.sr_encode_both(self._h, ids[b0:b1].data_ptr(), mask[b0:b1].data_ptr(), b1 - b0, L,
                                                        int(prec == "fp32"), out_s[b0:b1].data_ptr(), out_d[b0:b1].data_ptr(),
                                                        stream), "sr_encode_both")
            return (out_s, out_d) if src_device == self._device else (out_s.to(src_device), out_d.to(src_device))
        width = self.config.vocab_size if sparse else self.config.hidden_size
        out = torch.empty((B, width), dtype=torch.float32, device=self._device)
        what = ("sr_encode_sparse" if sparse else "sr_encode_dense") + ("_fp32" if prec == "fp32" else "")
        fn = getattr(self._lib, what)
        with torch.cuda.device(self._device):
            stream = _lib.stream_ptr()
            for b0, b1 in self._call_ranges(mask, sparse):
                _lib.check(fn(self._h, ids[b0:b1].data_ptr(), mask[b0:b1].data_ptr(), b1 - b0, L,
                              out[b0:b1].data_ptr(), stream), what)
        return out if src_device == self._device else out.to(src_device)

    def _encode_many(self, batches, sparse):
        if not batches:
            raise ValueError("encode_batches needs at least one batch")
        for ids, mask in batches:
            if ids.dim() != 2 or mask.shape != ids.shape:
                raise ValueError("input_ids and attention_mask must both be [batch, length]")
        prec = self.resolve_precision()
        if prec == "fp32" and self.fp32_planes == 0:
            raise _lib.SrHipError("fp32-regime encode requested (no torch.autocast(bf16) active) but the model was built with fp32_planes=0")
        self._ensure_engine(batches[0][0])
        src_device = batches[0][0].device
        B = sum(int(i.shape[0]) for i, _ in batches)
        L = max(int(i.shape[1]) for i, _ in batches)
        dev = self._device
        ids = torch.zeros((B, L), dtype=torch.int64, device=dev)
        mask = torch.zeros((B, L), dtype=torch.int64, device=dev)
        shift = torch.empty((B,), dtype=torch.int32, device=dev)
        b0 = 0
        for bi, bm in batches:
            n, l = int(bi.shape[0]), int(bi.shape[1])
            ids[b0:b0 + n, L - l:] = bi.to(device=dev, dtype=torch.int64)
            mask[b0:b0 + n, L - l:] = bm.to(device=dev, dtype=torch.int64)
            shift[b0:b0 + n] = L - l
            b0 += n
        mode = 2 if sparse == "both" else (1 if sparse else 0)
        out_s = torch.empty((B, self.config.vocab_size), dtype=torch.float32, device=dev) if mode != 0 else None
        out_d = torch.empty((B, self.config.hidden_size), dtype=torch.float32, device=dev) if mode != 1 else None
        with torch.cuda.device(dev):
            stream = _lib.stream_ptr()
            for r0, r1 in self._call_ranges(mask, sparse is True):
                _lib.check(self._lib.sr_encode_rows(self._h, ids[r0:r1].data_ptr(), mask[r0:r1].data_ptr(), r1 - r0, L,
                                                    shift[r0:r1].data_ptr(), mode, int(prec == "fp32"),
                                                    out_s[r0:r1].data_ptr() if out_s is not None else None,
                                                    out_d[r0:r1].data_ptr() if out_d is not None else None, stream), "sr_encode_rows")
        outs = tuple(o if src_device == dev else o.to(src_device) for o in (out_s, out_d) if o is not None)
        return outs if mode == 2 else outs[0]

    def _call_ranges(self, mask, sparse):
        B, L = mask.shape
        if B <= self.max_batch_seqs and B * L <= self.max_batch_tokens:
            return [(0, B)]
        m = mask != 0
        n = m.sum(1)
        pos = torch.arange(L, device=mask.device)
        first = torch.where(m, pos, L).min(1).values
        if sparse:
            last = torch.where(m, pos, -1).max(1).values
            span = torch.where(n > 0, last + 1 - first, 0)
        else:
            span = torch.where(n > 0, L - torch.minimum(first, L - n), 0)
        span = span.cpu().tolist()
        out, b0, tok = [], 0, 0
        for b, t in enumerate(span):
            if t > self.max_batch_tokens:
                raise ValueError(f"row {b} packs to {t} tokens, the workspace holds {self.max_batch_tokens} (raise max_batch_tokens)")
            if b > b0 and (tok + t > self.max_batch_tokens or b - b0 >= self.max_batch_seqs):
                out.append((b0, b))
                b0, tok = b, 0
            tok += t
        out.append((b0, B))
        return out

    def last_hidden_state_packed(self):
        n = ctypes.c_int64(0)
        buf = torch.empty((self.max_batch_tokens + 128, self.config.hidden_size), dtype=torch.float32, device=self._device)
        with torch.cuda.device(self._device):
            _lib.check(self._lib.sr_model_last_hidden(self._h, buf.data_ptr(), buf.shape[0], ctypes.byref(n),
                                                      _lib.stream_ptr()), "sr_model_last_hidden")
        return buf[:n.value]

    def __del__(self):
        try:
            if self._h is not None and self._lib is not None:
                self._lib.sr_model_destroy(self._h)
                self._h = None
        except Exception:
            pass


class LLM2Retriever(torch.nn.Module):
    TRANSFORMER_CLS = None
    TARGET_MODULES = TARGET_MODULES
    HAS_LM_HEAD = False
    _tied_weights_keys = None

    def __init__(self, base_model):
        super().__init__()
        self.base_model = base_model

    def encode(self, **inputs):
        raise NotImplementedError

    def doc_encode(self, **inputs):
        return self.encode(**inputs)

    def query_encode(self, **inputs):
        return self.encode(**inputs)

    _HEAD = None

    def encode_batches(self, batches):
        return self.base_model._encode_many([(b["input_ids"], b["attention_mask"]) for b in batches], self._HEAD)

    def forward(self, **inputs):
        raise NotImplementedError("training losses are out of scope of the MI355X inference path")

    def to(self, *args, **kwargs):
        self.base_model.to(*args, **kwargs)
        return self

    def cuda(self, device=None):
        self.base_model.cuda(device)
        return self

    @classmethod
    def _make(cls, base_model, **kw):
        return cls(base_model, **kw)

    @classmethod
    def _check_adapter_layout(cls, state, lora_config):
        return

    @classmethod
    def _load_impl(cls, model_name_or_path, lora_name_or_path, merge_peft, is_trainable, access_token, **make_kw):
        if is_trainable or not merge_peft:
            raise NotImplementedError("only merged, inference-only adapters are supported on the HIP path")
        lora = None
        if lora_name_or_path is not None:
            state = _load_adapter_state(lora_name_or_path)
            ldir = lora_name_or_path if os.path.isdir(lora_name_or_path) else None
            if ldir is None:
                from huggingface_hub import hf_hub_download
                cfg_path = hf_hub_download(lora_name_or_path, "adapter_config.json")
            else:
                cfg_path = os.path.join(ldir, "adapter_config.json")
            with open(cfg_path) as f:
                lora_config = json.load(f)
            cls._check_adapter_layout(state, lora_config)
            if lora_config.get("use_dora"):
                raise NotImplementedError("DoRA adapters (use_dora) are not supported")
            if lora_config.get("rank_pattern") or lora_config.get("alpha_pattern"):
                raise NotImplementedError("per-module rank_pattern / alpha_pattern are not supported")
            if lora_config.get("bias", "none") not in ("none", None):
                raise NotImplementedError(f"adapter bias='{lora_config['bias']}' is not supported (Llama linears have no bias)")
            r, alpha = int(lora_config["r"]), float(lora_config["lora_alpha"])
            scale = alpha / (r ** 0.5) if lora_config.get("use_rslora") else alpha / r
            A, Bm, extra = {}, {}, {}
            for k, v in state.items():
                name, ab = _adapter_target(k)
                if name is not None:
                    (A if ab == "A" else Bm)[name] = v
                    continue
                kk = k[len("base_model.model."):] if k.startswith("base_model.model.") else k
                if ".original_module." in kk:
                    continue
                for tag in (".modules_to_save.default.", ".modules_to_save."):
                    if tag in kk:
                        kk = kk.replace(tag, ".")
                        break
                if any(t in kk for t in ("lora_embedding_", "lora_magnitude_vector", ".lora_")) or not kk.endswith(".weight"):
                    raise ValueError(f"adapter tensor '{k}' is neither a LoRA A/B pair of a linear nor a full replacement weight; "
                                     "loading would silently drop it")
                extra[_canonical_name(kk)] = v
            if set(A) != set(Bm):
                raise ValueError("adapter has unmatched lora_A / lora_B tensors")
            lora = {"scale": scale, "A": A, "B": Bm, "extra": extra}
        base_dir = _resolve_dir(model_name_or_path, access_token)
        with open(os.path.join(base_dir, "config.json")) as f:
            config = LlamaConfigLite.from_dict(json.load(f))
        weights = _read_checkpoint(base_dir)
        if lora is not None:
            extra = lora.pop("extra")
            unknown = [n for n in extra if n not in weights and not (n == "lm_head.weight" and cls.HAS_LM_HEAD)]
            if unknown:
                raise ValueError(f"adapter replaces tensors absent from the base checkpoint: {unknown[:3]}")
            if "lm_head.weight" in extra and config.tie_word_embeddings:
                config.tie_word_embeddings = False
            weights.update(extra)
            missing = [n for n in lora["A"] if n not in weights]
            if missing:
                raise ValueError(f"adapter targets tensors absent from the base checkpoint: {missing[:3]}")
        if cls.HAS_LM_HEAD and not config.tie_word_embeddings and "lm_head.weight" not in weights:
            raise ValueError("checkpoint has no lm_head.weight and tie_word_embeddings is false")
        backbone = HipLlamaBackbone(config, weights, has_lm_head=cls.HAS_LM_HEAD, lora=lora)
        return cls._make(backbone, **make_kw)

    @classmethod
    def load(cls, model_name_or_path, lora_name_or_path=None, merge_peft=True, is_trainable=False, access_token=None):
        return cls._load_impl(model_name_or_path, lora_name_or_path, merge_peft, is_trainable, access_token)

    @classmethod
    def load_from_lora(cls, lora_name_or_path, merge_peft=True, is_trainable=False, access_token=None):
        if os.path.isdir(lora_name_or_path):
            adapter_config_path = os.path.join(lora_name_or_path, "adapter_config.json")
        else:
            from huggingface_hub import hf_hub_download
            adapter_config_path = hf_hub_download(lora_name_or_path, "adapter_config.json")
        with open(adapter_config_path, "r") as f:
            adapter_config = json.load(f)
        return cls.load(adapter_config["base_model_name_or_path"], lora_name_or_path=lora_name_or_path,
                        merge_peft=merge_peft, is_trainable=is_trainable, access_token=access_token)

    @classmethod
    def from_weights(cls, config, weights, max_batch_tokens=32768, max_batch_seqs=1024, precision="auto", fp32_planes=None,
                     **make_kw):
        weights = {_canonical_name(k): v for k, v in weights.items()}
        backbone = HipLlamaBackbone(config, weights, has_lm_head=cls.HAS_LM_HEAD, max_batch_tokens=max_batch_tokens,
                                    max_batch_seqs=max_batch_seqs, precision=precision, fp32_planes=fp32_planes)
        return cls._make(backbone, **make_kw)

    def save_pretrained(self, save_dir):
        raise NotImplementedError("saving is out of scope of the MI355X inference path")


class DecoderOnlyBiSparse(LLM2Retriever):
    HAS_LM_HEAD = True
    _HEAD = True

    def __init__(self, base_model):
        super().__init__(base_model)
        self.vocab_size = self.base_model.config.vocab_size

    def encode(self, **inputs):
        return self.base_model._encode(inputs["input_ids"], inputs["attention_mask"], sparse=True)

    def rerank_forward(self, **inputs):
        query_reps = self.encode(**inputs["tokenized_queries"])
        doc_reps = self.encode(**inputs["tokenized_docs"])
        return (query_reps * doc_reps).sum(dim=-1)


class DecoderOnlyBiDense(LLM2Retriever):
    HAS_LM_HEAD = False
    _HEAD = False

    def __init__(self, base_model, T=0.01):
        super().__init__(base_model)
        self.hidden_size = self.base_model.config.hidden_size
        self.T = T

    def encode(self, **inputs):
        return self.base_model._encode(inputs["input_ids"], inputs["attention_mask"], sparse=False)

    def rerank_forward(self, **inputs):
        query_reps = self.encode(**inputs["tokenized_queries"])
        doc_reps = self.encode(**inputs["tokenized_docs"])
        return (query_reps * doc_reps).sum(dim=-1)

    @classmethod
    def _check_adapter_layout(cls, state, lora_config):
        first = list(state.keys())[0]
        assert "base_model.model.model.layers" not in first
        assert "base_model.model.layers" in first
        am = lora_config.get("auto_mapping") or {}
        assert am.get("base_model_class") == cls.TRANSFORMER_CLS, (am.get("base_model_class"), cls.TRANSFORMER_CLS)

    @classmethod
    def load(cls, model_name_or_path, lora_name_or_path=None, merge_peft=True, is_trainable=False, T=0.01,
             access_token=None):
        return cls._load_impl(model_name_or_path, lora_name_or_path, merge_peft, is_trainable, access_token, T=T)


class LlamaBiSparse(DecoderOnlyBiSparse):
    TRANSFORMER_CLS = "LlamaBiForMNTP"


class DecoderOnlyBiHybrid(DecoderOnlyBiSparse):

    _HEAD = "both"

    def __init__(self, base_model, T=0.01):
        super().__init__(base_model)
        self.hidden_size = self.base_model.config.hidden_size
        self.T = T

    def encode(self, **inputs):
        return self.base_model._encode(inputs["input_ids"], inputs["attention_mask"], sparse="both")

    def rerank_forward(self, **inputs):
        raise NotImplementedError


class LlamaBiHybrid(DecoderOnlyBiHybrid):
    TRANSFORMER_CLS = "LlamaBiForMNTP"


class LlamaBiDense(DecoderOnlyBiDense):
    TRANSFORMER_CLS = "LlamaBiModel"


LlamaBiSparseForNCE = LlamaBiSparse
LlamaBiDenseForNCE = LlamaBiDense
```

Measured before the change: 13610.

## Drop fp16 low plane from GEMMs when weights have no residual bits

While weights are converted to split fp16 planes, a per-matrix flag now records whether any row has a nonzero low fp16 plane. When a matrix has none (for example weights that came from bf16), the activation split, weight packing and GEMM K-dimension shrink from three segments to two, and the SwiGLU epilogue writes two segments instead of three. This removes a third of the MFMA work and activation traffic for such layers while staying exact. It adds per-layer segment bookkeeping and a repacking step at finalize.

```diff
diff --git a/include/sr_hip.h b/include/sr_hip.h
--- a/include/sr_hip.h
+++ b/include/sr_hip.h
@@ -99,6 +99,7 @@
 int sr_model_set_weight(sr_model* m, const char* name, const void* d_ptr, int dtype,
                         int64_t rows, int64_t cols, sr_stream stream);
 int sr_model_finalize(sr_model* m);
+int sr_model_weight_segments(sr_model* m, int32_t* out, int64_t capacity, int64_t* n);
 int sr_encode_dense(sr_model* m, const int64_t* d_input_ids, const int64_t* d_attention_mask,
                     int32_t B, int32_t L, float* d_out, sr_stream stream);
 int sr_encode_sparse(sr_model* m, const int64_t* d_input_ids, const int64_t* d_attention_mask,
diff --git a/scaling_retriever_amd/_lib.py b/scaling_retriever_amd/_lib.py
--- a/scaling_retriever_amd/_lib.py
+++ b/scaling_retriever_amd/_lib.py
@@ -64,6 +64,7 @@
     "sr_model_create": (c_int, [ctypes.POINTER(c_void_p), ctypes.POINTER(SrModelConfig)]),
     "sr_model_set_weight": (c_int, [c_void_p, c_char_p, c_void_p, c_int, c_int64, c_int64, c_void_p]),
     "sr_model_finalize": (c_int, [c_void_p]),
+    "sr_model_weight_segments": (c_int, [c_void_p, ctypes.POINTER(ctypes.c_int32), c_int64, ctypes.POINTER(c_int64)]),
     "sr_encode_dense": (c_int, [c_void_p, c_void_p, c_void_p, c_int32, c_int32, c_void_p, c_void_p]),
     "sr_encode_sparse": (c_int, [c_void_p, c_void_p, c_void_p, c_int32, c_int32, c_void_p, c_void_p]),
     "sr_encode_dense_fp32": (c_int, [c_void_p, c_void_p, c_void_p, c_int32, c_int32, c_void_p, c_void_p]),
diff --git a/scaling_retriever_amd/csrc/encoder.hip b/scaling_retriever_amd/csrc/encoder.hip
--- a/scaling_retriever_amd/csrc/encoder.hip
+++ b/scaling_retriever_amd/csrc/encoder.hip
@@ -300,7 +300,7 @@
 
 __global__ __launch_bounds__(256) void convert_rows_split_h_kernel(const void* __restrict__ src, int src_dtype, int64_t rows, int64_t cols,
                                                                    bf16_t* __restrict__ dst, float* __restrict__ w_inv,
-                                                                   int64_t dst_row_base, int interleave) {
+                                                                   int64_t dst_row_base, int interleave, int* __restrict__ lo_nz) {
     __shared__ float red[4];
     const int64_t r = blockIdx.x;
     int64_t dr = r;
@@ -319,10 +319,25 @@
     const float sc = row_scale_pow2(mx);
     if (threadIdx.x == 0) w_inv[dr] = 1.0f / sc;
     bf16_t* drow = dst + dr * cols * 3;
+    bool nz = false;
     for (int64_t c = threadIdx.x; c < cols; c += 256) {
         unsigned short f0, f1;
         split_f16x2(at(c) * sc, f0, f1);
         drow[c] = f0; drow[cols + c] = f1; drow[2 * cols + c] = f0;
+        nz |= (f1 & 0x7fff) != 0;
+    }
+    if (nz) *lo_nz = 1;
+}
+
+__global__ __launch_bounds__(256) void pack_rows_2seg_kernel(const bf16_t* __restrict__ src, bf16_t* __restrict__ dst, int64_t K) {
+    const int64_t r = blockIdx.x;
+    const uint4* s0 = reinterpret_cast<const uint4*>(src + r * 3 * K);
+    uint4* d = reinterpret_cast<uint4*>(dst + r * 2 * K);
+    const int64_t kv = K / 8;
+    for (int64_t i = threadIdx.x; i < kv; i += 256) {
+        const uint4 v = s0[i];
+        d[i] = v;
+        d[kv + i] = v;
     }
 }
 
@@ -330,7 +345,7 @@
                                                            const int* __restrict__ tok_id, const float* __restrict__ w,
                                                            bf16_t* __restrict__ xs, float* __restrict__ a_inv, int T, int K, float eps,
                                                            const float* __restrict__ gu_cmax, float* __restrict__ act_sc,
-                                                           float* __restrict__ act_inv) {
+                                                           float* __restrict__ act_inv, int nseg) {
     const int t = blockIdx.x * 4 + (threadIdx.x >> 6);
     const int lane = threadIdx.x & 63;
     if (t >= T) return;
@@ -367,7 +382,7 @@
         const float osc = row_scale_pow2(s2 * *gu_cmax * 1.02f);
         if (lane == 0) { act_sc[t] = osc; act_inv[t] = 1.0f / osc; }
     }
-    bf16_t* orow = xs + (int64_t)t * K * 3;
+    bf16_t* orow = xs + (int64_t)t * K * nseg;
     for (int i = lane * 4; i < K; i += 256) {
         const f32x4 v = *reinterpret_cast<const f32x4*>(src + i);
         f32x4 g = {1.f, 1.f, 1.f, 1.f};
@@ -381,7 +396,7 @@
         }
         *reinterpret_cast<bf16x4*>(orow + i) = p1;
         *reinterpret_cast<bf16x4*>(orow + K + i) = p0;
-        *reinterpret_cast<bf16x4*>(orow + 2 * K + i) = p0;
+        if (nseg == 3) *reinterpret_cast<bf16x4*>(orow + 2 * K + i) = p0;
     }
 }
 
@@ -390,7 +405,7 @@
                                                                const int* __restrict__ tok_id, const float* __restrict__ w,
                                                                bf16_t* __restrict__ xs, float* __restrict__ a_inv, int T, float eps,
                                                                const float* __restrict__ gu_cmax, float* __restrict__ act_sc,
-                                                               float* __restrict__ act_inv) {
+                                                               float* __restrict__ act_inv, int nseg) {
     constexpr int K = 256 * NV;
     const int t = blockIdx.x * 4 + (threadIdx.x >> 6);
     const int lane = threadIdx.x & 63;
@@ -432,7 +447,7 @@
         const float osc = row_scale_pow2(s2 * *gu_cmax * 1.02f);
         if (lane == 0) { act_sc[t] = osc; act_inv[t] = 1.0f / osc; }
     }
-    bf16_t* orow = xs + (int64_t)t * K * 3;
+    bf16_t* orow = xs + (int64_t)t * K * nseg;
 #pragma unroll
     for (int j = 0; j < NV; ++j) {
         bf16x4 p0, p1;
@@ -445,24 +460,24 @@
         const int i = lane * 4 + 256 * j;
         *reinterpret_cast<bf16x4*>(orow + i) = p1;
         *reinterpret_cast<bf16x4*>(orow + K + i) = p0;
-        *reinterpret_cast<bf16x4*>(orow + 2 * K + i) = p0;
+        if (nseg == 3) *reinterpret_cast<bf16x4*>(orow + 2 * K + i) = p0;
     }
 }
 
 static void launch_rows_split_h(float* x, const float* embed, const int* tok, const float* w, bf16_t* xs, float* inv, int T, int K,
-                                float eps, hipStream_t s, const float* gu_cmax = nullptr, float* act_sc = nullptr,
+                                float eps, int nseg, hipStream_t s, const float* gu_cmax = nullptr, float* act_sc = nullptr,
                                 float* act_inv = nullptr) {
     const dim3 grid((unsigned)ceil_div64(T, 4)), block(256);
     switch (K) {
-        case 2048: hipLaunchKernelGGL(rows_split_h_reg_kernel<8>, grid, block, 0, s, x, embed, tok, w, xs, inv, T, eps, gu_cmax, act_sc, act_inv); break;
-        case 4096: hipLaunchKernelGGL(rows_split_h_reg_kernel<16>, grid, block, 0, s, x, embed, tok, w, xs, inv, T, eps, gu_cmax, act_sc, act_inv); break;
-        case 8192: hipLaunchKernelGGL(rows_split_h_reg_kernel<32>, grid, block, 0, s, x, embed, tok, w, xs, inv, T, eps, gu_cmax, act_sc, act_inv); break;
-        default: hipLaunchKernelGGL(rows_split_h_kernel, grid, block, 0, s, x, embed, tok, w, xs, inv, T, K, eps, gu_cmax, act_sc, act_inv);
+        case 2048: hipLaunchKernelGGL(rows_split_h_reg_kernel<8>, grid, block, 0, s, x, embed, tok, w, xs, inv, T, eps, gu_cmax, act_sc, act_inv, nseg); break;
+        case 4096: hipLaunchKernelGGL(rows_split_h_reg_kernel<16>, grid, block, 0, s, x, embed, tok, w, xs, inv, T, eps, gu_cmax, act_sc, act_inv, nseg); break;
+        case 8192: hipLaunchKernelGGL(rows_split_h_reg_kernel<32>, grid, block, 0, s, x, embed, tok, w, xs, inv, T, eps, gu_cmax, act_sc, act_inv, nseg); break;
+        default: hipLaunchKernelGGL(rows_split_h_kernel, grid, block, 0, s, x, embed, tok, w, xs, inv, T, K, eps, gu_cmax, act_sc, act_inv, nseg);
     }
 }
 
 __global__ __launch_bounds__(256) void gu_cmax_kernel(const bf16_t* __restrict__ wgu_s, const float* __restrict__ wgu_i, int I, int K,
-                                                      float* __restrict__ cmax) {
+                                                      int nseg, float* __restrict__ cmax) {
     const int j = blockIdx.x * 4 + (threadIdx.x >> 6);
     const int lane = threadIdx.x & 63;
     if (j >= I) return;
@@ -470,10 +485,11 @@
     float n2[2];
 #pragma unroll
     for (int h = 0; h < 2; ++h) {
-        const bf16_t* row = wgu_s + (h ? ru : rg) * 3 * (int64_t)K;
+        const bf16_t* row = wgu_s + (h ? ru : rg) * nseg * (int64_t)K;
         float ss = 0.f;
         for (int i = lane; i < K; i += 64) {
-            const float v = (float)__builtin_bit_cast(_Float16, row[i]) + (float)__builtin_bit_cast(_Float16, row[K + i]);
+            const float v = (float)__builtin_bit_cast(_Float16, row[i]) +
+                            (nseg == 3 ? (float)__builtin_bit_cast(_Float16, row[K + i]) : 0.f);
             ss += v * v;
         }
         for (int off = 32; off > 0; off >>= 1) ss += __shfl_xor(ss, off);
@@ -547,6 +563,7 @@
     bf16_t *wqkv_s = nullptr, *wo_s = nullptr, *wgu_s = nullptr, *wdown_s = nullptr;
     float *wqkv_i = nullptr, *wo_i = nullptr, *wgu_i = nullptr, *wdown_i = nullptr;
     float* gu_cmax = nullptr;
+    int qkv_seg = 3, o_seg = 3, gu_seg = 3, down_seg = 3;
 };
 
 struct sr_model {
@@ -557,6 +574,8 @@
     bf16_t* lm_head = nullptr;
     bf16_t* lm_head_s = nullptr;
     float* lm_head_i = nullptr;
+    int lm_head_seg = 3;
+    int* lo_nz = nullptr;
     float *attn_f = nullptr, *act_f = nullptr;
     float *xs_i = nullptr, *attn_i = nullptr, *act_i = nullptr;
     float* act_sc = nullptr;
@@ -588,7 +607,7 @@
     auto F = [](void* p) { if (p) (void)hipFree(p); };
     F(m->embed); F(m->lm_head); F(m->norm_w); F(m->rope_cos); F(m->rope_sin);
     F(m->lm_head_s); F(m->xs); F(m->qkv_f); F(m->attn_s); F(m->act_s);
-    F(m->lm_head_i); F(m->attn_f); F(m->act_f); F(m->xs_i); F(m->attn_i); F(m->act_i); F(m->act_sc);
+    F(m->lm_head_i); F(m->lo_nz); F(m->attn_f); F(m->act_f); F(m->xs_i); F(m->attn_i); F(m->act_i); F(m->act_sc);
     for (auto& l : m->layers) {
         F(l.wqkv); F(l.wo); F(l.wgu); F(l.wdown); F(l.ln1); F(l.ln2); F(l.wqkv_s); F(l.wo_s); F(l.wgu_s); F(l.wdown_s);
         F(l.wqkv_i); F(l.wo_i); F(l.wgu_i); F(l.wdown_i); F(l.gu_cmax);
@@ -668,6 +687,10 @@
     const bool f16p = c.fp32_planes == SR_FP32_PLANES_F16;
     if (c.has_lm_head && nsg) SR_ALLOC(m->lm_head_s, V * H * 2 * nsg);
     if (c.has_lm_head && f16p) SR_ALLOC(m->lm_head_i, V * 4);
+    if (f16p) {
+        SR_ALLOC(m->lo_nz, (4 * (int64_t)c.num_layers + 1) * 4);
+        (void)hipMemset(m->lo_nz, 0, (size_t)(4 * c.num_layers + 1) * 4);
+    }
     SR_ALLOC(m->norm_w, H * 4);
     for (auto& l : m->layers) {
         SR_ALLOC(l.wqkv, (nq + 2 * nkv) * H * 2);
@@ -738,12 +761,13 @@
 }
 
 static int convert_rows(const void* src, int dtype, int64_t rows, int64_t cols, bf16_t* dbf, float* df32, int64_t base,
-                        int interleave, hipStream_t s, bf16_t* dsplit = nullptr, int planes = 0, float* w_inv = nullptr) {
+                        int interleave, hipStream_t s, bf16_t* dsplit = nullptr, int planes = 0, float* w_inv = nullptr,
+                        int* lo_nz = nullptr) {
     hipLaunchKernelGGL(convert_rows_kernel, dim3((unsigned)rows), dim3(256), 0, s, src, dtype, rows, cols, dbf, df32, base,
                        interleave);
     if (dsplit && planes == SR_FP32_PLANES_F16)
         hipLaunchKernelGGL(convert_rows_split_h_kernel, dim3((unsigned)rows), dim3(256), 0, s, src, dtype, rows, cols, dsplit, w_inv, base,
-                           interleave);
+                           interleave, lo_nz);
     else if (dsplit && planes)
         hipLaunchKernelGGL(convert_rows_split_kernel, dim3((unsigned)rows), dim3(256), 0, s, src, dtype, rows, cols, dsplit, base,
                            interleave, split_map_w(planes));
@@ -757,8 +781,12 @@
     SR_REQUIRE(dtype == SR_DTYPE_F32 || dtype == SR_DTYPE_BF16, "sr_model_set_weight: dtype %d not supported", dtype);
     hipStream_t s = (hipStream_t)stream;
     std::lock_guard<std::mutex> lock(m->mu);
+    SR_REQUIRE(!m->finalized, "sr_model_set_weight: the model is already finalized; weights are fixed from then on");
     const sr_model_config& c = m->cfg;
     const int64_t H = c.hidden_size, I = c.intermediate_size, V = c.vocab_size;
+    int* const lo_nz = m->lo_nz;
+    auto lo_flag = [&](int64_t i) { return lo_nz ? lo_nz + i : nullptr; };
+    const int64_t lo_lm = 4 * (int64_t)c.num_layers;
     const int64_t nq = (int64_t)c.num_heads * c.head_dim, nkv = (int64_t)c.num_kv_heads * c.head_dim;
     std::string n(name);
     auto shape_is = [&](int64_t r, int64_t cc) { return rows == r && cols == cc; };
@@ -766,7 +794,8 @@
     if (n == "model.embed_tokens.weight") {
         SHAPE_REQ(V, H);
         SR_TRY(convert_rows(d_ptr, dtype, V, H, (c.has_lm_head && c.tie_word_embeddings) ? m->lm_head : nullptr, m->embed, 0, 0, s,
-                            (c.has_lm_head && c.tie_word_embeddings) ? m->lm_head_s : nullptr, c.fp32_planes, m->lm_head_i));
+                            (c.has_lm_head && c.tie_word_embeddings) ? m->lm_head_s : nullptr, c.fp32_planes, m->lm_head_i,
+                            lo_flag(lo_lm)));
         m->have_embed = true;
         if (c.has_lm_head && c.tie_word_embeddings) m->have_lm_head = true;
         return SR_OK;
@@ -774,7 +803,7 @@
     if (n == "lm_head.weight") {
         SR_REQUIRE(c.has_lm_head, "sr_model_set_weight: model was created without an lm_head");
         SHAPE_REQ(V, H);
-        SR_TRY(convert_rows(d_ptr, dtype, V, H, m->lm_head, nullptr, 0, 0, s, m->lm_head_s, c.fp32_planes, m->lm_head_i));
+        SR_TRY(convert_rows(d_ptr, dtype, V, H, m->lm_head, nullptr, 0, 0, s, m->lm_head_s, c.fp32_planes, m->lm_head_i, lo_flag(lo_lm)));
         m->have_lm_head = true;
         return SR_OK;
     }
@@ -789,18 +818,37 @@
     if (sscanf(name, "model.layers.%d.%127s", &li, rest) == 2 && li >= 0 && li < c.num_layers) {
         LayerW& l = m->layers[li];
         std::string r(rest);
-        if (r == "self_attn.q_proj.weight") { SHAPE_REQ(nq, H); SR_TRY(convert_rows(d_ptr, dtype, nq, H, l.wqkv, nullptr, 0, 0, s, l.wqkv_s, c.fp32_planes, l.wqkv_i)); l.have |= 1; return SR_OK; }
-        if (r == "self_attn.k_proj.weight") { SHAPE_REQ(nkv, H); SR_TRY(convert_rows(d_ptr, dtype, nkv, H, l.wqkv, nullptr, nq, 0, s, l.wqkv_s, c.fp32_planes, l.wqkv_i)); l.have |= 2; return SR_OK; }
-        if (r == "self_attn.v_proj.weight") { SHAPE_REQ(nkv, H); SR_TRY(convert_rows(d_ptr, dtype, nkv, H, l.wqkv, nullptr, nq + nkv, 0, s, l.wqkv_s, c.fp32_planes, l.wqkv_i)); l.have |= 4; return SR_OK; }
-        if (r == "self_attn.o_proj.weight") { SHAPE_REQ(H, nq); SR_TRY(convert_rows(d_ptr, dtype, H, nq, l.wo, nullptr, 0, 0, s, l.wo_s, c.fp32_planes, l.wo_i)); l.have |= 8; return SR_OK; }
-        if (r == "mlp.gate_proj.weight") { SHAPE_REQ(I, H); SR_TRY(convert_rows(d_ptr, dtype, I, H, l.wgu, nullptr, 0, 1, s, l.wgu_s, c.fp32_planes, l.wgu_i)); l.have |= 16; return SR_OK; }
-        if (r == "mlp.up_proj.weight") { SHAPE_REQ(I, H); SR_TRY(convert_rows(d_ptr, dtype, I, H, l.wgu, nullptr, 0, 2, s, l.wgu_s, c.fp32_planes, l.wgu_i)); l.have |= 32; return SR_OK; }
-        if (r == "mlp.down_proj.weight") { SHAPE_REQ(H, I); SR_TRY(convert_rows(d_ptr, dtype, H, I, l.wdown, nullptr, 0, 0, s, l.wdown_s, c.fp32_planes, l.wdown_i)); l.have |= 64; return SR_OK; }
+        if (r == "self_attn.q_proj.weight") { SHAPE_REQ(nq, H); SR_TRY(convert_rows(d_ptr, dtype, nq, H, l.wqkv, nullptr, 0, 0, s, l.wqkv_s, c.fp32_planes, l.wqkv_i, lo_flag(4 * li + 0))); l.have |= 1; return SR_OK; }
+        if (r == "self_attn.k_proj.weight") { SHAPE_REQ(nkv, H); SR_TRY(convert_rows(d_ptr, dtype, nkv, H, l.wqkv, nullptr, nq, 0, s, l.wqkv_s, c.fp32_planes, l.wqkv_i, lo_flag(4 * li + 0))); l.have |= 2; return SR_OK; }
+        if (r == "self_attn.v_proj.weight") { SHAPE_REQ(nkv, H); SR_TRY(convert_rows(d_ptr, dtype, nkv, H, l.wqkv, nullptr, nq + nkv, 0, s, l.wqkv_s, c.fp32_planes, l.wqkv_i, lo_flag(4 * li + 0))); l.have |= 4; return SR_OK; }
+        if (r == "self_attn.o_proj.weight") { SHAPE_REQ(H, nq); SR_TRY(convert_rows(d_ptr, dtype, H, nq, l.wo, nullptr, 0, 0, s, l.wo_s, c.fp32_planes, l.wo_i, lo_flag(4 * li + 1))); l.have |= 8; return SR_OK; }
+        if (r == "mlp.gate_proj.weight") { SHAPE_REQ(I, H); SR_TRY(convert_rows(d_ptr, dtype, I, H, l.wgu, nullptr, 0, 1, s, l.wgu_s, c.fp32_planes, l.wgu_i, lo_flag(4 * li + 2))); l.have |= 16; return SR_OK; }
+        if (r == "mlp.up_proj.weight") { SHAPE_REQ(I, H); SR_TRY(convert_rows(d_ptr, dtype, I, H, l.wgu, nullptr, 0, 2, s, l.wgu_s, c.fp32_planes, l.wgu_i, lo_flag(4 * li + 2))); l.have |= 32; return SR_OK; }
+        if (r == "mlp.down_proj.weight") { SHAPE_REQ(H, I); SR_TRY(convert_rows(d_ptr, dtype, H, I, l.wdown, nullptr, 0, 0, s, l.wdown_s, c.fp32_planes, l.wdown_i, lo_flag(4 * li + 3))); l.have |= 64; return SR_OK; }
         if (r == "input_layernorm.weight") { SHAPE_REQ(H, 1); SR_TRY(convert_rows(d_ptr, dtype, H, 1, nullptr, l.ln1, 0, 0, s)); l.have |= 128; return SR_OK; }
         if (r == "post_attention_layernorm.weight") { SHAPE_REQ(H, 1); SR_TRY(convert_rows(d_ptr, dtype, H, 1, nullptr, l.ln2, 0, 0, s)); l.have |= 256; return SR_OK; }
     }
     sr_set_error("sr_model_set_weight: unknown tensor name '%s'", name);
     return SR_ERR_INVALID;
+}
+
+static int pack_f16_weights(bf16_t*& w, int& nseg, bool lo_nz, int64_t rows, int64_t K) {
+    if (nseg == 2 || lo_nz) return SR_OK;
+    bf16_t* p = nullptr;
+    SR_CHECK_HIP(hipMalloc((void**)&p, (size_t)(rows * 2 * K * 2)));
+    hipLaunchKernelGGL(pack_rows_2seg_kernel, dim3((unsigned)rows), dim3(256), 0, nullptr, w, p, K);
+    hipError_t e = hipGetLastError();
+    if (e == hipSuccess) e = hipDeviceSynchronize();
+    if (e != hipSuccess) {
+        (void)hipFree(p);
+        sr_set_error("sr_model_finalize: re-packing a [%lld, %lld] weight matrix failed: %s", (long long)rows, (long long)K,
+                     hipGetErrorString(e));
+        return SR_ERR_HIP;
+    }
+    SR_CHECK_HIP(hipFree(w));
+    w = p;
+    nseg = 2;
+    return SR_OK;
 }
 
 extern "C" int sr_model_finalize(sr_model* m) {
@@ -812,17 +860,51 @@
         SR_REQUIRE(m->layers[i].have == 511, "sr_model_finalize: layer %d is missing tensors (mask 0x%x)", i, m->layers[i].have);
     SR_CHECK_HIP(hipDeviceSynchronize());
     if (m->cfg.fp32_planes == SR_FP32_PLANES_F16) {
-        for (int i = 0; i < m->cfg.num_layers; ++i) {
+        const sr_model_config& c = m->cfg;
+        const int64_t H = c.hidden_size, I = c.intermediate_size, V = c.vocab_size;
+        const int64_t nq = (int64_t)c.num_heads * c.head_dim, nkv = (int64_t)c.num_kv_heads * c.head_dim;
+        std::vector<int> nz((size_t)(4 * c.num_layers + 1));
+        SR_CHECK_HIP(hipMemcpy(nz.data(), m->lo_nz, nz.size() * 4, hipMemcpyDeviceToHost));
+        const char* env_seg = sr_dev_getenv("SR_F16_WEIGHT_SEGS");
+        if (!(env_seg && *env_seg == '3')) {
+            for (int i = 0; i < c.num_layers; ++i) {
+                LayerW& l = m->layers[i];
+                SR_TRY(pack_f16_weights(l.wqkv_s, l.qkv_seg, nz[4 * i + 0] != 0, nq + 2 * nkv, H));
+                SR_TRY(pack_f16_weights(l.wo_s, l.o_seg, nz[4 * i + 1] != 0, H, nq));
+                SR_TRY(pack_f16_weights(l.wgu_s, l.gu_seg, nz[4 * i + 2] != 0, 2 * I, H));
+                SR_TRY(pack_f16_weights(l.wdown_s, l.down_seg, nz[4 * i + 3] != 0, H, I));
+            }
+            if (c.has_lm_head) SR_TRY(pack_f16_weights(m->lm_head_s, m->lm_head_seg, nz[4 * c.num_layers] != 0, V, H));
+        }
+        for (int i = 0; i < c.num_layers; ++i) {
             LayerW& l = m->layers[i];
             if (!l.gu_cmax) SR_CHECK_HIP(hipMalloc((void**)&l.gu_cmax, 4));
             SR_CHECK_HIP(hipMemsetAsync(l.gu_cmax, 0, 4, nullptr));
-            hipLaunchKernelGGL(gu_cmax_kernel, dim3((unsigned)ceil_div64(m->cfg.intermediate_size, 4)), dim3(256), 0, nullptr, l.wgu_s, l.wgu_i,
-                               m->cfg.intermediate_size, m->cfg.hidden_size, l.gu_cmax);
+            hipLaunchKernelGGL(gu_cmax_kernel, dim3((unsigned)ceil_div64(I, 4)), dim3(256), 0, nullptr, l.wgu_s, l.wgu_i, (int)I, (int)H,
+                               l.gu_seg, l.gu_cmax);
         }
         SR_CHECK_LAUNCH();
     }
     SR_CHECK_HIP(hipDeviceSynchronize());
     m->finalized = true;
+    return SR_OK;
+}
+
+extern "C" int sr_model_weight_segments(sr_model* m, int32_t* out, int64_t capacity, int64_t* n) {
+    SR_REQUIRE(m && n, "sr_model_weight_segments: null argument");
+    SR_REQUIRE(m->finalized, "sr_model_weight_segments: sr_model_finalize was not called");
+    const sr_model_config& c = m->cfg;
+    std::vector<int32_t> v;
+    const bool f16p = c.fp32_planes == SR_FP32_PLANES_F16;
+    const int32_t plain = c.fp32_planes ? split_map_w(c.fp32_planes).n_seg : 0;
+    for (const LayerW& l : m->layers) {
+        v.push_back(f16p ? l.qkv_seg : plain); v.push_back(f16p ? l.o_seg : plain);
+        v.push_back(f16p ? l.gu_seg : plain); v.push_back(f16p ? l.down_seg : plain);
+    }
+    if (c.has_lm_head) v.push_back(f16p ? m->lm_head_seg : plain);
+    *n = (int64_t)v.size();
+    SR_REQUIRE(capacity >= 0 && (capacity == 0 || out), "sr_model_weight_segments: bad output buffer");
+    for (int64_t i = 0; i < capacity && i < (int64_t)v.size(); ++i) out[i] = v[(size_t)i];
     return SR_OK;
 }
 
@@ -895,16 +977,17 @@
     SR_CHECK_LAUNCH();
 
     if (prec == PREC_FP32 && c.fp32_planes == SR_FP32_PLANES_F16) {
-        auto split_rows = [&](float* src, const float* embed, const int* tok, const float* w, bf16_t* dst, float* inv, int K) {
-            launch_rows_split_h(src, embed, tok, w, dst, inv, T, K, c.rms_norm_eps, s);
+        auto split_rows = [&](float* src, const float* embed, const int* tok, const float* w, bf16_t* dst, float* inv, int K, int nseg) {
+            launch_rows_split_h(src, embed, tok, w, dst, inv, T, K, c.rms_norm_eps, nseg, s);
         };
         const char* env_fa = sr_dev_getenv("SR_FP32_FUSED_ACT");
         const bool fused_act = m->layers[0].gu_cmax && !(env_fa && *env_fa == '0');
         for (int li = 0; li < c.num_layers; ++li) {
             LayerW& l = m->layers[li];
-            split_rows(m->x, li == 0 ? m->embed : (const float*)nullptr, li == 0 ? m->tok_id : (const int*)nullptr, l.ln1, m->xs, m->xs_i, H);
+            split_rows(m->x, li == 0 ? m->embed : (const float*)nullptr, li == 0 ? m->tok_id : (const int*)nullptr, l.ln1, m->xs, m->xs_i, H,
+                       l.qkv_seg);
             GemmArgs g{};
-            g.A = m->xs; g.W = l.wqkv_s; g.M = T; g.N = nq + 2 * nkv; g.K = 3 * H; g.C = m->qkv_f; g.a_scale = m->xs_i; g.w_scale = l.wqkv_i;
+            g.A = m->xs; g.W = l.wqkv_s; g.M = T; g.N = nq + 2 * nkv; g.K = l.qkv_seg * H; g.C = m->qkv_f; g.a_scale = m->xs_i; g.w_scale = l.wqkv_i;
             g.pos = m->pos; g.rope_cos = m->rope_cos; g.rope_sin = m->rope_sin; g.n_rope = nq + nkv; g.head_dim = c.head_dim;
             SR_TRY(launch_gemm_bf16(EPI_QKV_ROPE_F32_H, g, s));
             AttnF32Args a{};
@@ -912,25 +995,26 @@
             a.B = B; a.nh = c.num_heads; a.nkv = c.num_kv_heads; a.hd = c.head_dim;
             a.scale = 1.0f / sqrtf((float)c.head_dim); a.max_seqlen = max_len;
             SR_TRY(launch_attention_f32(a, s));
-            split_rows(m->attn_f, nullptr, nullptr, nullptr, m->attn_s, m->attn_i, nq);
+            split_rows(m->attn_f, nullptr, nullptr, nullptr, m->attn_s, m->attn_i, nq, l.o_seg);
             g = GemmArgs{};
-            g.A = m->attn_s; g.W = l.wo_s; g.M = T; g.N = H; g.K = 3 * nq; g.C = m->x; g.a_scale = m->attn_i; g.w_scale = l.wo_i;
+            g.A = m->attn_s; g.W = l.wo_s; g.M = T; g.N = H; g.K = l.o_seg * nq; g.C = m->x; g.a_scale = m->attn_i; g.w_scale = l.wo_i;
             SR_TRY(launch_gemm_bf16(EPI_RESID_F32_H, g, s));
             if (fused_act) {
-                launch_rows_split_h(m->x, nullptr, nullptr, l.ln2, m->xs, m->xs_i, T, H, c.rms_norm_eps, s, l.gu_cmax, m->act_sc, m->act_i);
+                launch_rows_split_h(m->x, nullptr, nullptr, l.ln2, m->xs, m->xs_i, T, H, c.rms_norm_eps, l.gu_seg, s, l.gu_cmax, m->act_sc,
+                                    m->act_i);
                 g = GemmArgs{};
-                g.A = m->xs; g.W = l.wgu_s; g.M = T; g.N = 2 * I; g.K = 3 * H; g.C = m->act_s; g.a_scale = m->xs_i; g.w_scale = l.wgu_i;
-                g.out_scale = m->act_sc;
+                g.A = m->xs; g.W = l.wgu_s; g.M = T; g.N = 2 * I; g.K = l.gu_seg * H; g.C = m->act_s; g.a_scale = m->xs_i; g.w_scale = l.wgu_i;
+                g.out_scale = m->act_sc; g.out_nseg = l.down_seg;
                 SR_TRY(launch_gemm_bf16(EPI_SWIGLU_SPLIT_H, g, s));
             } else {
-                split_rows(m->x, nullptr, nullptr, l.ln2, m->xs, m->xs_i, H);
+                split_rows(m->x, nullptr, nullptr, l.ln2, m->xs, m->xs_i, H, l.gu_seg);
                 g = GemmArgs{};
-                g.A = m->xs; g.W = l.wgu_s; g.M = T; g.N = 2 * I; g.K = 3 * H; g.C = m->act_f; g.a_scale = m->xs_i; g.w_scale = l.wgu_i;
+                g.A = m->xs; g.W = l.wgu_s; g.M = T; g.N = 2 * I; g.K = l.gu_seg * H; g.C = m->act_f; g.a_scale = m->xs_i; g.w_scale = l.wgu_i;
                 SR_TRY(launch_gemm_bf16(EPI_SWIGLU_F32_H, g, s));
-                split_rows(m->act_f, nullptr, nullptr, nullptr, m->act_s, m->act_i, I);
+                split_rows(m->act_f, nullptr, nullptr, nullptr, m->act_s, m->act_i, I, l.down_seg);
             }
             g = GemmArgs{};
-            g.A = m->act_s; g.W = l.wdown_s; g.M = T; g.N = H; g.K = 3 * I; g.C = m->x; g.a_scale = m->act_i; g.w_scale = l.wdown_i;
+            g.A = m->act_s; g.W = l.wdown_s; g.M = T; g.N = H; g.K = l.down_seg * I; g.C = m->x; g.a_scale = m->act_i; g.w_scale = l.wdown_i;
             SR_TRY(launch_gemm_bf16(EPI_RESID_F32_H, g, s));
         }
         SR_CHECK_LAUNCH();
@@ -1024,8 +1108,8 @@
     GemmEpilogue epi = EPI_SEGMAX;
     if (prec == PREC_FP32 && m->cfg.fp32_planes == SR_FP32_PLANES_F16) {
         launch_rows_split_h(m->x, (const float*)nullptr, (const int*)nullptr, (const float*)m->norm_w, m->xs, m->xs_i, T, H,
-                            m->cfg.rms_norm_eps, s);
-        g.A = m->xs; g.W = m->lm_head_s; g.K = 3 * H; g.a_scale = m->xs_i; g.w_scale = m->lm_head_i;
+                            m->cfg.rms_norm_eps, m->lm_head_seg, s);
+        g.A = m->xs; g.W = m->lm_head_s; g.K = m->lm_head_seg * H; g.a_scale = m->xs_i; g.w_scale = m->lm_head_i;
         epi = EPI_SEGMAX_H;
     } else if (prec == PREC_FP32) {
         const SplitMap ma = split_map_a(m->cfg.fp32_planes);
diff --git a/scaling_retriever_amd/csrc/gemm_bf16.hip b/scaling_retriever_amd/csrc/gemm_bf16.hip
--- a/scaling_retriever_amd/csrc/gemm_bf16.hip
+++ b/scaling_retriever_amd/csrc/gemm_bf16.hip
@@ -621,7 +621,8 @@
     } else if constexpr (KL == 1 && BEPI == EPI_SWIGLU_SPLITH_BASE) {
         unsigned char* const stg0 = smem + 2 * STAGE_BYTES + wave * 8192;
         const int half_n = g.N >> 1;
-        const int64_t ldc = 3 * (int64_t)half_n;
+        const bool seg3 = g.out_nseg == 3;
+        const int64_t ldc = (int64_t)g.out_nseg * half_n;
         const int nb = (n0 >> 1) + wn * 64;
 #pragma unroll
         for (int j = 0; j < MB; ++j) {
@@ -654,7 +655,7 @@
                         *reinterpret_cast<sr_i32x4*>(crow) = v;
                     } else {
                         *reinterpret_cast<sr_i32x4*>(crow + half_n) = v;
-                        *reinterpret_cast<sr_i32x4*>(crow + 2 * half_n) = v;
+                        if (seg3) *reinterpret_cast<sr_i32x4*>(crow + 2 * half_n) = v;
                     }
                 }
             }
@@ -766,7 +767,8 @@
         }
     } else if constexpr (BEPI == EPI_SWIGLU_SPLITH_BASE) {
         const int half_n = g.N >> 1;
-        const int64_t ldc = 3 * (int64_t)half_n;
+        const bool seg3 = g.out_nseg == 3;
+        const int64_t ldc = (int64_t)g.out_nseg * half_n;
 #pragma unroll
         for (int j = 0; j < MB; ++j) {
             const int m = m0 + wm * MB * 16 + j * 16 + frow;
@@ -788,7 +790,7 @@
                 bf16_t* crow = reinterpret_cast<bf16_t*>(g.C) + (int64_t)m * ldc + n;
                 *reinterpret_cast<bf16x4*>(crow) = p1;
                 *reinterpret_cast<bf16x4*>(crow + half_n) = p0;
-                *reinterpret_cast<bf16x4*>(crow + 2 * half_n) = p0;
+                if (seg3) *reinterpret_cast<bf16x4*>(crow + 2 * half_n) = p0;
             }
         }
     } else if constexpr (BEPI == EPI_SWIGLU_SPLIT) {
@@ -1002,7 +1004,7 @@
     t.A = g.A + (int64_t)row0 * g.K;
     t.M = g.M - row0;
     const int64_t ldc = (EPI == EPI_SWIGLU || EPI == EPI_SWIGLU_F32 || EPI == EPI_SWIGLU_F32_H)
-                            ? g.N / 2 : (EPI == EPI_SWIGLU_SPLIT ? (int64_t)g.out_map.n_seg * (g.N / 2) : (EPI == EPI_SWIGLU_SPLIT_H ? 3 * (int64_t)(g.N / 2) : g.N));
+                            ? g.N / 2 : (EPI == EPI_SWIGLU_SPLIT ? (int64_t)g.out_map.n_seg * (g.N / 2) : (EPI == EPI_SWIGLU_SPLIT_H ? (int64_t)g.out_nseg * (g.N / 2) : g.N));
     const int64_t esz = (EPI == EPI_STORE_F32 || EPI == EPI_RESID_F32 || EPI == EPI_QKV_ROPE_F32 || EPI == EPI_SWIGLU_F32 ||
                          (EPI >= EPI_H_FIRST && EPI != EPI_SWIGLU_SPLIT_H)) ? 4 : 2;
     if constexpr (EPI != EPI_SEGMAX && EPI != EPI_SEGMAX_H) t.C = reinterpret_cast<unsigned char*>(g.C) + (int64_t)row0 * ldc * esz;
@@ -1062,6 +1064,8 @@
     SR_REQUIRE(g.K % G_BK == 0, "gemm: K=%d must be a multiple of %d", g.K, G_BK);
     const bool swiglu = epi == EPI_SWIGLU || epi == EPI_SWIGLU_SPLIT || epi == EPI_SWIGLU_F32 || epi == EPI_SWIGLU_F32_H || epi == EPI_SWIGLU_SPLIT_H;
     SR_REQUIRE(epi != EPI_SWIGLU_SPLIT_H || g.out_scale, "gemm(swiglu split, fp16 planes): missing output row scales");
+    SR_REQUIRE(epi != EPI_SWIGLU_SPLIT_H || g.out_nseg == 2 || g.out_nseg == 3, "gemm(swiglu split, fp16 planes): out_nseg %d is not 2 or 3",
+               g.out_nseg);
     SR_REQUIRE(g.N % 16 == 0 && (!swiglu || g.N % 32 == 0), "gemm: N=%d must be a multiple of 16 (32 for SwiGLU)", g.N);
     SR_REQUIRE(epi < EPI_H_FIRST || (g.a_scale && g.w_scale), "gemm(fp16 planes): missing row scales");
     SR_REQUIRE(epi != EPI_SWIGLU_SPLIT || (g.out_map.n_seg >= 1 && g.out_map.n_seg <= SR_MAX_SEG), "gemm(swiglu split): bad segment map");
diff --git a/scaling_retriever_amd/csrc/kernels.h b/scaling_retriever_amd/csrc/kernels.h
--- a/scaling_retriever_amd/csrc/kernels.h
+++ b/scaling_retriever_amd/csrc/kernels.h
@@ -50,6 +50,7 @@
     const float* a_scale;
     const float* w_scale;
     const float* out_scale;
+    int out_nseg;
     SplitMap out_map;
     int m_fastest;
     int xcd_order;
diff --git a/scaling_retriever_amd/modeling/llm_encoder.py b/scaling_retriever_amd/modeling/llm_encoder.py
--- a/scaling_retriever_amd/modeling/llm_encoder.py
+++ b/scaling_retriever_amd/modeling/llm_encoder.py
@@ -335,6 +335,15 @@
             _lib.check(self._lib.sr_model_last_hidden(self._h, buf.data_ptr(), buf.shape[0], ctypes.byref(n),
                                                       _lib.stream_ptr()), "sr_model_last_hidden")
         return buf[:n.value]
+
+    def weight_segments(self):
+        if self._h is None:
+            raise _lib.SrHipError("the model has no engine yet (call .to(device) first)")
+        n = ctypes.c_int64(0)
+        _lib.check(self._lib.sr_model_weight_segments(self._h, None, 0, ctypes.byref(n)), "sr_model_weight_segments")
+        out = (ctypes.c_int32 * max(n.value, 1))()
+        _lib.check(self._lib.sr_model_weight_segments(self._h, out, n.value, ctypes.byref(n)), "sr_model_weight_segments")
+        return [int(v) for v in out[:n.value]]
 
     def __del__(self):
         try:
```

New measurement: 16200, median of 6. 19.0% higher.
